# alberto-paparella/MusicRecommendation

Measured on AMD Instinct MI355X. Metric: scored (test-user,song) pairs/sec, ItemBasedModel, 1/2/4/8 MI355X + mAP@10, higher is better.
Workload: dtype int64

## Files before the change

### include/mr_engine.h

```cpp
#ifndef MR_ENGINE_H
#define MR_ENGINE_H

#include <stdint.h>
#include <stddef.h>

#ifdef __cplusplus
extern "C" {
#endif

#define MR_OK          0
#define MR_E_INVALID  -1
#define MR_E_HIP      -2
#define MR_E_OOM      -3
#define MR_E_STATE    -4
#define MR_E_IO       -5
#define MR_E_PARSE    -6
#define MR_E_RCCL     -7

#define MR_UBM 0
#define MR_IBM 1

#define MR_OUT_F32 0
#define MR_OUT_F64 1

typedef struct mr_dataset {
  int32_t n_train_users;
  int32_t n_test_users;
  int32_t n_songs;
  int32_t reserved0;
  const int64_t* tr_off;
  const int32_t* tr_songs;
  const int64_t* te_off;
  const int32_t* te_songs;
  const int32_t* song_count;
  const int32_t* tr_len;
  const int32_t* te_len;
} mr_dataset;

typedef struct mr_options {
  int32_t device;
  int32_t frac_bits;
  int32_t song_lo;
  int32_t song_hi;
  int32_t block_songs;
  int32_t out_dtype;
  int32_t topk;
  int32_t dense;
  int32_t time_kernels;
  int32_t stage1;
  int32_t stage1_chunk;
  int32_t train_order;
  int32_t topk_lists;
  int32_t ibm_route;
  int32_t reserved[2];
} mr_options;

typedef struct mr_ctx mr_ctx;

int mr_options_default(mr_options* opt);

int mr_create(const mr_options* opt, mr_ctx** out);
int mr_destroy(mr_ctx* ctx);

int mr_load(mr_ctx* ctx, const mr_dataset* d);

int mr_shard_info(const mr_ctx* ctx, int32_t* song_lo, int32_t* song_hi, int32_t* n_test_users);

int mr_launch_info(const mr_ctx* ctx, int32_t* shape, int32_t* block_songs, int32_t* n_tiles);

int mr_batch_info(const mr_ctx* ctx, int32_t* batch, int32_t* chunk, int32_t* n_chunks);

int mr_route_info(const mr_ctx* ctx, int32_t* route, int32_t* n_rows, int64_t* pool_entries);

int mr_topk_mode(const mr_ctx* ctx, int32_t* candidate_only);

int mr_cooc_stats(mr_ctx* ctx, int64_t* index_nnz, int64_t* consumed, int64_t* build_reads);

typedef struct mr_cooc_bytes_t {
  int64_t heavy_rows, light_rows;
  int64_t heavy_reads, light_reads;
  int64_t heavy_index_bytes, light_index_bytes;
  int64_t heavy_visits;
  int64_t consumed_bytes;
  int64_t group_tiles;
  int64_t n_groups;
  int64_t index_sparse_entries, index_dense_songs;
  int64_t consumed_sparse_entries, consumed_dense_songs;
} mr_cooc_bytes_t;
int mr_cooc_bytes(mr_ctx* ctx, mr_cooc_bytes_t* out);

int mr_shard_tile_songs(const mr_options* opt, int32_t n_train_users, int32_t n_test_users,
                        int32_t* tile_songs);

int mr_shard_tile_songs_n(const mr_options* opt, int32_t n_train_users, int32_t n_test_users, int32_t n_songs,
                          int32_t n_shards, int32_t* tile_songs);

int mr_run(mr_ctx* ctx, int model);
int mr_sync(mr_ctx* ctx);

int mr_graph_capture(mr_ctx* ctx, int model, int32_t n_steps);
int mr_graph_launch(mr_ctx* ctx);

int mr_device_outputs(const mr_ctx* ctx, void** dense, int32_t** topk_songs,
                      int64_t** topk_keys, double** topk_scores);

int mr_run_into(mr_ctx* ctx, int model, void* dense_dev);

typedef struct mr_view {
  int32_t n_test_users, n_songs, song_lo, song_hi, out_dtype, device;
  const int64_t* te_off;
  const int32_t* te_songs;
  void* stream;
} mr_view;
int mr_view_get(const mr_ctx* ctx, mr_view* view);

int mr_topk_dense_device(mr_ctx* ctx, const void* dense_dev, int32_t k);

int mr_score_dense(mr_ctx* ctx, int model, void* out);
int mr_topk(mr_ctx* ctx, int model, int k, int32_t* songs, double* scores, int64_t* keys);

int mr_copy_dense(mr_ctx* ctx, void* out);
int mr_copy_topk(mr_ctx* ctx, int32_t* songs, double* scores, int64_t* keys);
int mr_copy_topk_device(mr_ctx* ctx, int32_t* songs, int64_t* keys);
int mr_copy_topk_device_async(mr_ctx* ctx, int32_t* songs, int64_t* keys);

int mr_topk_merge_host(int32_t n_shards, int32_t n_te, int32_t k,
                       const int32_t* songs_in, const int64_t* keys_in, const double* scores_in,
                       int32_t* songs_out, int64_t* keys_out, double* scores_out);
int mr_topk_merge_device(mr_ctx* ctx, int32_t n_shards, int32_t n_te, int32_t k,
                         const int32_t* songs_in, const int64_t* keys_in, const double* scores_in,
                         int32_t* songs_out, int64_t* keys_out, double* scores_out);
int mr_topk_merge_device_async(mr_ctx* ctx, int32_t n_shards, int32_t n_te, int32_t k, const int32_t* songs_in,
                               const int64_t* keys_in, int32_t* songs_out, int64_t* keys_out, double* scores_out);

int mr_topk_record_bytes(int32_t n_te, int32_t k, int64_t* rec_bytes);
int mr_topk_merge_records_async(mr_ctx* ctx, int32_t n_shards, int32_t n_te, int32_t k, const void* records,
                                int64_t rec_bytes, int32_t* songs_out, int64_t* keys_out, double* scores_out);

#define MR_COMB_LINEAR      0
#define MR_COMB_AGGREGATION 1
#define MR_COMB_STOCHASTIC  2
int mr_combine_device(mr_ctx* ctx, int kind, double param, uint64_t seed, int64_t pair_base, int64_t n_pairs,
                      const void* ubm, const void* ibm, void* out);
int mr_combine_all_device(mr_ctx* ctx, double alpha, double ibm_percentage, double ibm_probability, uint64_t seed,
                          int64_t pair_base, int64_t n_pairs, const void* ubm, const void* ibm, void* out_linear,
                          void* out_aggregation, void* out_stochastic, double* minmax);
int mr_eval_minmax_device(mr_ctx* ctx, const void* dense, double* mn, double* mx);
int mr_dense_minmax(mr_ctx* ctx, double* mn, double* mx);
int mr_eval_counts_device(mr_ctx* ctx, const void* dense, double mn, double mx, const int64_t* lab_off,
                          const int32_t* lab_songs, int32_t* pred_counts, int32_t* tp_counts, int32_t n_thresholds);
int mr_eval_map(int32_t n_classes, const int32_t* pred_counts, const int32_t* tp_counts, const int32_t* pos,
                int32_t n_label_songs, double* map_out, int32_t n_thresholds);
int mr_eval_map_device(mr_ctx* ctx, const void* dense, double mn, double mx, const int64_t* lab_off,
                       const int32_t* lab_songs, const int32_t* pos, int32_t n_label_songs, double* map_out,
                       int32_t n_thresholds);
int mr_eval_class_counts_device(mr_ctx* ctx, int32_t n_models, const void* const* dense, const double* mn,
                                const double* mx, const int64_t* lab_off, const int32_t* lab_songs, int32_t n_classes,
                                const int32_t* classes, int32_t* counts, int32_t n_thresholds);
int mr_eval_map_counts_device(mr_ctx* ctx, int32_t n_models, int32_t n_classes, const int32_t* class_pos,
                              const int32_t* counts, int32_t n_label_songs, double* maps_out, int32_t n_thresholds);

#define MR_SWEEP_MAX_PARAMS 64
int mr_sweep_minmax_device(mr_ctx* ctx, int kind, int32_t n_params, const double* params, uint64_t seed,
                           int64_t pair_base, int64_t n_pairs, const void* ubm, const void* ibm, double* mn,
                           double* mx);
int mr_sweep_class_counts_device(mr_ctx* ctx, int kind, int32_t n_params, const double* params, uint64_t seed,
                                 int64_t pair_base, int64_t n_pairs, const void* ubm, const void* ibm,
                                 const double* mn, const double* mx, const int64_t* lab_off,
                                 const int32_t* lab_songs, int32_t n_classes, const int32_t* classes,
                                 int32_t* counts, int32_t n_thresholds);
int mr_sweep_map_device(mr_ctx* ctx, int kind, int32_t n_params, const double* params, uint64_t seed,
                        int64_t pair_base, int64_t n_pairs, const void* ubm, const void* ibm, const int64_t* lab_off,
                        const int32_t* lab_songs, const int32_t* pos, int32_t n_label_songs, double* maps_out,
                        double* minmax_out, int32_t n_thresholds);

#define MR_RANK_MAX_K 1024
int mr_rank_dense_device(mr_ctx* ctx, const void* dense_dev, int32_t K, int32_t* songs_dev, double* scores_dev);
int mr_rank_merge_host(int32_t n_lists, int32_t n_te, int32_t K, const int32_t* songs_in, const double* scores_in,
                       int32_t* songs_out, double* scores_out);
int mr_rank_map_device(mr_ctx* ctx, const int32_t* songs_dev, int32_t K, int32_t k_eval, const int64_t* lab_off,
                       const int32_t* lab_songs, double* ap_out, double* map_out);
int mr_rank_map_host(int32_t n_te, const int32_t* songs, int32_t K, int32_t k_eval, const int64_t* lab_off,
                     const int32_t* lab_songs, double* ap_out, double* map_out);

#define MR_SIMILAR_SCRATCH_BYTES (256 << 20)
int mr_similar_songs_device(mr_ctx* ctx, int32_t n_q, const int32_t* query_songs , int32_t K,
                            int32_t* songs_dev, double* scores_dev, double* dense_dev);

#define MR_ASYM_MAX_Q 8
int mr_asym_tables(double alpha, int32_t n, const int32_t* counts, double* pow_a, double* pow_b);
int mr_ibm_asym_device(mr_ctx* ctx, double alpha, int32_t q, void* dense_dev);

#define MR_UASYM_SCRATCH_BYTES (256 << 20)
int mr_ubm_asym_device(mr_ctx* ctx, double alpha, int32_t q, int32_t frac_bits, void* dense_dev);

int mr_kernel_times(mr_ctx* ctx, int32_t which, int64_t* launches, double* total_ms, int32_t reset);

int mr_timing_begin(mr_ctx* ctx);
int mr_timing_stop(mr_ctx* ctx);
int mr_timing_end(mr_ctx* ctx, int64_t* launches, double* total_ms);

int mr_debug_stamps(mr_ctx* ctx, int64_t* out, int64_t n);

void* mr_stream(const mr_ctx* ctx);

const char* mr_last_error(void);

#define MR_TRANSPORT_AUTO 0
#define MR_TRANSPORT_COPY 1
#define MR_TRANSPORT_RCCL 2

typedef struct mr_group_options {
  int32_t n_song_shards;
  int32_t n_user_blocks;
  int32_t transport;
  int32_t n_devices;
  const int32_t* devices;
} mr_group_options;

typedef struct mr_group mr_group;

// ... 45 lines not shown
```

### musicrecommendation_amd/_lib.py

```python
from __future__ import annotations

import ctypes
import os
from ctypes import POINTER, c_char_p, c_double, c_int, c_int32, c_int64, c_void_p

_HERE = os.path.dirname(os.path.abspath(__file__))
_VARIANT = os.environ.get("MR_ENGINE_LIB", "")
LIB_PATH = os.path.join(_HERE, f"libmr_engine_{_VARIANT}.so" if _VARIANT else "libmr_engine.so")

MR_OK = 0
MR_E_INVALID = -1
MR_E_HIP = -2
MR_E_OOM = -3
MR_E_STATE = -4
MR_E_IO = -5
MR_E_PARSE = -6
MR_E_RCCL = -7
MR_TRANSPORT_AUTO, MR_TRANSPORT_COPY, MR_TRANSPORT_RCCL = 0, 1, 2
MR_UBM = 0
MR_IBM = 1
STAGE1 = {"auto": 0, "fused": 1, "separate": 2, "wide": 4}
SHAPES = {0: "separate", 1: "fused", 3: "wide"}
MR_OUT_F32 = 0
MR_OUT_F64 = 1

_ERRNAMES = {
    MR_E_INVALID: "MR_E_INVALID",
    MR_E_HIP: "MR_E_HIP",
    MR_E_OOM: "MR_E_OOM",
    MR_E_STATE: "MR_E_STATE",
    MR_E_IO: "MR_E_IO",
    MR_E_PARSE: "MR_E_PARSE",
    MR_E_RCCL: "MR_E_RCCL",
}


class MrDataset(ctypes.Structure):
    _fields_ = [
        ("n_train_users", c_int32),
        ("n_test_users", c_int32),
        ("n_songs", c_int32),
        ("reserved0", c_int32),
        ("tr_off", POINTER(c_int64)),
        ("tr_songs", POINTER(c_int32)),
        ("te_off", POINTER(c_int64)),
        ("te_songs", POINTER(c_int32)),
        ("song_count", POINTER(c_int32)),
        ("tr_len", POINTER(c_int32)),
        ("te_len", POINTER(c_int32)),
    ]


class MrOptions(ctypes.Structure):
    _fields_ = [
        ("device", c_int32),
        ("frac_bits", c_int32),
        ("song_lo", c_int32),
        ("song_hi", c_int32),
        ("block_songs", c_int32),
        ("out_dtype", c_int32),
        ("topk", c_int32),
        ("dense", c_int32),
        ("time_kernels", c_int32),
        ("stage1", c_int32),
        ("stage1_chunk", c_int32),
        ("train_order", c_int32),
        ("topk_lists", c_int32),
        ("ibm_route", c_int32),
        ("reserved", c_int32 * 2),
    ]


class MrGroupOptions(ctypes.Structure):
    _fields_ = [
        ("n_song_shards", c_int32),
        ("n_user_blocks", c_int32),
        ("transport", c_int32),
        ("n_devices", c_int32),
        ("devices", POINTER(c_int32)),
    ]


class MrView(ctypes.Structure):
    _fields_ = [
        ("n_test_users", c_int32),
        ("n_songs", c_int32),
        ("song_lo", c_int32),
        ("song_hi", c_int32),
        ("out_dtype", c_int32),
        ("device", c_int32),
        ("te_off", c_void_p),
        ("te_songs", c_void_p),
        ("stream", c_void_p),
    ]


class MrCoocBytes(ctypes.Structure):
    _fields_ = [(n, c_int64) for n in ("heavy_rows", "light_rows", "heavy_reads", "light_reads",
                                       "heavy_index_bytes", "light_index_bytes", "heavy_visits", "consumed_bytes",
                                       "group_tiles", "n_groups", "index_sparse_entries", "index_dense_songs",
                                       "consumed_sparse_entries", "consumed_dense_songs")]


MR_COMB_LINEAR = 0
MR_COMB_AGGREGATION = 1
MR_COMB_STOCHASTIC = 2
MR_SWEEP_MAX_PARAMS = 64
MR_RANK_MAX_K = 1024
MR_ASYM_MAX_Q = 8


class EngineError(RuntimeError):
    def __init__(self, code: int, where: str, msg: str):
        super().__init__(f"{where}: {_ERRNAMES.get(code, code)}: {msg}")
        self.code = code


SIGNATURES = {
    "mr_options_default": (c_int, [POINTER(MrOptions)]),
    "mr_create": (c_int, [POINTER(MrOptions), POINTER(c_void_p)]),
    "mr_destroy": (c_int, [c_void_p]),
    "mr_load": (c_int, [c_void_p, POINTER(MrDataset)]),
    "mr_shard_info": (c_int, [c_void_p, POINTER(c_int32), POINTER(c_int32), POINTER(c_int32)]),
    "mr_launch_info": (c_int, [c_void_p, POINTER(c_int32), POINTER(c_int32), POINTER(c_int32)]),
    "mr_batch_info": (c_int, [c_void_p, POINTER(c_int32), POINTER(c_int32), POINTER(c_int32)]),
    "mr_route_info": (c_int, [c_void_p, POINTER(c_int32), POINTER(c_int32), POINTER(c_int64)]),
    "mr_topk_mode": (c_int, [c_void_p, POINTER(c_int32)]),
    "mr_cooc_stats": (c_int, [c_void_p, POINTER(c_int64), POINTER(c_int64), POINTER(c_int64)]),
    "mr_cooc_bytes": (c_int, [c_void_p, POINTER(MrCoocBytes)]),
    "mr_shard_tile_songs": (c_int, [POINTER(MrOptions), c_int32, c_int32, POINTER(c_int32)]),
    "mr_shard_tile_songs_n": (c_int, [POINTER(MrOptions), c_int32, c_int32, c_int32, c_int32, POINTER(c_int32)]),
    "mr_run": (c_int, [c_void_p, c_int]),
    "mr_sync": (c_int, [c_void_p]),
    "mr_graph_capture": (c_int, [c_void_p, c_int, c_int32]),
    "mr_graph_launch": (c_int, [c_void_p]),
    "mr_device_outputs": (c_int, [c_void_p, POINTER(c_void_p), POINTER(c_void_p), POINTER(c_void_p), POINTER(c_void_p)]),
    "mr_score_dense": (c_int, [c_void_p, c_int, c_void_p]),
    "mr_topk": (c_int, [c_void_p, c_int, c_int, c_void_p, c_void_p, c_void_p]),
    "mr_copy_dense": (c_int, [c_void_p, c_void_p]),
    "mr_copy_topk": (c_int, [c_void_p, c_void_p, c_void_p, c_void_p]),
    "mr_copy_topk_device": (c_int, [c_void_p, c_void_p, c_void_p]),
    "mr_copy_topk_device_async": (c_int, [c_void_p, c_void_p, c_void_p]),
    "mr_topk_merge_device_async": (c_int, [c_void_p, c_int32, c_int32, c_int32, c_void_p, c_void_p, c_void_p, c_void_p,
                                           c_void_p]),
    "mr_topk_record_bytes": (c_int, [c_int32, c_int32, POINTER(c_int64)]),
    "mr_topk_merge_records_async": (c_int, [c_void_p, c_int32, c_int32, c_int32, c_void_p, c_int64, c_void_p, c_void_p,
                                            c_void_p]),
    "mr_topk_merge_host": (c_int, [c_int32, c_int32, c_int32, c_void_p, c_void_p, c_void_p, c_void_p, c_void_p, c_void_p]),
    "mr_topk_merge_device": (c_int, [c_void_p, c_int32, c_int32, c_int32, c_void_p, c_void_p, c_void_p, c_void_p, c_void_p, c_void_p]),
    "mr_kernel_times": (c_int, [c_void_p, c_int32, POINTER(c_int64), POINTER(c_double), c_int32]),
    "mr_debug_stamps": (c_int, [c_void_p, c_void_p, c_int64]),
    "mr_timing_begin": (c_int, [c_void_p]),
    "mr_timing_stop": (c_int, [c_void_p]),
    "mr_timing_end": (c_int, [c_void_p, POINTER(c_int64), POINTER(c_double)]),
    "mr_stream": (c_void_p, [c_void_p]),
    "mr_run_into": (c_int, [c_void_p, c_int, c_void_p]),
    "mr_view_get": (c_int, [c_void_p, POINTER(MrView)]),
    "mr_topk_dense_device": (c_int, [c_void_p, c_void_p, c_int32]),
    "mr_combine_device": (c_int, [c_void_p, c_int, c_double, ctypes.c_uint64, c_int64, c_int64, c_void_p, c_void_p, c_void_p]),
    "mr_combine_all_device": (c_int, [c_void_p, c_double, c_double, c_double, ctypes.c_uint64, c_int64, c_int64,
                                      c_void_p, c_void_p, c_void_p, c_void_p, c_void_p, POINTER(c_double)]),
    "mr_eval_minmax_device": (c_int, [c_void_p, c_void_p, POINTER(c_double), POINTER(c_double)]),
    "mr_dense_minmax": (c_int, [c_void_p, POINTER(c_double), POINTER(c_double)]),
    "mr_eval_counts_device": (c_int, [c_void_p, c_void_p, c_double, c_double, c_void_p, c_void_p, c_void_p, c_void_p,
                                      c_int32]),
    "mr_eval_map_device": (c_int, [c_void_p, c_void_p, c_double, c_double, c_void_p, c_void_p, c_void_p, c_int32,
                                   POINTER(c_double), c_int32]),
    "mr_eval_map": (c_int, [c_int32, c_void_p, c_void_p, c_void_p, c_int32, POINTER(c_double), c_int32]),
    "mr_eval_class_counts_device": (c_int, [c_void_p, c_int32, c_void_p, c_void_p, c_void_p, c_void_p, c_void_p,
                                            c_int32, c_void_p, c_void_p, c_int32]),
    "mr_eval_map_counts_device": (c_int, [c_void_p, c_int32, c_int32, c_void_p, c_void_p, c_int32, c_void_p,
                                          c_int32]),
    "mr_sweep_minmax_device": (c_int, [c_void_p, c_int, c_int32, c_void_p, ctypes.c_uint64, c_int64, c_int64, c_void_p,
                                       c_void_p, c_void_p, c_void_p]),
    "mr_sweep_class_counts_device": (c_int, [c_void_p, c_int, c_int32, c_void_p, ctypes.c_uint64, c_int64, c_int64,
                                             c_void_p, c_void_p, c_void_p, c_void_p, c_void_p, c_void_p, c_int32,
                                             c_void_p, c_void_p, c_int32]),
    "mr_sweep_map_device": (c_int, [c_void_p, c_int, c_int32, c_void_p, ctypes.c_uint64, c_int64, c_int64, c_void_p,
                                    c_void_p, c_void_p, c_void_p, c_void_p, c_int32, c_void_p, c_void_p, c_int32]),
    "mr_rank_dense_device": (c_int, [c_void_p, c_void_p, c_int32, c_void_p, c_void_p]),
    "mr_rank_merge_host": (c_int, [c_int32, c_int32, c_int32, c_void_p, c_void_p, c_void_p, c_void_p]),
    "mr_rank_map_device": (c_int, [c_void_p, c_void_p, c_int32, c_int32, c_void_p, c_void_p, c_void_p,
                                   POINTER(c_double)]),
    "mr_rank_map_host": (c_int, [c_int32, c_void_p, c_int32, c_int32, c_void_p, c_void_p, c_void_p,
                                 POINTER(c_double)]),
    "mr_similar_songs_device": (c_int, [c_void_p, c_int32, c_void_p, c_int32, c_void_p, c_void_p, c_void_p]),
    "mr_asym_tables": (c_int, [c_double, c_int32, c_void_p, c_void_p, c_void_p]),
    "mr_ibm_asym_device": (c_int, [c_void_p, c_double, c_int32, c_void_p]),
    "mr_ubm_asym_device": (c_int, [c_void_p, c_double, c_int32, c_int32, c_void_p]),
    "mr_last_error": (c_char_p, []),
    "mr_corpus_from_tsv": (c_int, [c_char_p, c_char_p, c_char_p, POINTER(c_void_p)]),
    "mr_corpus_dataset": (c_int, [c_void_p, POINTER(MrDataset)]),
    "mr_corpus_labels": (c_int, [c_void_p, POINTER(POINTER(c_int64)), POINTER(POINTER(c_int32)), POINTER(c_int32), POINTER(c_int32)]),
    "mr_corpus_name": (c_char_p, [c_void_p, c_int32, c_int32]),
    "mr_corpus_names": (c_int, [c_void_p, c_int32, c_char_p, c_int64, POINTER(c_int64)]),
    "mr_corpus_free": (c_int, [c_void_p]),
    "mr_version": (c_char_p, []),
    "mr_model_write_tsv": (c_int, [c_char_p, c_int32, c_int32, c_void_p, c_void_p, c_void_p, c_int32]),
    "mr_model_read_tsv": (c_int, [c_char_p, c_int32, c_int32, c_void_p, c_void_p, c_void_p]),
    "mr_java_double_string": (c_int, [c_double, c_char_p, c_int32]),
    "mr_song_shards": (c_int, [POINTER(MrDataset), c_int32, c_void_p]),
    "mr_song_shards_tiled": (c_int, [POINTER(MrDataset), c_int32, c_int32, c_void_p]),
    "mr_group_options_default": (c_int, [POINTER(MrGroupOptions)]),
    "mr_group_create": (c_int, [POINTER(MrOptions), POINTER(MrGroupOptions), POINTER(c_void_p)]),
    "mr_group_destroy": (c_int, [c_void_p]),
    "mr_group_load": (c_int, [c_void_p, POINTER(MrDataset)]),
    "mr_group_info": (c_int, [c_void_p, c_int32, POINTER(c_int32), POINTER(c_int32), POINTER(c_int32),
                              POINTER(c_int32), POINTER(c_int32)]),
    "mr_group_transport": (c_int, [c_void_p, POINTER(c_int32)]),
    "mr_group_shape": (c_int, [c_void_p, POINTER(c_int32), POINTER(c_int32), POINTER(c_int32)]),
    "mr_group_context": (c_void_p, [c_void_p, c_int32]),
    "mr_group_run": (c_int, [c_void_p, c_int]),
    "mr_group_sync": (c_int, [c_void_p]),
    "mr_group_copy_topk": (c_int, [c_void_p, c_void_p, c_void_p, c_void_p]),
    "mr_group_topk": (c_int, [c_void_p, c_int, c_int, c_void_p, c_void_p, c_void_p]),
    "mr_group_device_topk": (c_int, [c_void_p, c_int32, POINTER(c_void_p), POINTER(c_void_p), POINTER(c_void_p)]),
    "mr_group_copy_dense": (c_int, [c_void_p, c_void_p]),
    "mr_group_score_dense": (c_int, [c_void_p, c_int, c_void_p]),
    "mr_group_allgather_dense": (c_int, [c_void_p, c_void_p]),
}

_lib = None


def _preload_torch_runtime() -> None:
    try:
        import torch
    except Exception:
        pass


def lib() -> ctypes.CDLL:
    global _lib
    if _lib is not None:
        return _lib
    if not os.path.exists(LIB_PATH):
        raise ImportError(
            f"{LIB_PATH} is missing: build the HIP engine first "
            "(python -c 'import __graft_entry__ as g; g.build()'); there is no CPU fallback"
        )
    _preload_torch_runtime()
    L = ctypes.CDLL(LIB_PATH)
    for name, (res, args) in SIGNATURES.items():
        fn = getattr(L, name)
        fn.restype = res
        fn.argtypes = args
    _lib = L
    return L


def check(rc: int, where: str) -> None:
    if rc != MR_OK:
        msg = lib().mr_last_error()
        raise EngineError(rc, where, msg.decode() if msg else "")
```

### musicrecommendation_amd/csrc/mr_engine.hip

```cpp
#include <hip/hip_runtime.h>

#include <algorithm>
#include <atomic>
#include <climits>
#include <cmath>
#include <cstdarg>
#include <cstdio>
#include <cstdlib>
#include <cstring>
#include <limits>
#include <mutex>
#include <string>
#include <vector>

#ifndef MR_TILE_ROWS
#define MR_TILE_ROWS 32
#endif

#include "mr_engine.h"
#include "mr_hip_util.h"
#include "mr_internal.h"
#include "mr_par.h"
#include "mr_tile_walk.h"


namespace {

using mr_internal::kGridRows;
using mr_internal::kGridRowsXcd;

constexpr int kThreads = 256;
constexpr int kWaves = kThreads / 64;
constexpr int kMaxTopK = 64;
constexpr int kMaxBlockSongs = 16384;
constexpr int kLdsBytes = 160 * 1024;
constexpr int kMaxWideBlockSongs = 65536;
constexpr int kMaxLdsTrainUsers = 16384;
constexpr int kStage1Chunk = 4096;
constexpr int kMaxChunks = 2048;
constexpr int kMaxFusedTrainUsers = 4096;
constexpr long long kKeyNone = -1;
constexpr int kMaxTopkTile = 1024;
constexpr int kMaxTopkLarge = 16;
constexpr int kFusedPre = 4;
constexpr int kWideMapDefault = 1;

thread_local std::string g_err = "no error";

int fail(int code, const char* fmt, ...) {
  char buf[1024];
  va_list ap;
  va_start(ap, fmt);
  vsnprintf(buf, sizeof buf, fmt, ap);
  va_end(ap);
  g_err = buf;
  return code;
}

}

namespace mr_host {
int fail(int code, const char* fmt, ...) {
  char buf[1024];
  va_list ap;
  va_start(ap, fmt);
  vsnprintf(buf, sizeof buf, fmt, ap);
  va_end(ap);
  g_err = buf;
  return code;
}
}

namespace {

struct ScoreLds {
  int acc, y, heard, s_lo, s_w, s_pre, s_scan, wk, ws, fk, fs, flag, cpre, stg, gm, stage_lists, total;
};
constexpr int kTopkScratch256 = (64 + 1) * 12 + 4 + 64 * 4 + 256 * 4;

constexpr int kStgItems = 256;
constexpr int kStgBytes = kStgItems * 8 + kStgItems * 4 + (kStgItems + 4) * 4;

__host__ __device__ inline int align16(int x) { return (x + 15) & ~15; }
__host__ __device__ inline int merge_lists_per_pass(int k);

__host__ __device__ inline ScoreLds score_lds(int bs, int fused_ntr, int k, int n_tiles, int n_chunks = 0) {
  ScoreLds L;
  const int fused = fused_ntr > 0 ? 1 : 0;
  const int kk = k > 0 ? k : 1;
  const int per = merge_lists_per_pass(kk);
  L.stage_lists = (k > 0 && n_tiles > 1) ? (n_tiles < per ? n_tiles : per) : 0;
  int a_bytes = bs * 8 + fused_ntr * 8;
  const int st_bytes = L.stage_lists * kk * 8 + align16(L.stage_lists * kk * 4);
  const int wide_bytes = (k > 0 && bs > kMaxTopkTile) ? kThreads * kk * 8 + kThreads * kk * 4 : 0;
  if (wide_bytes > a_bytes) a_bytes = wide_bytes;
  int o = 0;
  L.acc = o; L.y = bs * 8; o = align16(a_bytes > st_bytes ? a_bytes : st_bytes);
  L.heard = o; o = align16(o + (bs / 32) * 4);
  L.s_lo = o; o += fused * kThreads * 8;
  L.s_w = o; o += fused * kThreads * 8;
  L.s_pre = o; o = align16(o + (kThreads + 1) * 4);
  L.s_scan = o; o = align16(o + kWaves * 4);
  L.wk = o; o = align16(o + kWaves * kMaxTopK * 8);
  L.ws = o; o = align16(o + kWaves * kMaxTopK * 4);
  L.fk = o; o = align16(o + kMaxTopK * 8);
  L.fs = o; o = align16(o + kMaxTopK * 4);
  L.flag = o; o = align16(o + 16);
  L.cpre = o; o = align16(o + (n_chunks > 0 ? (n_chunks + 1) * 4 : 0));
  L.stg = o; o = align16(o + (n_chunks > 0 ? kWaves * kStgBytes : 0));
  L.gm = o; o = align16(o + kTopkScratch256);
  L.total = o;
  return L;
}


constexpr int kStampSlots = 32;
__device__ __forceinline__ void stamp_at(long long* sb, int i) {
#ifdef MR_STAMPS
  if (sb && threadIdx.x == 0) {
    sb[i] = (long long)__builtin_amdgcn_s_memrealtime();
    sb[16 + i] = (long long)__builtin_amdgcn_s_memtime();
  }
#endif
}
__device__ __forceinline__ void stamp_rt(long long* sb, int i) {
#ifdef MR_STAMPS
  if (sb && threadIdx.x == 0) sb[i] = (long long)__builtin_amdgcn_s_memrealtime();
#endif
}
__device__ __forceinline__ void stamp_rt_wave(long long* sb, int i) {
#ifdef MR_STAMPS
  if (sb && (threadIdx.x & 63) == 0) sb[i] = (long long)__builtin_amdgcn_s_memrealtime();
#endif
}
__device__ __forceinline__ void stamp_val(long long* sb, int i, long long v, bool wave = false) {
#ifdef MR_STAMPS
  if (sb && (wave ? (threadIdx.x & 63) == 0 : threadIdx.x == 0)) sb[i] = v;
#endif
}
#ifdef MR_STAMPS
#define MR_STAMP(i) stamp_at(p.stamps ? p.stamps + ((size_t)blockIdx.y * gridDim.x + blockIdx.x) * kStampSlots : nullptr, (i))
#else
#define MR_STAMP(i) do {} while (0)
#endif

__device__ __forceinline__ int wave_incl_scan(int x) {
#ifndef MR_NO_DPP
  x += __builtin_amdgcn_update_dpp(0, x, 0x111, 0xf, 0xf, false);
  x += __builtin_amdgcn_update_dpp(0, x, 0x112, 0xf, 0xf, false);
  x += __builtin_amdgcn_update_dpp(0, x, 0x114, 0xf, 0xf, false);
  x += __builtin_amdgcn_update_dpp(0, x, 0x118, 0xf, 0xf, false);
  x += __builtin_amdgcn_update_dpp(0, x, 0x142, 0xa, 0xf, false);
  x += __builtin_amdgcn_update_dpp(0, x, 0x143, 0xc, 0xf, false);
#else
  const int lane = threadIdx.x & 63;
#pragma unroll
  for (int d = 1; d < 64; d <<= 1) {
    const int y = __shfl_up(x, d, 64);
    if (lane >= d) x += y;
  }
#endif
  return x;
}

__device__ __forceinline__ int wave_lane(int x, int l) { return __builtin_amdgcn_readlane(x, l); }

__host__ __device__ inline unsigned long long ordered_key(double x) {
  unsigned long long b;
  memcpy(&b, &x, sizeof b);
  return (b >> 63) ? ~b : (b | (1ull << 63));
}
__host__ __device__ inline double ordered_value(unsigned long long k) {
  const unsigned long long b = (k >> 63) ? (k & ~(1ull << 63)) : ~k;
  double x;
  memcpy(&x, &b, sizeof x);
  return x;
}

__device__ __forceinline__ int block_excl_scan(int x, int* total, int* sbuf) {
  const int lane = threadIdx.x & 63, w = threadIdx.x >> 6;
  const int incl = wave_incl_scan(x);
  if (lane == 63) sbuf[w] = incl;
  __syncthreads();
  int off = 0, tot = 0;
#pragma unroll
  for (int i = 0; i < kWaves; ++i) {
    int s = sbuf[i];
    off += (i < w) ? s : 0;
    tot += s;
  }
  __syncthreads();
  *total = tot;
  return off + incl - x;
}

__device__ __forceinline__ bool cand_before(long long ka, int sa, long long kb, int sb) {
  return ka > kb || (ka == kb && sa < sb);
}


#define MR_DPP(op, x, mod) asm volatile("s_nop 1\n\t" op " %0, %0, %0 " mod : "+v"(x))
#define MR_DPP_REDUCE(op, x)                                          \
  do {                                                                \
    MR_DPP(op, x, "row_shr:1 row_mask:0xf bank_mask:0xf");            \
    MR_DPP(op, x, "row_shr:2 row_mask:0xf bank_mask:0xf");            \
    MR_DPP(op, x, "row_shr:4 row_mask:0xf bank_mask:0xf");            \
    MR_DPP(op, x, "row_shr:8 row_mask:0xf bank_mask:0xf");            \
    MR_DPP(op, x, "row_bcast:15 row_mask:0xa bank_mask:0xf");         \
    MR_DPP(op, x, "row_bcast:31 row_mask:0xc bank_mask:0xf");         \
    asm volatile("s_nop 1" ::: "memory");                             \
  } while (0)

__device__ __forceinline__ int wave_max_i32(int x) {
  MR_DPP_REDUCE("v_max_i32_dpp", x);
  return __builtin_amdgcn_readlane(x, 63);
}
__device__ __forceinline__ unsigned wave_max_u32(unsigned x) {
  MR_DPP_REDUCE("v_max_u32_dpp", x);
  return (unsigned)__builtin_amdgcn_readlane((int)x, 63);
}
__device__ __forceinline__ int wave_min_i32(int x) {
  MR_DPP_REDUCE("v_min_i32_dpp", x);
  return __builtin_amdgcn_readlane(x, 63);
}

__device__ __forceinline__ void wave_argmax(long long& k, int& s) {
  const int hi = (int)(k >> 32);
  const unsigned lo = (unsigned)(k & 0xffffffffll);
  const int H = wave_max_i32(hi);
  unsigned long long m = __ballot(hi == H);
  unsigned Lo;
  if (__popcll(m) == 1) {
    const int l = __ffsll((long long)m) - 1;
    Lo = (unsigned)__builtin_amdgcn_readlane((int)lo, l);
    s = __builtin_amdgcn_readlane(s, l);
  } else {
    Lo = wave_max_u32(hi == H ? lo : 0u);
    m = __ballot(hi == H && lo == Lo);
    if (__popcll(m) == 1) {
      s = __builtin_amdgcn_readlane(s, __ffsll((long long)m) - 1);
    } else {
      s = wave_min_i32((hi == H && lo == Lo) ? s : INT_MAX);
    }
  }
  k = (long long)(((unsigned long long)(unsigned)H << 32) | Lo);
}

__device__ __forceinline__ void take_if_before(long long& ka, int& sa, long long kb, int sb) {
  const bool t = cand_before(kb, sb, ka, sa);
  ka = t ? kb : ka;
  sa = t ? sb : sa;
}

template <int CTRL>
__device__ __forceinline__ void dpp_take(long long& k, int& s) {
  const unsigned lo = (unsigned)__builtin_amdgcn_update_dpp(0, (int)(unsigned)(unsigned long long)k, CTRL, 0xf, 0xf,
                                                            false);
  const int hi = __builtin_amdgcn_update_dpp(0, (int)(k >> 32), CTRL, 0xf, 0xf, false);
  const int os = __builtin_amdgcn_update_dpp(0, s, CTRL, 0xf, 0xf, false);
  take_if_before(k, s, (long long)(((unsigned long long)(unsigned)hi << 32) | lo), os);
}

template <int GS>
__device__ __forceinline__ void group_best(long long& k, int& s) {
  static_assert(GS == 1 || GS == 2 || GS == 4 || GS == 8 || GS == 16, "group size");
  if constexpr (GS >= 2) dpp_take<0xB1>(k, s);
  if constexpr (GS >= 4) dpp_take<0x4E>(k, s);
  if constexpr (GS >= 8) dpp_take<0x141>(k, s);
  if constexpr (GS >= 16) dpp_take<0x140>(k, s);
}

template <int M>
__device__ __forceinline__ void lane_sort(long long (&rk)[M], int (&rs)[M]) {
#pragma unroll
  for (int round = 0; round < M; ++round) {
#pragma unroll
    for (int j = round & 1; j + 1 < M; j += 2) {
      const bool sw = cand_before(rk[j + 1], rs[j + 1], rk[j], rs[j]);
      const long long k0 = rk[j], k1 = rk[j + 1];
      const int s0 = rs[j], s1 = rs[j + 1];
      rk[j] = sw ? k1 : k0;
      rk[j + 1] = sw ? k0 : k1;
      rs[j] = sw ? s1 : s0;
      rs[j + 1] = sw ? s0 : s1;
    }
  }
}

template <int M, bool SORTED = false>
__device__ __forceinline__ void wave_topk_regs(long long (&rk)[M], int (&rs)[M], int k, long long* out_k,
                                               int* out_s) {
  const int lane = threadIdx.x & 63;
#pragma unroll
  for (int j = 0; j < M; ++j)
    if (rk[j] < 0) { rk[j] = kKeyNone; rs[j] = INT_MAX; }
  if (!SORTED) lane_sort<M>(rk, rs);
  int r = 0;
  for (; r < k; ++r) {
    long long bk = rk[0];
    int bs = rs[0];
    wave_argmax(bk, bs);
    if (bk < 0) break;
    if (lane == 0) { out_k[r] = bk; out_s[r] = bs; }
    const bool win = rk[0] == bk && rs[0] == bs;
#pragma unroll
    for (int j = 0; j + 1 < M; ++j) {
      rk[j] = win ? rk[j + 1] : rk[j];
      rs[j] = win ? rs[j + 1] : rs[j];
    }
    rk[M - 1] = win ? kKeyNone : rk[M - 1];
    rs[M - 1] = win ? INT_MAX : rs[M - 1];
  }
  for (int i = r + lane; i < k; i += 64) { out_k[i] = kKeyNone; out_s[i] = -1; }
}

__device__ __forceinline__ void wave_merge_lists(int L, int k, const long long* lk, const int* ls,
                                                 long long* out_k, int* out_s) {
  const int lane = threadIdx.x & 63;
  int pos[4];
  long long hk[4], nk[4];
  int hs[4], ns[4];
#pragma unroll
  for (int j = 0; j < 4; ++j) {
    const int l = lane + 64 * j;
    pos[j] = 0;
    hk[j] = nk[j] = kKeyNone;
    hs[j] = ns[j] = INT_MAX;
    if (l < L) {
      hk[j] = lk[(size_t)l * k];
      hs[j] = ls[(size_t)l * k];
      if (k > 1) {
        nk[j] = lk[(size_t)l * k + 1];
        ns[j] = ls[(size_t)l * k + 1];
      }
    }
    if (hk[j] < 0) { hk[j] = kKeyNone; hs[j] = INT_MAX; }
    if (nk[j] < 0) { nk[j] = kKeyNone; ns[j] = INT_MAX; }
  }
  int r = 0;
  for (; r < k; ++r) {
    long long bk = hk[0];
    int bs = hs[0];
#pragma unroll
    for (int j = 1; j < 4; ++j) take_if_before(bk, bs, hk[j], hs[j]);
    wave_argmax(bk, bs);
    if (bk < 0) break;
    if (lane == 0) { out_k[r] = bk; out_s[r] = bs; }
#pragma unroll
    for (int j = 0; j < 4; ++j) {
      if (hk[j] == bk && hs[j] == bs) {
        hk[j] = nk[j];
        hs[j] = ns[j];
        ++pos[j];
        nk[j] = kKeyNone;
        ns[j] = INT_MAX;
        if (pos[j] + 1 < k) {
          const int l = lane + 64 * j;
          nk[j] = lk[(size_t)l * k + pos[j] + 1];
          ns[j] = ls[(size_t)l * k + pos[j] + 1];
          if (nk[j] < 0) { nk[j] = kKeyNone; ns[j] = INT_MAX; }
        }
      }
    }
  }
  for (int i = r + lane; i < k; i += 64) { out_k[i] = kKeyNone; out_s[i] = -1; }
}

template <typename Get>
__device__ __forceinline__ void block_topk(int n, int k, Get get, long long* wk, int* ws, long long* out_k,
                                           int* out_s) {
  const int w = threadIdx.x >> 6, lane = threadIdx.x & 63;
  long long rk[4];
  int rs[4];
  if (n <= 256) {
    if (w == 0) {
#pragma unroll
      for (int j = 0; j < 4; ++j) {
        rk[j] = kKeyNone;
        rs[j] = INT_MAX;
        if (lane + 64 * j < n) get(lane + 64 * j, rk[j], rs[j]);
      }
      wave_topk_regs<4>(rk, rs, k, out_k, out_s);
    }
    __syncthreads();
    return;
  }
#pragma unroll
  for (int j = 0; j < 4; ++j) {
    const int i = w * 64 + lane + kThreads * j;
    rk[j] = kKeyNone;
    rs[j] = INT_MAX;
    if (i < n) get(i, rk[j], rs[j]);
  }
  wave_topk_regs<4>(rk, rs, k, wk + w * k, ws + w * k);
  __syncthreads();
  if (w == 0) wave_merge_lists(kWaves, k, wk, ws, out_k, out_s);
  __syncthreads();
}

template <int KS>
__device__ __forceinline__ void lane_list_insert(long long (&tk)[KS], int (&ts)[KS], int k, long long key, int song,
                                                 long long& thr) {
  long long ck = key;
  int cs = song;
#pragma unroll
  for (int t = 0; t < KS; ++t) {
    const bool b = t < k && cand_before(ck, cs, tk[t], ts[t]);
    const long long ok = tk[t];
    const int os = ts[t];
    tk[t] = b ? ck : tk[t];
    ts[t] = b ? cs : ts[t];
    ck = b ? ok : ck;
    cs = b ? os : cs;
  }
  long long nt = kKeyNone;
#pragma unroll
  for (int t = 0; t < KS; ++t) nt = (t == k - 1) ? tk[t] : nt;
  thr = nt;
}

template <typename Get>
__device__ __forceinline__ void block_topk_wide(int n, int k, Get get, long long* lk, int* ls, long long* wk,
                                                int* ws, long long* out_k, int* out_s) {
  const int tid = threadIdx.x, w = tid >> 6;
  long long tk[kMaxTopkLarge];
  int ts[kMaxTopkLarge];
#pragma unroll
  for (int t = 0; t < kMaxTopkLarge; ++t) { tk[t] = kKeyNone; ts[t] = INT_MAX; }
  long long thr = kKeyNone;
  for (int i = tid; i < n; i += kThreads) {
    long long key;
    int song;
    get(i, key, song);
    if (key > thr) lane_list_insert(tk, ts, k, key, song, thr);
  }
  __syncthreads();
#pragma unroll
  for (int t = 0; t < kMaxTopkLarge; ++t)
    if (t < k) { lk[tid * k + t] = tk[t]; ls[tid * k + t] = tk[t] >= 0 ? ts[t] : -1; }
  __syncthreads();
  wave_merge_lists(64, k, lk + (size_t)w * 64 * k, ls + (size_t)w * 64 * k, wk + w * k, ws + w * k);
  __syncthreads();
  if (w == 0) wave_merge_lists(kWaves, k, wk, ws, out_k, out_s);
  __syncthreads();
}

template <int NT, int NG = NT / 16>
__host__ __device__ constexpr int topk_scratch_bytes() {
  return (NG + 1) * 12 + 4 + NG * 4 + 256 * 4;
}
static_assert(topk_scratch_bytes<256, 64>() == kTopkScratch256, "score_lds scratch size");
template <int NT, typename Get>
__device__ __forceinline__ void thread_best(int n, Get get, long long& mk, int& ms) {
  mk = kKeyNone;
  ms = INT_MAX;
#pragma unroll 4
  for (int i = threadIdx.x; i < n; i += NT) {
    long long key;
    int song;
    get(i, key, song);
    if (key >= 0) take_if_before(mk, ms, key, song);
  }
}
struct TopkDst {
  long long* key = nullptr;
  int* song = nullptr;
  double* score = nullptr;
  bool sc1 = false;
};
__device__ __forceinline__ void topk_dst_write(const TopkDst& d, int slot, long long key, int song) {
  if (d.sc1) {
    __hip_atomic_store(d.key + slot, key, __ATOMIC_RELAXED, __HIP_MEMORY_SCOPE_AGENT);
    __hip_atomic_store(d.song + slot, song, __ATOMIC_RELAXED, __HIP_MEMORY_SCOPE_AGENT);
  } else {
    d.key[slot] = key;
    d.song[slot] = song;
  }
  if (d.score) d.score[slot] = key >= 0 ? __longlong_as_double(key) : (double)NAN;
}

#ifndef MR_LIGHT_CAS1
#define MR_LIGHT_CAS1 1
#endif
#ifndef MR_LIGHT_FDIV
#define MR_LIGHT_FDIV 1
#endif
__device__ __forceinline__ int tile_of(int key, int bs, float inv_bs) {
  if (!MR_LIGHT_FDIV) return key / bs;
  int t = (int)((float)key * inv_bs);
  t -= t * bs > key ? 1 : 0;
  t += (t + 1) * bs <= key ? 1 : 0;
  return t;
}

#ifndef MR_RANK_Q_FUSED
#define MR_RANK_Q_FUSED 64
#endif
#ifndef MR_RANK_Q_WIDE
#define MR_RANK_Q_WIDE 16
#endif
#ifndef MR_MERGE_INTERLEAVE
#define MR_MERGE_INTERLEAVE 1
#endif
#ifndef MR_RANK_UNROLL_FUSED
#define MR_RANK_UNROLL_FUSED 4
#endif
template <int NT>
constexpr int kRankQ = NT <= 256 ? MR_RANK_Q_FUSED : MR_RANK_Q_WIDE;
template <int NT>
constexpr int kRankU = NT <= 256 ? MR_RANK_UNROLL_FUSED : 1;

template <int NT>
__device__ __forceinline__ void rank_survivors(int nc, int k, const long long* ck, const int* cs, int* crank,
                                               long long* out_k, int* out_s, const TopkDst& dst = TopkDst{}) {
  const int tid = threadIdx.x, lane = tid & 63;
  if (nc * nc > kRankQ<NT> * NT) {
    if (tid < 64) {
      long long rk[4];
      int rs[4];
#pragma unroll
      for (int j = 0; j < 4; ++j) {
        const int c = lane + 64 * j;
        rk[j] = c < nc ? ck[c] : kKeyNone;
        rs[j] = c < nc ? cs[c] : INT_MAX;
      }
      wave_topk_regs<4>(rk, rs, k, out_k, out_s);
    }
    __syncthreads();
    if (dst.key)
      for (int r = tid; r < k; r += NT) topk_dst_write(dst, r, out_k[r], out_s[r]);
    return;
  }
  if (nc > 0) {
    const int sl = NT / nc;
    const int per = (nc + sl - 1) / sl;
    if (tid < sl * nc) {
      const int i = tid % nc, j0 = (tid / nc) * per;
      const long long mine = ck[i];
      const int mines = cs[i];
      int c = 0;
      const int je = min(nc, j0 + per);
      int j = j0;
      constexpr int U = kRankU<NT>;
      if constexpr (U > 1) {
        for (; j + U <= je; j += U) {
          long long o[U];
          int os[U];
#pragma unroll
          for (int r = 0; r < U; ++r) { o[r] = ck[j + r]; os[r] = cs[j + r]; }
#pragma unroll
          for (int r = 0; r < U; ++r) c += cand_before(o[r], os[r], mine, mines) ? 1 : 0;
        }
      }
      for (; j < je; ++j) c += cand_before(ck[j], cs[j], mine, mines) ? 1 : 0;
      if (c) atomicAdd(&crank[i], c);
    }
  }
  __syncthreads();
  if (dst.key) {
    if (tid < nc && crank[tid] < k) topk_dst_write(dst, crank[tid], ck[tid], cs[tid]);
    if (tid >= nc && tid < k) topk_dst_write(dst, tid, kKeyNone, -1);
    return;
  }
  if (tid < nc && crank[tid] < k) { out_k[crank[tid]] = ck[tid]; out_s[crank[tid]] = cs[tid]; }
  if (tid >= nc && tid < k) { out_k[tid] = kKeyNone; out_s[tid] = -1; }
  __syncthreads();
}


template <int NT, int NG = NT / 16>
__device__ __forceinline__ void block_tau(int k, long long mk, int ms, unsigned char* gm, long long& tau_k,
                                          int& tau_s, long long* sb = nullptr) {
  constexpr int GS = NT / NG;
  static_assert(NT % 64 == 0 && NT % NG == 0 && NG <= 64 && GS <= 64 && NT * 16 >= NG * NG,
                "block shape");
  long long* gk = reinterpret_cast<long long*>(gm);
  int* gs = reinterpret_cast<int*>(gk + NG + 1);
  int* counter = gs + NG + 1;
  int* grank = counter + 1;
  int* crank = grank + NG;
  const int tid = threadIdx.x, lane = tid & 63;
#ifndef MR_NO_DPP
  if constexpr (GS <= 16) {
    group_best<GS>(mk, ms);
  } else
#endif
  {
#pragma unroll
    for (int d = 1; d < GS; d <<= 1) {
      const long long ok = __shfl_xor(mk, d, 64);
      const int os = __shfl_xor(ms, d, 64);
      take_if_before(mk, ms, ok, os);
    }
  }
  if ((lane & (GS - 1)) == 0) { gk[tid / GS] = mk; gs[tid / GS] = ms; }
  if (tid < NG) grank[tid] = 0;
  if (tid == 0) *counter = 0;
  __syncthreads();
  stamp_at(sb, 9);
  {
    constexpr int SL = NT / NG, PER = (NG + SL - 1) / SL;
    const int i = tid % NG, j0 = (tid / NG) * PER;
    const long long mine = gk[i];
    const int mines = gs[i];
    int c = 0;
#pragma unroll
    for (int jj = 0; jj < PER; ++jj) {
      const int j = j0 + jj;
      if (j < NG) {
        const long long o = gk[j];
        const int os = gs[j];
        c += (cand_before(o, os, mine, mines) || (o == mine && os == mines && j < i)) ? 1 : 0;
      }
    }
    if (c) atomicAdd(&grank[i], c);
  }
  __syncthreads();
  if (tid < NG && grank[tid] == k - 1) { gk[NG] = gk[tid]; gs[NG] = gs[tid]; }
  if (tid < 256) crank[tid] = 0;
  __syncthreads();
  stamp_at(sb, 10);
  tau_k = gk[NG];
  tau_s = gs[NG];
  if (tau_k < 0) { tau_k = 0; tau_s = INT_MAX; }
}

template <int NT, typename Get, int NG = NT / 16>
__device__ __forceinline__ bool block_topk_threshold(int n, int k, Get get, long long mk, int ms, unsigned char* gm,
                                                     long long* ck, int* cs, int cap, long long* out_k, int* out_s,
                                                     long long* sb = nullptr, const TopkDst& dst = TopkDst{}) {
  long long* gk = reinterpret_cast<long long*>(gm);
  int* gs = reinterpret_cast<int*>(gk + NG + 1);
  int* counter = gs + NG + 1;
  int* crank = counter + 1 + NG;
  const int tid = threadIdx.x;
  if (k > NG || k <= 0 || cap > 256) return false;
  long long tk;
  int tsg;
  block_tau<NT, NG>(k, mk, ms, gm, tk, tsg, sb);
#pragma unroll 4
  for (int i = tid; i < n; i += NT) {
    long long key;
    int song;
    get(i, key, song);
    if (key >= 0 && !cand_before(tk, tsg, key, song)) {
      const int pos = atomicAdd(counter, 1);
      if (pos < cap) { ck[pos] = key; cs[pos] = song; }
    }
  }
  __syncthreads();
  stamp_at(sb, 11);
  const int nc = *counter;
  if (nc > cap) return false;
  rank_survivors<NT>(nc, k, ck, cs, crank, out_k, out_s, dst);
  return true;
}

constexpr int kMergeStageBytes = 32 * 1024;
__host__ __device__ inline int merge_lists_per_pass(int k) {
  const int kk = k > 0 ? k : 1;
  int l = kMergeStageBytes / (12 * kk);
  return l > 256 ? 256 : (l < 2 ? 2 : l);
}

__device__ __forceinline__ void wave_lds_sync() {
  __builtin_amdgcn_fence(__ATOMIC_RELEASE, "wavefront");
  __builtin_amdgcn_wave_barrier();
  __builtin_amdgcn_fence(__ATOMIC_ACQUIRE, "wavefront");
}

template <typename T>
__device__ __forceinline__ void st_sc1(T* p, T v) {
  __hip_atomic_store(p, v, __ATOMIC_RELAXED, __HIP_MEMORY_SCOPE_AGENT);
}
template <typename T>
__device__ __forceinline__ T ld_sc1(const T* p) {
  return __hip_atomic_load(const_cast<T*>(p), __ATOMIC_RELAXED, __HIP_MEMORY_SCOPE_AGENT);
}

struct NbrParams {
  int n_tr;
  int user0;
  int cap;
  int frac_bits;
  int chunk, n_chunks;
  const long long* te_off;
  const int* te_songs;
  const long long* trs_off;
  const int* trs_users;
  const long long* q_song;
  const double* sqrt_tr;
  const double* sqrt_te;
  int* nbr_v;
  long long* nbr_q;
  int* nbr_cnt;
  const int* sbound;
};

__device__ __forceinline__ long long lower_bound_user(const int* trs_users, long long lo, long long hi, int v) {
  while (lo < hi) {
    const long long m = (lo + hi) >> 1;
    if (trs_users[m] < v) lo = m + 1; else hi = m;
  }
  return lo;
}

template <int MODEL, typename Add, typename Mark>
__device__ __forceinline__ void walk_neighbours(long long t0, long long t1, const int* te_songs,
                                                const long long* trs_off, const int* trs_users,
                                                const long long* q_song, long long* s_lo, long long* s_w,
                                                int* s_pre, int* s_scan, Add add, Mark mark, bool ranged = false,
                                                int v0 = 0, int v1 = 0, const int* sbound = nullptr,
                                                int chunk_idx = 0, int nc1 = 0, const int2* te_rng = nullptr,
                                                const long long* te_q = nullptr, long long* sb = nullptr) {
  const int tid = threadIdx.x;
  for (long long base = t0; base < t1; base += kThreads) {
    const int n = (int)min((long long)kThreads, t1 - base);
    int len = 0;
    if (tid < n && te_rng && !ranged) {
      const int s2 = te_songs[base + tid];
      const int2 r = te_rng[base + tid];
      len = r.y;
      s_lo[tid] = r.x;
      s_w[tid] = (MODEL == MR_IBM) ? te_q[base + tid] : 1ll;
      mark(s2);
    } else if (tid < n) {
      const int s2 = te_songs[base + tid];
      long long lo = trs_off[s2], hi = trs_off[s2 + 1];
      if (ranged && sbound) {
        const int* b = sbound + (size_t)s2 * nc1 + chunk_idx;
        lo = b[0];
        hi = b[1];
      } else if (ranged) {
        lo = lower_bound_user(trs_users, lo, hi, v0);
        hi = lower_bound_user(trs_users, lo, hi, v1);
      }
      len = (int)(hi - lo);
      s_lo[tid] = lo;
      s_w[tid] = (MODEL == MR_IBM) ? q_song[s2] : 1ll;
      mark(s2);
    }
    int total;
    const int pre = block_excl_scan(len, &total, s_scan);
    s_pre[tid] = pre;
    if (tid == 0) s_pre[kThreads] = total;
    __syncthreads();
    stamp_at(sb, 10);
    const int nsteps = n > 1 ? 32 - __clz(n - 1) : 0;
    for (int i0 = tid; i0 < total; i0 += 16 * kThreads) {
      const int ib = i0 - tid;
      int v[16];
      unsigned long long wv[16];
#pragma unroll
      for (int r = 0; r < 16; ++r) { v[r] = -1; wv[r] = 0ull; }
#pragma unroll
      for (int g2 = 0; g2 < 4; g2 += 2) {
        if (ib + g2 * 4 * kThreads >= total) break;
        if (ib + (g2 + 1) * 4 * kThreads < total) {
          int a[8], b[8];
#pragma unroll
          for (int e = 0; e < 8; ++e) { a[e] = 0; b[e] = n; }
          for (int st = 0; st < nsteps; ++st) {
#pragma unroll
            for (int e = 0; e < 8; ++e) {
              const int i = i0 + (g2 * 4 + e) * kThreads;
              const int m = (a[e] + b[e]) >> 1;
              if (s_pre[m] <= i) a[e] = m; else b[e] = m;
            }
          }
#pragma unroll
          for (int e = 0; e < 8; ++e) {
            const int i = i0 + (g2 * 4 + e) * kThreads;
            if (i < total) {
              v[g2 * 4 + e] = trs_users[s_lo[a[e]] + (i - s_pre[a[e]])];
              wv[g2 * 4 + e] = (unsigned long long)s_w[a[e]];
            }
          }
          continue;
        }
        const int g = g2;
        int a[4], b[4];
#pragma unroll
        for (int e = 0; e < 4; ++e) { a[e] = 0; b[e] = n; }
        for (int st = 0; st < nsteps; ++st) {
#pragma unroll
          for (int e = 0; e < 4; ++e) {
            const int i = i0 + (g * 4 + e) * kThreads;
            const int m = (a[e] + b[e]) >> 1;
            if (s_pre[m] <= i) a[e] = m; else b[e] = m;
          }
        }
#pragma unroll
        for (int e = 0; e < 4; ++e) {
          const int i = i0 + (g * 4 + e) * kThreads;
          if (i < total) {
            v[g * 4 + e] = trs_users[s_lo[a[e]] + (i - s_pre[a[e]])];
            wv[g * 4 + e] = (unsigned long long)s_w[a[e]];
          }
        }
      }
#pragma unroll
      for (int r = 0; r < 16; ++r)
        if (v[r] >= 0) add(v[r], wv[r]);
    }
    stamp_at(sb, 11);
    __syncthreads();
  }
}

template <int MODEL>
__device__ __forceinline__ void accumulate_neighbours(unsigned long long* Y, long long t0, long long t1,
                                                      const int* te_songs, const long long* trs_off,
                                                      const int* trs_users, const long long* q_song,
                                                      long long* s_lo, long long* s_w, int* s_pre, int* s_scan,
                                                      unsigned* heard, int blo, int bhi, bool ranged = false,
                                                      int v0 = 0, int v1 = 0, const int* sbound = nullptr,
                                                      int chunk_idx = 0, int nc1 = 0, const int2* te_rng = nullptr,
                                                      const long long* te_q = nullptr, long long* sb = nullptr) {
  walk_neighbours<MODEL>(
      t0, t1, te_songs, trs_off, trs_users, q_song, s_lo, s_w, s_pre, s_scan,
      [&](int v, unsigned long long w) { atomicAdd(&Y[v - v0], w); },
      [&](int s2) {
        if (heard && s2 >= blo && s2 < bhi) atomicOr(&heard[(s2 - blo) >> 5], 1u << ((s2 - blo) & 31));
      },
      ranged, v0, v1, sbound, chunk_idx, nc1, te_rng, te_q, sb);
}

template <int MODEL>
__device__ __forceinline__ long long neighbour_weight(unsigned long long y, double rs_u, double sqrt_tr_v,
                                                      double two_f) {
  if (MODEL == MR_IBM) return (long long)y;
  const double c = (double)(long long)y / (rs_u * sqrt_tr_v);
  return (long long)rint(c * two_f);
}

template <int MODEL>
__global__ __launch_bounds__(kThreads) void k_neighbours(NbrParams p) {
  extern __shared__ __align__(16) unsigned char smem_raw[];
  unsigned long long* Y = reinterpret_cast<unsigned long long*>(smem_raw);
  long long* s_lo = reinterpret_cast<long long*>(smem_raw + align16(p.chunk * 8));
  long long* s_w = s_lo + kThreads;
  int* s_pre = reinterpret_cast<int*>(s_w + kThreads);
  int* s_scan = s_pre + kThreads + 4;

  const int c = blockIdx.x;
  const int bu = blockIdx.y;
  const int u = p.user0 + bu;
  const int tid = threadIdx.x;
  const int cv0 = c * p.chunk, cv1 = min(p.n_tr, cv0 + p.chunk), cw = cv1 - cv0;
  for (int i = tid; i < cw; i += kThreads) Y[i] = 0ull;
  __syncthreads();
  accumulate_neighbours<MODEL>(Y, p.te_off[u], p.te_off[u + 1], p.te_songs, p.trs_off, p.trs_users, p.q_song,
                               s_lo, s_w, s_pre, s_scan, nullptr, 0, 0, p.n_chunks > 1, cv0, cv1, p.sbound, c,
                               p.n_chunks + 1);

  const double two_f = ldexp(1.0, p.frac_bits);
  const double rs_u = p.sqrt_te[u];
  int* out_v = p.nbr_v + (size_t)bu * p.cap + (size_t)c * p.chunk;
  long long* out_q = p.nbr_q + (size_t)bu * p.cap + (size_t)c * p.chunk;
  const int lane = tid & 63, w = tid >> 6;
  const int q4 = (cw + kWaves * 64 - 1) / (kWaves * 64) * 64;
  const int wb = min(cw, w * q4), we = min(cw, wb + q4);
  int nz = 0;
  for (int i0 = wb; i0 < we; i0 += 64) {
    const int i = i0 + lane;
    nz += __popcll(__ballot(i < we && Y[i] != 0ull));
  }
  if (lane == 0) s_scan[w] = nz;
  __syncthreads();
  int base = 0, written = 0;
#pragma unroll
  for (int x = 0; x < kWaves; ++x) {
    base += x < w ? s_scan[x] : 0;
    written += s_scan[x];
  }
  const unsigned long long below = lane ? (~0ull >> (64 - lane)) : 0ull;
  for (int i0 = wb; i0 < we; i0 += 64) {
    const int i = i0 + lane;
    const unsigned long long y = i < we ? Y[i] : 0ull;
    const unsigned long long m = __ballot(y != 0ull);
    if (y != 0ull) {
      const int pos = base + __popcll(m & below);
      const int v = cv0 + i;
      out_v[pos] = v;
      out_q[pos] = neighbour_weight<MODEL>(y, rs_u, MODEL == MR_UBM ? p.sqrt_tr[v] : 0.0, two_f);
    }
    base += __popcll(m);
  }
  if (tid == 0) p.nbr_cnt[(size_t)bu * p.n_chunks + c] = written;
}

#ifndef MR_FUSED_SCHED
#define MR_FUSED_SCHED 1
#endif
#ifndef MR_SCHED_SE
#define MR_SCHED_SE 8
#endif
#ifndef MR_COUNTER_STRIDE
#define MR_COUNTER_STRIDE 64
#endif
constexpr int kCounterStride = MR_COUNTER_STRIDE;
struct ScoreParams {
  int n_tr;
  int user0;
  int song_lo, song_hi, width;
  int block_songs, n_tiles;
  int frac_bits, topk, dense;
  const long long* te_off;
  const int* te_songs;
  const int* toff;
  const unsigned short* tsongs;
  const unsigned* tpack;
  const int2* te_rng;
  const long long* te_q;
  const uint2* te_sched;
  const long long* sched_off;
  const double* sqrt_c;
  const long long* trs_off;
  const int* trs_users;
  const long long* q_song;
  const double* sqrt_tr;
  const double* sqrt_te;
  int cap;
  int chunk, n_chunks;
  int n_users, xcd_remap;
  int merge_rows;
  const int* nbr_v;
  const long long* nbr_q;
  const int* nbr_cnt;
  void* dense_out;
  long long* cand_key;
  int* cand_song;
  unsigned* counter;
  long long* top_key;
  int* top_song;
  double* top_score;
  long long* stamps;
  int topk_lists;
  int n_rows, nseg;
  const int* te_row;
  const long long* seg_off;
  const int* seg_len;
  const unsigned* pool;
  unsigned long long* mm_key;
  int mm_n;
  int cand;
  const float* rsq_c;
};

template <int MODEL, typename OutT, bool FUSED>
__global__ __launch_bounds__(kThreads) void k_score(ScoreParams p) {
  extern __shared__ __align__(16) unsigned char smem_raw[];
  const int bs = p.block_songs;
  const ScoreLds L = score_lds(bs, FUSED ? p.n_tr : 0, p.topk, p.n_tiles, FUSED ? 0 : p.n_chunks);
  unsigned long long* acc = reinterpret_cast<unsigned long long*>(smem_raw + L.acc);
  unsigned* heard = reinterpret_cast<unsigned*>(smem_raw + L.heard);
  long long* wk = reinterpret_cast<long long*>(smem_raw + L.wk);
  int* ws = reinterpret_cast<int*>(smem_raw + L.ws);
  long long* fk = reinterpret_cast<long long*>(smem_raw + L.fk);
  int* fs = reinterpret_cast<int*>(smem_raw + L.fs);
  int* flag = reinterpret_cast<int*>(smem_raw + L.flag);

  int tile = blockIdx.x;
  int bu = blockIdx.y;
  if (p.xcd_remap) {
    const int lin = blockIdx.y * gridDim.x + blockIdx.x;
    const int slot = lin >> 3;
    bu = (slot / p.n_tiles) * 8 + (lin & 7);
    tile = slot % p.n_tiles;
    if (bu >= p.n_users) return;
  }
  const int u = p.user0 + bu;
  const int tid = threadIdx.x;
  const int blo = p.song_lo + tile * bs;
  const int bhi = min(p.song_hi, blo + bs);
  const int bw = bhi - blo;
  const double two_f = ldexp(1.0, p.frac_bits);
#ifdef MR_STAMPS
  long long* sb = p.stamps ? p.stamps + ((size_t)blockIdx.y * gridDim.x + blockIdx.x) * kStampSlots : nullptr;
#endif
  MR_STAMP(0);

  for (int i = tid; i < bw; i += kThreads) acc[i] = 0ull;
  for (int i = tid; i < bs / 32; i += kThreads) heard[i] = 0u;
  const long long t0 = p.te_off[u], t1 = p.te_off[u + 1];
  const bool sched = FUSED && p.te_sched != nullptr;
  constexpr int kSE = MR_SCHED_SE;
  long long se0 = 0, se1 = 0;
  int hs0 = -1;
  uint2 sc1[kSE];
  if (sched) {
    se0 = p.sched_off[u];
    se1 = p.sched_off[u + 1];
    if (t1 > t0) hs0 = p.te_songs[min(t0 + tid, t1 - 1)];
    if (se1 > se0) {
#pragma unroll
      for (int r = 0; r < kSE; ++r) sc1[r] = p.te_sched[min(se0 + tid + (long long)r * kThreads, se1 - 1)];
    }
  }
  double sc[kFusedPre];
#pragma unroll
  for (int j = 0; j < kFusedPre; ++j) {
    const int i = tid + j * kThreads;
    sc[j] = (MODEL == MR_IBM && i < bw) ? p.sqrt_c[blo + i] : 1.0;
  }

  if (FUSED) {
    const int e0 = p.toff[(size_t)tile * p.n_tr], e1 = p.toff[(size_t)(tile + 1) * p.n_tr];
    unsigned pk[kFusedPre];
#pragma unroll
    for (int j = 0; j < kFusedPre; ++j) {
      const int i = e0 + tid + j * kThreads;
      pk[j] = i < e1 ? p.tpack[i] : 0xffffffffu;
    }
    double str[kFusedPre];
#pragma unroll
    for (int r = 0; r < kFusedPre; ++r) {
      const int v = tid + r * kThreads;
      str[r] = (MODEL == MR_UBM && v < p.n_tr) ? p.sqrt_tr[v] : 1.0;
    }
    unsigned long long* Y = reinterpret_cast<unsigned long long*>(smem_raw + L.y);
    int v[kSE];
    unsigned long long wv[kSE];
    auto gather = [&]() {
#pragma unroll
      for (int r = 0; r < kSE; ++r) {
        v[r] = p.trs_users[sc1[r].x];
        wv[r] = (MODEL == MR_IBM) ? (unsigned long long)p.te_q[t0 + sc1[r].y] : 1ull;
      }
    };
    const bool any = sched && se1 > se0;
    for (int i = tid; i < p.n_tr; i += kThreads) Y[i] = 0ull;
    __syncthreads();
    if (sched) {
      if (any) gather();
      auto mark = [&](int s2) {
        if (s2 >= blo && s2 < bhi) atomicOr(&heard[(s2 - blo) >> 5], 1u << ((s2 - blo) & 31));
      };
      if (t0 + tid < t1) mark(hs0);
      for (long long i = t0 + tid + kThreads; i < t1; i += kThreads) mark(p.te_songs[i]);
#ifdef MR_STAMPS
      stamp_at(sb, 10);
#endif
      for (long long i0 = se0 + tid; any;) {
#pragma unroll
        for (int r = 0; r < kSE; ++r)
          if (i0 + (long long)r * kThreads < se1) atomicAdd(&Y[v[r]], wv[r]);
        i0 += (long long)kSE * kThreads;
        if (i0 >= se1) break;
#pragma unroll
        for (int r = 0; r < kSE; ++r) sc1[r] = p.te_sched[min(i0 + (long long)r * kThreads, se1 - 1)];
        gather();
      }
#ifdef MR_STAMPS
      stamp_at(sb, 11);
#endif
      __syncthreads();
    } else
    accumulate_neighbours<MODEL>(Y, t0, t1, p.te_songs, p.trs_off, p.trs_users, p.q_song,
                                 reinterpret_cast<long long*>(smem_raw + L.s_lo),
                                 reinterpret_cast<long long*>(smem_raw + L.s_w),
                                 reinterpret_cast<int*>(smem_raw + L.s_pre),
                                 reinterpret_cast<int*>(smem_raw + L.s_scan), heard, blo, bhi, false, 0, 0,
                                 nullptr, 0, 0, p.te_rng, p.te_q,
#ifdef MR_STAMPS
                                 sb
#else
                                 nullptr
#endif
    );
    MR_STAMP(1);
    if (MODEL == MR_UBM) {
      const double rs_u = p.sqrt_te[u];
      for (int v = tid, r = 0; v < p.n_tr; v += kThreads, ++r) {
        const unsigned long long y = Y[v];
        if (y != 0ull) {
          double sv;
          if (r < kFusedPre) {
            sv = str[0];
#pragma unroll
            for (int x = 1; x < kFusedPre; ++x) sv = r == x ? str[x] : sv;
          } else {
            sv = p.sqrt_tr[v];
          }
          Y[v] = (unsigned long long)neighbour_weight<MODEL>(y, rs_u, sv, two_f);
        }
      }
      __syncthreads();
    }
#pragma unroll
    for (int j = 0; j < kFusedPre; ++j) {
      if (pk[j] == 0xffffffffu) continue;
      const unsigned long long y = Y[pk[j] >> 16];
      if (y != 0ull) atomicAdd(&acc[pk[j] & 0xffffu], y);
    }
    for (int i = e0 + tid + kFusedPre * kThreads; i < e1; i += kThreads) {
      const unsigned e = p.tpack[i];
      const unsigned long long y = Y[e >> 16];
      if (y != 0ull) atomicAdd(&acc[e & 0xffffu], y);
    }
  } else {
    __syncthreads();
    for (long long i = t0 + tid; i < t1; i += kThreads) {
      const int s = p.te_songs[i];
      if (s >= blo && s < bhi) atomicOr(&heard[(s - blo) >> 5], 1u << ((s - blo) & 31));
    }
    int* cpre = reinterpret_cast<int*>(smem_raw + L.cpre);
    int* s_scan = reinterpret_cast<int*>(smem_raw + L.s_scan);
    const int nch = p.n_chunks;
    int cnt = 0;
    for (int c0 = 0; c0 < nch; c0 += kThreads) {
      const int cc = c0 + tid;
      const int x = cc < nch ? p.nbr_cnt[(size_t)bu * nch + cc] : 0;
      int tot;
      const int pre = block_excl_scan(x, &tot, s_scan);
      if (cc < nch) cpre[cc] = cnt + pre;
      cnt += tot;
    }
    if (tid == 0) cpre[nch] = cnt;
    __syncthreads();
    MR_STAMP(1);
    const int* nv = p.nbr_v + (size_t)bu * p.cap;
    const long long* nq = p.nbr_q + (size_t)bu * p.cap;
    const int lane = tid & 63, w = tid >> 6;
    unsigned char* stg = smem_raw + L.stg + w * kStgBytes;
    unsigned long long* st_q = reinterpret_cast<unsigned long long*>(stg);
    int* st_a = reinterpret_cast<int*>(stg + kStgItems * 8);
    int* st_pre = st_a + kStgItems;
    constexpr int R = kStgItems / 64;
    constexpr int E = 16;
    const int* toff_t = p.toff + (size_t)tile * p.n_tr;
    int cur = 0;
    auto load_list = [&](int k0, int (&v)[R], unsigned long long (&q)[R]) {
#pragma unroll
      for (int r = 0; r < R; ++r) {
        const int k = k0 + r * 64 + lane;
        v[r] = -1;
        q[r] = 0ull;
        if (k < cnt) {
          while (cur + 1 < nch && cpre[cur + 1] <= k) ++cur;
          const size_t idx = (size_t)cur * p.chunk + (k - cpre[cur]);
          v[r] = nv[idx];
          q[r] = (unsigned long long)nq[idx];
        }
      }
    };
    auto load_offsets = [&](const int (&v)[R], int (&a)[R], int (&b)[R]) {
#pragma unroll
      for (int r = 0; r < R; ++r) {
        a[r] = b[r] = 0;
        if (v[r] >= 0) {
          a[r] = toff_t[v[r]];
          b[r] = toff_t[v[r] + 1];
        }
      }
    };
    const int step = kWaves * kStgItems;
    int v0[R], a0[R], b0[R], v1[R], a1[R], b1[R], v2[R];
    unsigned long long q0[R], q1[R], q2[R];
    int k0 = w * kStgItems;
    load_list(k0, v0, q0);
    load_offsets(v0, a0, b0);
    load_list(k0 + step, v1, q1);
    for (; k0 < cnt; k0 += step) {
      int run = 0;
#pragma unroll
      for (int r = 0; r < R; ++r) {
        const int len = b0[r] - a0[r];
        const int incl = wave_incl_scan(len);
        const int it = r * 64 + lane;
        st_a[it] = a0[r];
        st_pre[it] = run + incl - len;
        st_q[it] = q0[r];
        run += __shfl(incl, 63, 64);
      }
      if (lane == 0) st_pre[kStgItems] = run;
      wave_lds_sync();
      load_offsets(v1, a1, b1);
      load_list(k0 + 2 * step, v2, q2);
      for (int j0 = 0; j0 < run; j0 += 64 * E) {
        int song[E], it[E];
#pragma unroll
        for (int e = 0; e < E; ++e) {
          const int j = j0 + e * 64 + lane;
          song[e] = -1;
          it[e] = 0;
          if (j < run) {
            int lo = 0, hi = kStgItems;
#pragma unroll
            for (int st = 0; st < 8; ++st) {
              const int m = (lo + hi) >> 1;
              if (st_pre[m] <= j) lo = m; else hi = m;
            }
            song[e] = (int)p.tsongs[st_a[lo] + (j - st_pre[lo])];
            it[e] = lo;
          }
        }
#pragma unroll
        for (int e = 0; e < E; ++e)
          if (song[e] >= 0) atomicAdd(&acc[song[e]], st_q[it[e]]);
      }
      wave_lds_sync();
#pragma unroll
      for (int r = 0; r < R; ++r) {
        a0[r] = a1[r]; b0[r] = b1[r]; q0[r] = q1[r];
        v1[r] = v2[r]; q1[r] = q2[r];
      }
    }
  }
  __syncthreads();
  MR_STAMP(2);

  const double inv_f = ldexp(1.0, -p.frac_bits);
  OutT* out = reinterpret_cast<OutT*>(p.dense_out) + (size_t)u * p.width + (blo - p.song_lo);
  long long mk = kKeyNone;
  int ms = INT_MAX;
#pragma unroll
  for (int j = 0; j < kFusedPre; ++j) {
    const int i = tid + j * kThreads;
    if (i < bw) {
      const bool h = (heard[i >> 5] >> (i & 31)) & 1u;
      double score = (double)(long long)acc[i] * inv_f;
      if (MODEL == MR_IBM) score = score / sc[j];
      if (p.dense) out[i] = h ? (OutT)NAN : (OutT)score;
      const long long key = h ? kKeyNone : __double_as_longlong(score);
      acc[i] = (unsigned long long)key;
      if (key > mk) { mk = key; ms = blo + i; }
    }
  }
  for (int i = tid + kFusedPre * kThreads; i < bw; i += kThreads) {
    const bool h = (heard[i >> 5] >> (i & 31)) & 1u;
    double score = (double)(long long)acc[i] * inv_f;
    if (MODEL == MR_IBM) score = score / p.sqrt_c[blo + i];
    if (p.dense) out[i] = h ? (OutT)NAN : (OutT)score;
    const long long key = h ? kKeyNone : __double_as_longlong(score);
    acc[i] = (unsigned long long)key;
    if (key > mk) { mk = key; ms = blo + i; }
  }
  const int k = p.topk;
  if (k <= 0) return;
  __syncthreads();
  MR_STAMP(3);

  auto get_key = [&](int i, long long& key, int& song) {
    key = (long long)acc[i];
    song = blo + i;
  };
  bool thr_done = false;
  long long* ck = p.cand_key + (size_t)u * p.n_tiles * k;
  int* cs = p.cand_song + (size_t)u * p.n_tiles * k;
  TopkDst tdst;
#ifndef MR_TOPK_VIA_LDS
  if (p.n_tiles == 1) {
    tdst.key = p.top_key + (size_t)u * k;
    tdst.song = p.top_song + (size_t)u * k;
    tdst.score = p.top_score + (size_t)u * k;
  } else {
    tdst.key = ck + (size_t)tile * k;
    tdst.song = cs + (size_t)tile * k;
    tdst.sc1 = true;
  }
#endif
  if (!p.topk_lists && k <= kThreads / 16) {
#ifdef MR_STAMPS
    long long* sbt = sb ? sb + 3 : nullptr;
#else
    long long* sbt = nullptr;
#endif
    thr_done = block_topk_threshold<kThreads, decltype(get_key), MR_TILE_ROWS>(
        bw, k, get_key, mk, ms, smem_raw + L.gm, wk, ws, kWaves * kMaxTopK, fk, fs, sbt, tdst);
  }
  const bool direct = thr_done && tdst.key;
  if (thr_done) {
  } else if (bs <= kMaxTopkTile) {
    block_topk(bw, k, get_key, wk, ws, fk, fs);
  } else {
    long long* lk = reinterpret_cast<long long*>(smem_raw + L.acc);
    int* ls = reinterpret_cast<int*>(smem_raw + L.acc + kThreads * k * 8);
    block_topk_wide(bw, k, get_key, lk, ls, wk, ws, fk, fs);
  }
  MR_STAMP(4);

  if (p.n_tiles == 1) {
    if (!direct)
      for (int r = tid; r < k; r += kThreads) {
        const size_t o = (size_t)u * k + r;
        p.top_key[o] = fk[r];
        p.top_song[o] = fs[r];
        p.top_score[o] = fk[r] >= 0 ? __longlong_as_double(fk[r]) : (double)NAN;
      }
    return;
  }

  if (!direct)
    for (int r = tid; r < k; r += kThreads) {
      st_sc1(&ck[(size_t)tile * k + r], fk[r]);
      st_sc1(&cs[(size_t)tile * k + r], fs[r]);
    }
  asm volatile("s_waitcnt vmcnt(0)" ::: "memory");
  __syncthreads();
  if (tid == 0) {
    const unsigned old = __hip_atomic_fetch_add(&p.counter[(size_t)u * kCounterStride], 1u, __ATOMIC_RELAXED,
                                                __HIP_MEMORY_SCOPE_AGENT);
    *flag = (old == (unsigned)(p.n_tiles - 1));
  }
  __syncthreads();
  MR_STAMP(5);
#ifdef MR_STAMPS
  if (tid == 0 && sb)
    sb[15] = (long long)(*flag) | ((long long)__builtin_amdgcn_s_getreg((20 << 0) | (0 << 6) | (3 << 11)) << 8);
#endif
  if (!*flag) return;

  bool merged_direct = false;
  {
    long long* mk = reinterpret_cast<long long*>(smem_raw + L.acc);
    int* ms = reinterpret_cast<int*>(smem_raw + L.acc + L.stage_lists * k * 8);
    const int w = tid >> 6;
    int done = 0, off = 0;
    merged_direct = false;
#ifndef MR_MERGE_VIA_LDS
    const int nck = p.n_tiles * k;
    if (!p.topk_lists && nck <= kThreads && k <= kThreads / 16 && p.merge_rows == 32) {
      long long rk = kKeyNone;
      int rs = INT_MAX;
      if (tid < nck) {
#if MR_MERGE_INTERLEAVE
        const int ci = (tid % p.n_tiles) * k + tid / p.n_tiles;
#else
        const int ci = tid;
#endif
        rk = ld_sc1(&ck[ci]);
        rs = ld_sc1(&cs[ci]);
      }
      MR_STAMP(6);
      auto get_r = [&](int, long long& key, int& song) { key = rk; song = rs; };
      TopkDst mdst;
      mdst.key = p.top_key + (size_t)u * k;
      mdst.song = p.top_song + (size_t)u * k;
      mdst.score = p.top_score + (size_t)u * k;
      merged_direct = block_topk_threshold<kThreads, decltype(get_r), 32>(
          nck, k, get_r, rk >= 0 ? rk : kKeyNone, rk >= 0 ? rs : INT_MAX, smem_raw + L.gm, wk, ws,
          kWaves * kMaxTopK, fk, fs, nullptr, mdst);
      MR_STAMP(8);
    }
#endif
    while (!merged_direct && done < p.n_tiles) {
      const int nl = min(p.n_tiles - done, L.stage_lists - off);
      for (int i0 = tid; i0 < nl * k; i0 += 4 * kThreads) {
        long long lk4[4];
        int ls4[4];
#pragma unroll
        for (int r = 0; r < 4; ++r) {
          const int i = i0 + r * kThreads;
          lk4[r] = kKeyNone;
          ls4[r] = -1;
          if (i < nl * k) {
            lk4[r] = ld_sc1(&ck[(size_t)done * k + i]);
            ls4[r] = ld_sc1(&cs[(size_t)done * k + i]);
          }
        }
#pragma unroll
        for (int r = 0; r < 4; ++r) {
          const int i = i0 + r * kThreads;
          if (i < nl * k) {
            mk[off * k + i] = lk4[r];
            ms[off * k + i] = ls4[r];
          }
        }
      }
      for (int i = tid; i < off * k; i += kThreads) {
        mk[i] = fk[i];
        ms[i] = fs[i];
      }
      __syncthreads();
      MR_STAMP(6);
      bool merged = false;
      TopkDst mdst;
#ifndef MR_TOPK_VIA_LDS
      mdst.key = p.top_key + (size_t)u * k;
      mdst.song = p.top_song + (size_t)u * k;
      mdst.score = p.top_score + (size_t)u * k;
#endif
      if (!p.topk_lists && done == 0 && nl == p.n_tiles && k <= kThreads / 16) {
        auto get_c = [&](int i, long long& key, int& song) { key = mk[i]; song = ms[i]; };
        long long bk;
        int bsg;
        thread_best<kThreads>(nl * k, get_c, bk, bsg);
        if (p.merge_rows == 16)
          merged = block_topk_threshold<kThreads, decltype(get_c), 16>(nl * k, k, get_c, bk, bsg, smem_raw + L.gm,
                                                                      wk, ws, kWaves * kMaxTopK, fk, fs, nullptr, mdst);
        else if (p.merge_rows == 64)
          merged = block_topk_threshold<kThreads, decltype(get_c), 64>(nl * k, k, get_c, bk, bsg, smem_raw + L.gm,
                                                                      wk, ws, kWaves * kMaxTopK, fk, fs, nullptr, mdst);
        else
          merged = block_topk_threshold<kThreads, decltype(get_c), 32>(nl * k, k, get_c, bk, bsg, smem_raw + L.gm,
                                                                      wk, ws, kWaves * kMaxTopK, fk, fs, nullptr, mdst);
      }
      if (!merged) {
        if (w == 0) wave_merge_lists(nl + off, k, mk, ms, fk, fs);
        __syncthreads();
      }
      MR_STAMP(8);
      merged_direct = merged && mdst.key;
      done += nl;
      off = 1;
    }
  }
  if (!merged_direct)
    for (int r = tid; r < k; r += kThreads) {
      const size_t o = (size_t)u * k + r;
      p.top_key[o] = fk[r];
      p.top_song[o] = fs[r];
      p.top_score[o] = fk[r] >= 0 ? __longlong_as_double(fk[r]) : (double)NAN;
    }
  if (tid == 0) p.counter[(size_t)u * kCounterStride] = 0u;
  MR_STAMP(9);
}

template <int NT>
__device__ __forceinline__ int block_excl_scan_nt(int x, int* total, int* sbuf) {
  constexpr int NW = NT / 64;
  const int lane = threadIdx.x & 63, w = threadIdx.x >> 6;
  const int incl = wave_incl_scan(x);
  if (lane == 63) sbuf[w] = incl;
  __syncthreads();
  int off = 0, tot = 0;
#pragma unroll
  for (int i = 0; i < NW; ++i) {
    const int v = sbuf[i];
    off += (i < w) ? v : 0;
    tot += v;
  }
  __syncthreads();
  *total = tot;
  return off + incl - x;
}

template <int NT>
struct WideLds {
  int acc, heard, cpre, s_scan, wk, ws, fk, fs, gm, total;
  WideLds<1024> as_wide() const { return WideLds<1024>{acc, heard, cpre, s_scan, wk, ws, fk, fs, gm, total}; }
};
template <int NT>
__host__ __device__ inline WideLds<NT> wide_lds(int bs, int k, int n_chunks) {
  constexpr int NW = NT / 64;
  const int kk = k > 0 ? k : 1;
  WideLds<NT> L;
  int o = 0;
  L.acc = o; o = align16(o + bs * 8);
  L.heard = o; o = align16(o + (bs / 32) * 4);
  L.cpre = o; o = align16(o + (n_chunks + 1) * 4);
  L.s_scan = o; o = align16(o + NW * 4);
  L.wk = o; o = align16(o + NW * kk * 8);
  L.ws = o; o = align16(o + NW * kk * 4);
  L.fk = o; o = align16(o + kk * 8);
  L.fs = o; o = align16(o + kk * 4);
  L.gm = o; o = align16(o + topk_scratch_bytes<NT>());
  L.total = o;
  return L;
}

constexpr int kWideThreads = 1024;
#ifndef MR_WIDE_R
#define MR_WIDE_R 4
#endif
#ifndef MR_WIDE_SEG
#define MR_WIDE_SEG 12
#endif
#ifndef MR_WIDE_Z16
#define MR_WIDE_Z16 1
#endif
#ifndef MR_WIDE_EB
#define MR_WIDE_EB 8
#endif
#ifndef MR_COOC_U
#define MR_COOC_U 4
#endif
#ifndef MR_COOC_DU
#define MR_COOC_DU 4
#endif
#ifndef MR_COOC_DS
#define MR_COOC_DS 8
#endif
#ifndef MR_COOC_SPLIT
#define MR_COOC_SPLIT 1
#endif
#ifndef MR_COOC_DOT2
#define MR_COOC_DOT2 1
#endif
typedef unsigned short us2_t __attribute__((ext_vector_type(2)));
#ifndef MR_COOC_NOZERO
#define MR_COOC_NOZERO 1
#endif
#ifndef MR_GROUP_STUB
#define MR_GROUP_STUB 0
#endif
#ifndef MR_COOC_DPF
#define MR_COOC_DPF 1
#endif
#ifndef MR_COOC_PF
#define MR_COOC_PF 0
#endif
#ifndef MR_COOC_R
#define MR_COOC_R 2
#endif
#ifndef MR_COOC_NT16
#define MR_COOC_NT16 512
#endif
#ifndef MR_COOC_P16
#define MR_COOC_P16 1
#endif
#ifndef MR_COOC_NT
#define MR_COOC_NT 1024
#endif
typedef unsigned u32x4_a4 __attribute__((ext_vector_type(4), aligned(4)));
constexpr int kCoocCntBits = 17;
constexpr int kCoocDenseTail = -3;
constexpr int kDenseDS = MR_COOC_DS;
constexpr int kDenseBlock = 64 * kDenseDS;
__host__ __device__ inline int cooc_dense_words(int bw) {
  return (bw + kDenseBlock - 1) / kDenseBlock * (kDenseBlock / 4);
}
__host__ __device__ inline int cooc_dense_song(int c, int i) { return (c >> 6) * kDenseBlock + 64 * i + (c & 63); }
constexpr int kCoocDenseDiv = 3;
#ifndef MR_COOC_BIG_ROW
#define MR_COOC_BIG_ROW 2048
#endif
constexpr int kCoocBigRow = MR_COOC_BIG_ROW;
constexpr unsigned kCoocCntMask = (1u << kCoocCntBits) - 1u;
constexpr int kCoocMaxTile = 1 << (32 - kCoocCntBits);

#ifndef MR_WIDE_U16
constexpr bool kWideWordSeg = true;
#else
constexpr bool kWideWordSeg = false;
#endif

#ifndef MR_CAND_EB
#define MR_CAND_EB 4
#endif
#ifndef MR_CAND_PRE
#define MR_CAND_PRE 1
#endif
template <int MODEL, int NT, int EMAX>
__device__ __forceinline__ bool wide_cand_topk(const ScoreParams& p, const unsigned long long* acc,
                                               const unsigned* heard, int blo, int bw, int k, unsigned char* gm,
                                               long long* ck, int* cs, int cap, long long* fk, int* fs,
                                               long long* sb, bool have_rv, const float (&pre_rv)[MR_CAND_EB]) {
  constexpr int NG = NT / 16;
  const int tid = threadIdx.x;
  float ap[EMAX];
  float ba = -1.f;
  int be = -1;
  constexpr int EB = MR_CAND_EB;
#pragma unroll
  for (int e0 = 0; e0 < EMAX; e0 += EB) {
    unsigned long long av[EB];
    float rv[EB];
#pragma unroll
    for (int j = 0; j < EB; ++j) {
      const int i = tid + (e0 + j) * NT;
      av[j] = 0ull;
// ... 1492 lines not shown
    p.top_song[o] = fs[r];
    p.top_score[o] = fk[r] >= 0 ? __longlong_as_double(fk[r]) : (double)NAN;
  }
}

constexpr long long kWideMinUserPairs = 100000;

struct MergeParams {
  int n_lists, k_in, k_out;
  long long user_stride, list_stride_k, list_stride_s;
  const long long* keys;
  const int* songs;
  long long* out_keys;
  int* out_songs;
  double* out_scores;
};

inline int64_t topk_record_bytes(size_t n) { return (int64_t)((12 * n + 15) / 16 * 16); }

__host__ __device__ inline int merge_lds_bytes(int k) {
  return align16(merge_lists_per_pass(k) * k * 12) + align16(kMaxTopK * 12);
}

__global__ __launch_bounds__(kThreads) void k_topk_merge(MergeParams p) {
  extern __shared__ __align__(16) unsigned char smem_raw[];
  const int k = p.k_out;
  const int per = merge_lists_per_pass(k);
  long long* mk = reinterpret_cast<long long*>(smem_raw);
  int* ms = reinterpret_cast<int*>(mk + per * k);
  long long* fk = reinterpret_cast<long long*>(smem_raw + align16(per * k * 12));
  int* fs = reinterpret_cast<int*>(fk + kMaxTopK);
  const int bu = blockIdx.x;
  const int tid = threadIdx.x;
  const long long* keys = p.keys + (size_t)bu * p.user_stride;
  const int* songs = p.songs + (size_t)bu * p.user_stride;
  int done = 0, off = 0;
  while (done < p.n_lists) {
    const int nl = min(p.n_lists - done, per - off);
    for (int i = tid; i < nl * k; i += kThreads) {
      const int l = done + i / k, r = i - (i / k) * k;
      const bool in = r < p.k_in;
      mk[off * k + i] = in ? keys[(size_t)l * p.list_stride_k + r] : kKeyNone;
      ms[off * k + i] = in ? songs[(size_t)l * p.list_stride_s + r] : -1;
    }
    for (int i = tid; i < off * k; i += kThreads) {
      mk[i] = fk[i];
      ms[i] = fs[i];
    }
    __syncthreads();
    if ((tid >> 6) == 0) wave_merge_lists(nl + off, k, mk, ms, fk, fs);
    __syncthreads();
    done += nl;
    off = 1;
  }
  const size_t o = (size_t)bu * k;
  for (int r = tid; r < k; r += kThreads) {
    p.out_keys[o + r] = fk[r];
    p.out_songs[o + r] = fs[r];
    if (p.out_scores) p.out_scores[o + r] = fk[r] >= 0 ? __longlong_as_double(fk[r]) : (double)NAN;
  }
}

__global__ __launch_bounds__(256) void k_sbound(const long long* trs_off, const int* trs_users, int n_s, int nc1,
                                                int chunk, int* sbound) {
  const size_t total = (size_t)n_s * nc1;
  for (size_t i = (size_t)blockIdx.x * 256 + threadIdx.x; i < total; i += (size_t)gridDim.x * 256) {
    const int s = (int)(i / nc1);
    const long long bound = (long long)(int)(i - (size_t)s * nc1) * chunk;
    long long a = trs_off[s], b = trs_off[s + 1];
    while (a < b) {
      const long long m = (a + b) >> 1;
      if (trs_users[m] < bound) a = m + 1; else b = m;
    }
    sbound[i] = (int)a;
  }
}

template <typename T>
struct DevBuf {
  T* p = nullptr;
  size_t n = 0;
  bool own = true;
  void release() {
    if (p && own) (void)hipFree(p);
    p = nullptr;
    n = 0;
    own = true;
  }
};

template <typename T>
int dev_alloc(DevBuf<T>& b, size_t n) {
  b.release();
  if (n == 0) n = 1;
  MR_HIP(hipMalloc(reinterpret_cast<void**>(&b.p), n * sizeof(T)));
  b.n = n;
  return MR_OK;
}

template <typename T>
int dev_upload(DevBuf<T>& b, const T* src, size_t n, hipStream_t st) {
  int rc = dev_alloc(b, n);
  if (rc) return rc;
  if (n) MR_HIP(hipMemcpyAsync(b.p, src, n * sizeof(T), hipMemcpyHostToDevice, st));
  return MR_OK;
}

using ScoreKernel = void (*)(ScoreParams);
using NbrKernel = void (*)(NbrParams);

enum Shape { kShapeSeparate = 0, kShapeFused = 1, kShapeWide = 3 };

struct CoocPlan {
  int route = 1;
  std::vector<int32_t> row_song, te_row;
  std::vector<int64_t> row_base;
  std::vector<int64_t> row_reads;
  std::vector<int32_t> row_slots;
  std::vector<int32_t> heavy_rows, light_rows;
  std::vector<int32_t> shard_deg;
  std::vector<int32_t> row_users;
  std::vector<int32_t> row_listeners;
  std::vector<uint8_t> row_light;
  int64_t build_reads = 0;
  int64_t pool_cap = 0;
  int32_t max_shard_deg = 0;
  int n_light_tier[6] = {0, 0, 0, 0, 0, 0};
  bool all32 = false;
  int n_heavy32 = 0;
  int n_big16 = 0, tcap16 = 0, tcap32 = 0;
  int dense_div = 0, force32 = 0;
  unsigned sat = 255;
  int grp = 0, n_grp = 0, urec_words = 0, lrec_words = 0;
  int64_t n_lrec = 0;
  int64_t n_llrec = 0;
  int group_nt = 1024;
  int cooc_nt = 1024;
  int n_rows() const { return (int)row_song.size(); }
  int n_heavy() const { return (int)heavy_rows.size(); }
  int n_light() const { return (int)light_rows.size(); }
};

inline bool is_u32_row(const CoocPlan& p, int32_t listeners) { return p.all32 || listeners >= 65536; }

}

struct mr_ctx {
  mr_options opt{};
  int dev_share = 1;
  hipStream_t stream = nullptr;
  bool loaded = false;
  bool ran = false;
  bool fused = false;
  int shape = kShapeSeparate;
  int last_model = -1;
  int n_tr = 0, n_te = 0, n_s = 0;
  int song_lo = 0, song_hi = 0, width = 0;
  int block_songs = 0, n_tiles = 0;
  int cap = 0, batch = 0;
  int chunk = 1, n_chunks = 1;
  size_t score_lds = 0, nbr_lds = 0, merge_lds = 0, wide_lds = 0;
  ScoreKernel score_kernel[2] = {nullptr, nullptr};
  NbrKernel nbr_kernel[2] = {nullptr, nullptr};
  DevBuf<long long> tr_off, te_off, trs_off, q_song, cand_key, top_key, nbr_q;
  DevBuf<int> te_songs, trs_users, toff, nbr_v, nbr_cnt, cand_song, top_song;
  DevBuf<unsigned short> tsongs;
  DevBuf<unsigned> tpack;
  DevBuf<int2> te_rng;
  DevBuf<long long> te_q;
  DevBuf<uint2> te_sched;
  DevBuf<long long> sched_off;
  DevBuf<int> sbound;
  DevBuf<unsigned> counter;
  DevBuf<double> sqrt_c, sqrt_tr, sqrt_te, top_score;
  DevBuf<float> rsq_c;
  std::vector<int32_t> song_count;
  std::vector<int32_t> te_len_h, tr_len_h;
  int32_t max_ctr = 0;
  bool cand_on = false;
  DevBuf<unsigned char> dense;
  DevBuf<long long> stamps;
  hipEvent_t stage_ev[2] = {nullptr, nullptr};
  static constexpr int kRing = 1024;
  std::vector<hipEvent_t> ring;
  int ring_used = 0;
  bool ring_has_stage1[kRing] = {};
  long long launches[3] = {0, 0, 0};
  double ms[3] = {0, 0, 0};
  hipEvent_t win[2] = {nullptr, nullptr};
  bool win_open = false;
  bool win_stopped = false;
  void* dense_override = nullptr;
  DevBuf<unsigned long long> mm_key;
  bool mm_on = false, mm_valid = false;
  hipGraph_t graph = nullptr;
  hipGraphExec_t graph_exec = nullptr;
  int graph_steps = 0;
  DevBuf<unsigned> flag;
  long long win_launches = 0;
  CoocPlan cooc;
  size_t cooc_score_lds = 0, cooc_lds = 0;
  int nseg = 0;
  ScoreKernel cooc_kernel = nullptr;
  DevBuf<int> row_song, te_row, seg_len;
  DevBuf<long long> row_base, seg_off;
  DevBuf<unsigned> pool;
  DevBuf<unsigned> row_nnz;
  bool cooc_ran = false;
  hipStream_t side[2] = {nullptr, nullptr};
  hipEvent_t side_fork = nullptr, side_join[2] = {nullptr, nullptr};
  size_t bstamp_off = 0;
  size_t lstamp_off = 0;
  DevBuf<int> rows_order, row_slots;
  DevBuf<int4> rdesc;
  DevBuf<long long> sr_off;
  DevBuf<unsigned> sr_songs;
  DevBuf<unsigned> urec;
  DevBuf<unsigned> lrec;
  DevBuf<uint2> llrec;

  void release_data() {
    tr_off.release(); te_off.release(); trs_off.release(); q_song.release();
    cand_key.release(); top_key.release(); nbr_q.release();
    tsongs.release(); tpack.release(); te_rng.release(); te_q.release(); te_sched.release(); sched_off.release(); te_songs.release(); trs_users.release(); toff.release(); sbound.release();
    nbr_v.release(); nbr_cnt.release(); cand_song.release(); top_song.release();
    counter.release();
    sqrt_c.release(); sqrt_tr.release(); sqrt_te.release(); top_score.release();
    rsq_c.release(); cand_on = false;
    song_count = std::vector<int32_t>();
    te_len_h = std::vector<int32_t>(); tr_len_h = std::vector<int32_t>(); max_ctr = 0;
    dense.release();
    mm_key.release(); mm_on = mm_valid = false;
    stamps.release();
    flag.release();
    row_song.release(); te_row.release(); seg_len.release(); row_base.release(); seg_off.release();
    pool.release();
    rows_order.release(); row_slots.release(); sr_off.release(); sr_songs.release(); row_nnz.release();
    urec.release(); lrec.release(); llrec.release(); rdesc.release();
    cooc = CoocPlan{};
    cooc_kernel = nullptr;
    if (graph_exec) (void)hipGraphExecDestroy(graph_exec);
    if (graph) (void)hipGraphDestroy(graph);
    graph_exec = nullptr;
    graph = nullptr;
    graph_steps = 0;
    loaded = ran = cooc_ran = false;
  }
};

namespace {

template <class F>
int64_t first_bad(int64_t n, F&& bad, int64_t grain = 1 << 14) {
  std::atomic<int64_t> best{INT64_MAX};
  mr_par::parallel_for(n, [&](int64_t lo, int64_t hi, int) {
    for (int64_t i = lo; i < hi && i < best.load(std::memory_order_relaxed); ++i)
      if (bad(i)) {
        int64_t cur = best.load();
        while (i < cur && !best.compare_exchange_weak(cur, i)) {}
        return;
      }
  }, grain);
  const int64_t b = best.load();
  return b == INT64_MAX ? -1 : b;
}

int validate_csr(const char* what, int n_rows, int n_cols, const int64_t* off, const int32_t* col) {
  if (!off || (off[n_rows] > 0 && !col)) return fail(MR_E_INVALID, "%s: null CSR array", what);
  if (off[0] != 0) return fail(MR_E_INVALID, "%s: offsets[0] = %lld != 0", what, (long long)off[0]);
  const int64_t r0 = first_bad(n_rows, [&](int64_t r) { return off[r + 1] < off[r]; });
  if (r0 >= 0) return fail(MR_E_INVALID, "%s: offsets decrease at row %d", what, (int)r0);
  const int64_t r1 = first_bad(n_rows, [&](int64_t r) {
    for (int64_t i = off[r]; i < off[r + 1]; ++i)
      if (col[i] < 0 || col[i] >= n_cols || (i > off[r] && col[i] <= col[i - 1])) return true;
    return false;
  }, 1 << 10);
  if (r1 >= 0) {
    const int r = (int)r1;
    for (int64_t i = off[r]; i < off[r + 1]; ++i) {
      if (col[i] < 0 || col[i] >= n_cols)
        return fail(MR_E_INVALID, "%s: row %d has column %d outside [0,%d)", what, r, col[i], n_cols);
      if (i > off[r] && col[i] <= col[i - 1])
        return fail(MR_E_INVALID, "%s: row %d is not sorted strictly ascending", what, r);
    }
  }
  if (off[n_rows] >= (int64_t)INT32_MAX)
    return fail(MR_E_INVALID, "%s: %lld entries exceed the int32 index range", what, (long long)off[n_rows]);
  return MR_OK;
}

std::vector<int64_t> weighted_cuts(const int64_t* prefix, int64_t n, int parts) {
  std::vector<int64_t> cut(parts + 1, n);
  cut[0] = 0;
  const int64_t total = prefix[n] - prefix[0];
  for (int w = 1; w < parts; ++w) {
    const int64_t target = prefix[0] + total * w / parts;
    cut[w] = std::max(cut[w - 1], (int64_t)(std::lower_bound(prefix, prefix + n + 1, target) - prefix));
    cut[w] = std::min(cut[w], n);
  }
  return cut;
}

int merge_rows_opt() {
  static const int rows = [] {
    const char* e = std::getenv("MR_MERGE_ROWS");
    const int r = e ? std::atoi(e) : 32;
    return (r == 16 || r == 64) ? r : 32;
  }();
  return rows;
}

constexpr int64_t kLightSlotsNarrow = 8192;
int64_t cooc_light_max_opt(bool narrow) {
  const char* e = std::getenv("MR_COOC_LIGHT_MAX");
  int64_t v = e ? std::atoll(e) : (narrow ? kLightSlotsNarrow : kLightSlots);
  int64_t s = 1024;
  while (s * 2 <= std::min<int64_t>(v, kLightSlots)) s *= 2;
  return s;
}
int64_t cooc_light_load_opt() {
  const char* e = std::getenv("MR_COOC_LIGHT_LOAD");
  const int64_t v = e ? std::atoll(e) : 80;
  return std::min<int64_t>(100, std::max<int64_t>(10, v));
}
bool cooc_light_opt() {
  const char* e = std::getenv("MR_COOC_LIGHT");
  return !(e && std::atoi(e) == 0);
}
bool fused_sched_opt() {
  const char* e = std::getenv("MR_FUSED_SCHED");
  return MR_FUSED_SCHED && !(e && std::atoi(e) == 0);
}
int cooc_nt_opt() {
  const char* e = std::getenv("MR_COOC_NT");
  return e && std::atoi(e) == 512 ? 512 : 1024;
}
int cooc_group_nt_opt() {
  const char* e = std::getenv("MR_COOC_GNT");
  return e && std::atoi(e) == 512 ? 512 : 1024;
}
int cooc_group_max_opt() {
  const char* e = std::getenv("MR_COOC_GRP");
  const int v = e ? std::atoi(e) : 0;
  return v > 0 ? v : kMaxGroupTiles;
}
bool cooc_group_opt() {
  const char* e = std::getenv("MR_COOC_GROUP");
  return !(e && std::atoi(e) == 0);
}
bool cooc_side_opt() {
  const char* e = std::getenv("MR_COOC_SIDE");
  return !(e && std::atoi(e) == 0);
}
int cooc_dense_div_opt() {
  const char* e = std::getenv("MR_COOC_DENSE_DIV");
  return e ? std::max(0, std::atoi(e)) : kCoocDenseDiv;
}
int cooc_dense32_opt() {
  const char* e = std::getenv("MR_COOC_DENSE32");
  return e && std::atoi(e) == 1 ? 1 : 0;
}
unsigned cooc_sat_opt() {
  const char* e = std::getenv("MR_COOC_SAT");
  const long v = e ? std::atol(e) : 255;
  return (unsigned)std::min<long>(255, std::max<long>(1, v));
}

bool cooc_pays(double v_est, double e_est, const std::vector<int64_t>& bound, const std::vector<int64_t>& reads,
               const std::vector<int32_t>& row_song, const std::vector<int32_t>& col_tr, int n_tiles) {
  double build = 0.0;
  for (size_t r = 0; r < row_song.size(); ++r) {
    const double c = col_tr[row_song[r]];
    if (bound[r] <= light_bound_max(kLightSlots) && c <= kLightCntMask) build += 12.8e-12 * (double)(reads[r] - c) + 28e-9;
    else build += n_tiles * (35e-12 * c + 24e-9);
  }
  return build + 0.49e-12 * e_est < 5.75e-12 * v_est;
}

int batch_users_opt() {
  const char* e = std::getenv("MR_BATCH_USERS");
  const int n = e ? std::atoi(e) : 0;
  return n >= 1 ? n : 0;
}

int wide_map_opt() {
  static const int m = [] {
    const char* e = std::getenv("MR_WIDE_MAP");
    const int v = e ? std::atoi(e) : 0;
    return v >= 1 && v <= 3 ? v : kWideMapDefault;
  }();
  return m;
}

int auto_block_songs(int width, int n_te, bool fused, int k, int n_tr) {
  long long cover = ((long long)width + 255) / 256 * 256;
  if (!fused && n_tr > kMaxLdsTrainUsers && k <= kMaxTopkLarge)
    return (int)std::max<long long>(256, std::min<long long>(kMaxBlockSongs, cover));
  const long long cap = k > 0 ? kMaxTopkTile : (fused ? 8192 : kMaxBlockSongs);
  const long long target = fused ? 256 : 1024;
  long long want = ((long long)width * std::max(1, n_te) + target - 1) / target;
  long long bs = ((want + 255) / 256) * 256;
  bs = std::max<long long>(256, std::min<long long>(cap, bs));
  return (int)std::max<long long>(256, std::min(bs, cover));
}

template <int MODEL>
void pick_kernels(mr_ctx* c) {
  const bool f64 = c->opt.out_dtype == MR_OUT_F64;
  if (c->fused)
    c->score_kernel[MODEL] = f64 ? k_score<MODEL, double, true> : k_score<MODEL, float, true>;
  else
    c->score_kernel[MODEL] = f64 ? k_score<MODEL, double, false> : k_score<MODEL, float, false>;
  if (c->shape == kShapeWide) {
    if (c->opt.topk == 10)
      c->score_kernel[MODEL] = f64 ? k_score_wide<MODEL, double, kWideThreads, 10, false>
                                   : k_score_wide<MODEL, float, kWideThreads, 10, false>;
    else
      c->score_kernel[MODEL] = f64 ? k_score_wide<MODEL, double, kWideThreads, kMaxTopkLarge, false>
                                   : k_score_wide<MODEL, float, kWideThreads, kMaxTopkLarge, false>;
    if constexpr (MODEL == MR_IBM) {
      if (c->cooc.route == 2 && c->cooc.cooc_nt == 512) {
        if (c->opt.topk == 10)
          c->cooc_kernel = f64 ? k_score_wide<MR_IBM, double, 512, 10, true> : k_score_wide<MR_IBM, float, 512, 10, true>;
        else
          c->cooc_kernel = f64 ? k_score_wide<MR_IBM, double, 512, kMaxTopkLarge, true>
                               : k_score_wide<MR_IBM, float, 512, kMaxTopkLarge, true>;
      } else if (c->cooc.route == 2) {
        if (c->opt.topk == 10)
          c->cooc_kernel = f64 ? k_score_wide<MR_IBM, double, kWideThreads, 10, true>
                               : k_score_wide<MR_IBM, float, kWideThreads, 10, true>;
        else
          c->cooc_kernel = f64 ? k_score_wide<MR_IBM, double, kWideThreads, kMaxTopkLarge, true>
                               : k_score_wide<MR_IBM, float, kWideThreads, kMaxTopkLarge, true>;
      }
    }
  }
  c->nbr_kernel[MODEL] = k_neighbours<MODEL>;
}

int pick_shape(const mr_options& o, int n_tr, int n_te) {
  const int k = o.topk;
  if (o.stage1 == 1) return kShapeFused;
  if (o.stage1 == 2) return kShapeSeparate;
  if (o.stage1 == 4) return kShapeWide;
  if (n_tr > kMaxFusedTrainUsers && k <= kMaxTopkLarge) return kShapeWide;
  if ((long long)n_te * n_tr >= kWideMinUserPairs && k <= kMaxTopkLarge) return kShapeWide;
  return n_tr <= kMaxFusedTrainUsers ? kShapeFused : kShapeSeparate;
}

int stage1_chunk_for(const mr_options& o, int n_tr) {
  return o.stage1_chunk > 0 ? std::min(o.stage1_chunk, std::max(1, n_tr))
         : n_tr <= kMaxLdsTrainUsers ? std::max(1, n_tr) : kStage1Chunk;
}

int wide_bmax(int k, int n_chunks) {
  int bmax = 256;
  while (bmax + 256 <= 65536 && wide_lds<kWideThreads>(bmax + 256, k, n_chunks).total <= kLdsBytes) bmax += 256;
  return bmax;
}

}

static int check_dataset(const mr_dataset* d, std::vector<int32_t>& col_tr) {
  mr_par::PhaseTrace trace("MR_LOAD_TRACE", "mr_load");
  const int n_tr = d->n_train_users, n_te = d->n_test_users, n_s = d->n_songs;
  if (n_tr < 0 || n_te <= 0 || n_s <= 0)
    return fail(MR_E_INVALID, "bad sizes: n_train_users=%d n_test_users=%d n_songs=%d", n_tr, n_te, n_s);
  if (n_tr > kMaxChunks * kStage1Chunk)
    return fail(MR_E_INVALID, "n_train_users=%d exceeds the stage-1 limit %d of this build", n_tr,
                kMaxChunks * kStage1Chunk);
  int rc;
  if ((rc = validate_csr("train user->songs", n_tr, n_s, d->tr_off, d->tr_songs))) return rc;
  if ((rc = validate_csr("test user->songs", n_te, n_s, d->te_off, d->te_songs))) return rc;
  if (!d->song_count || !d->tr_len || !d->te_len) return fail(MR_E_INVALID, "null count arrays");
  {
    const int64_t v = first_bad(n_tr, [&](int64_t v) {
      const int64_t deg = d->tr_off[v + 1] - d->tr_off[v];
      return deg <= 0 || d->tr_len[v] < deg;
    });
    if (v >= 0)
      return fail(MR_E_INVALID, "train user %d: %lld distinct songs but length %d", (int)v,
                  (long long)(d->tr_off[v + 1] - d->tr_off[v]), d->tr_len[v]);
    const int64_t u = first_bad(n_te, [&](int64_t u) {
      const int64_t deg = d->te_off[u + 1] - d->te_off[u];
      return deg <= 0 || d->te_len[u] < deg;
    });
    if (u >= 0)
      return fail(MR_E_INVALID, "test user %d: %lld distinct songs but length %d", (int)u,
                  (long long)(d->te_off[u + 1] - d->te_off[u]), d->te_len[u]);
  }
  const int64_t nnz_tr = d->tr_off[n_tr];
  const int W = (int)std::max<int64_t>(1, std::min<int64_t>(mr_par::usable_cores(), nnz_tr >> 18));
  col_tr.assign(n_s, 0);
  std::vector<int32_t> col_te(n_s, 0);
  {
    std::vector<std::vector<int32_t>> h(W);
    const std::vector<int64_t> cut = weighted_cuts(d->tr_off, n_tr, W);
    mr_par::parallel_for(W, [&](int64_t w0, int64_t w1, int) {
      for (int64_t w = w0; w < w1; ++w) {
        h[w].assign(n_s, 0);
        for (int64_t i = d->tr_off[cut[w]]; i < d->tr_off[cut[w + 1]]; ++i) h[w][d->tr_songs[i]]++;
      }
    }, 1, W);
    mr_par::parallel_for(n_s, [&](int64_t a, int64_t b, int) {
      for (int w = 0; w < W; ++w)
        for (int64_t s2 = a; s2 < b; ++s2) col_tr[s2] += h[w][s2];
    }, 4096);
  }
  for (int64_t i = 0; i < d->te_off[n_te]; ++i) col_te[d->te_songs[i]]++;
  {
    const int64_t s_bad = first_bad(n_s, [&](int64_t s2) {
      return d->song_count[s2] < col_tr[s2] + col_te[s2] || d->song_count[s2] <= 0;
    });
    if (s_bad >= 0)
      return fail(MR_E_INVALID, "song %d: count %d below its %d distinct listeners (or zero)", (int)s_bad,
                  d->song_count[s_bad], col_tr[s_bad] + col_te[s_bad]);
  }
  trace("validate");
  return MR_OK;
}

namespace {

struct TrainIndex {
  int W = 1;
  std::vector<int64_t> ucut;
  std::vector<int32_t> perm, len;
  std::vector<int64_t> off, trs_off;
  mr_par::buffer<int32_t> songs, trs_users;
};

void renumber_train(const mr_dataset* d, int train_order, TrainIndex& ti) {
  const int n_tr = d->n_train_users;
  ti.perm.resize(std::max(1, n_tr));
  if (train_order == 0 && n_tr > 0) {
    int64_t max_deg = 0;
    for (int v = 0; v < n_tr; ++v) max_deg = std::max(max_deg, d->tr_off[v + 1] - d->tr_off[v]);
    std::vector<int64_t> at((size_t)max_deg + 1, 0);
    for (int v = 0; v < n_tr; ++v) at[max_deg - (d->tr_off[v + 1] - d->tr_off[v])]++;
    int64_t run = 0;
    for (auto& x : at) { const int64_t n = x; x = run; run += n; }
    for (int v = 0; v < n_tr; ++v) ti.perm[at[max_deg - (d->tr_off[v + 1] - d->tr_off[v])]++] = v;
  } else {
    for (int v = 0; v < n_tr; ++v) ti.perm[v] = v;
  }
  ti.off.assign((size_t)n_tr + 1, 0);
  mr_par::parallel_for(n_tr, [&](int64_t a, int64_t b, int) {
    for (int64_t v = a; v < b; ++v) ti.off[v] = d->tr_off[ti.perm[v] + 1] - d->tr_off[ti.perm[v]];
  });
  ti.off[n_tr] = mr_par::exclusive_scan(ti.off.data(), (int64_t)n_tr);
  ti.songs.resize((size_t)std::max<int64_t>(1, d->tr_off[n_tr]));
  ti.len.resize(std::max(1, n_tr));
  mr_par::parallel_dynamic(n_tr, 2048, [&](int64_t v, int) {
    const int o = ti.perm[v];
    std::copy(d->tr_songs + d->tr_off[o], d->tr_songs + d->tr_off[o + 1], ti.songs.begin() + ti.off[v]);
    ti.len[v] = d->tr_len[o];
  });
}

void transpose_train(int n_tr, int n_s, TrainIndex& ti) {
  const int W = ti.W;
  ti.ucut = weighted_cuts(ti.off.data(), n_tr, W);
  const std::vector<int64_t>&tr_off = ti.off, &trs_off = ti.trs_off, &ucut = ti.ucut;
// ... 395 lines not shown
                 const TileCsr& tiles) {
  const int n_tr = d->n_train_users, n_te = d->n_test_users;
  const std::vector<int64_t>& trs_off = ti.trs_off;
  hipStream_t st = c->stream;
  int rc;
  std::vector<uint32_t> tpack(tiles.tsongs.size(), 0u);
  for (size_t t = 0; t < (size_t)lp.n_tiles; ++t)
    for (int v = 0; v < n_tr; ++v)
      for (int32_t i = tiles.toff[t * n_tr + v]; i < tiles.toff[t * n_tr + v + 1]; ++i)
        tpack[i] = ((uint32_t)v << 16) | tiles.tsongs[i];
  if ((rc = dev_upload(c->tpack, tpack.data(), tpack.size(), st))) return rc;
  const size_t nte = (size_t)d->te_off[n_te];
  std::vector<int2> rng(std::max<size_t>(1, nte));
  std::vector<long long> tq(std::max<size_t>(1, nte));
  for (size_t i = 0; i < nte; ++i) {
    const int s2 = d->te_songs[i];
    rng[i] = make_int2((int)trs_off[s2], (int)(trs_off[s2 + 1] - trs_off[s2]));
    tq[i] = sc.q_song[s2];
  }
  if ((rc = dev_upload(c->te_rng, rng.data(), rng.size(), st))) return rc;
  if ((rc = dev_upload(c->te_q, tq.data(), tq.size(), st))) return rc;
  std::vector<long long> h_sched_off((size_t)n_te + 1, 0);
  for (int u = 0; u < n_te; ++u) {
    long long n = 0;
    for (long long i = d->te_off[u]; i < d->te_off[u + 1]; ++i) n += rng[(size_t)i].y;
    h_sched_off[(size_t)u + 1] = h_sched_off[(size_t)u] + n;
  }
  const long long n_sched = h_sched_off[(size_t)n_te];
  if (fused_sched_opt() && n_sched <= (1ll << 26)) {
    std::vector<uint2> sched(std::max<long long>(1, n_sched));
    size_t o = 0;
    for (int u = 0; u < n_te; ++u)
      for (long long i = d->te_off[u]; i < d->te_off[u + 1]; ++i)
        for (int e = 0; e < rng[(size_t)i].y; ++e)
          sched[o++] = make_uint2((unsigned)(rng[(size_t)i].x + e), (unsigned)(i - d->te_off[u]));
    if ((rc = dev_upload(c->te_sched, sched.data(), sched.size(), st))) return rc;
    if ((rc = dev_upload(c->sched_off, h_sched_off.data(), h_sched_off.size(), st))) return rc;
  }
  return MR_OK;
}

int upload_cooc(mr_ctx* c, const CoocPlan& p, const TrainIndex& ti, const LaunchPlan& lp, int n_tr) {
  const int n_tiles = lp.n_tiles, lo = lp.lo;
  const std::vector<int64_t>& trs_off = ti.trs_off;
  hipStream_t st = c->stream;
  int rc;
  const size_t nr = p.row_song.size();
  if ((rc = dev_upload(c->row_song, p.row_song.data(), nr, st))) return rc;
  if ((rc = dev_upload(c->te_row, p.te_row.data(), p.te_row.size(), st))) return rc;
  if ((rc = dev_upload(c->row_base, reinterpret_cast<const long long*>(p.row_base.data()), nr + 1, st))) return rc;
  if ((rc = dev_alloc(c->row_nnz, nr))) return rc;
  if ((rc = dev_alloc(c->seg_off, nr * n_tiles))) return rc;
  if ((rc = dev_alloc(c->seg_len, nr * n_tiles))) return rc;
  if ((rc = dev_alloc(c->pool, (size_t)p.pool_cap))) return rc;
  const size_t n_heavy = p.heavy_rows.size();
  std::vector<int32_t> order(p.heavy_rows);
  order.insert(order.end(), p.light_rows.begin(), p.light_rows.end());
  if ((rc = dev_upload(c->rows_order, order.data(), order.size(), st))) return rc;
  {
    std::vector<int4> rd(std::max<size_t>(1, order.size()));
    int64_t at_lrec = 0, at_llrec = 0;
    for (size_t i = 0; i < order.size(); ++i) {
      const int32_t r = order[i], s2 = p.row_song[r];
      const int cnt = (int)(trs_off[s2 + 1] - trs_off[s2]);
      int z = (int)trs_off[s2];
      if (p.grp > 0 && (int)i >= p.n_heavy32 && i < n_heavy) {
        z = (int)at_lrec;
        at_lrec += cnt;
      } else if (i >= n_heavy) {
        z = (int)at_llrec;
        at_llrec += cnt;
      }
      rd[i] = make_int4(r, p.row_slots[r], z, cnt);
    }
    if ((rc = dev_upload(c->rdesc, rd.data(), rd.size(), st))) return rc;
    MR_HIP(hipStreamSynchronize(st));
  }
  if ((rc = dev_upload(c->row_slots, p.row_slots.data(), p.row_slots.size(), st))) return rc;
  if (p.light_rows.empty() && p.grp == 0) return MR_OK;
  std::vector<int64_t> so((size_t)n_tr + 1, 0);
  std::copy(p.shard_deg.begin(), p.shard_deg.begin() + n_tr, so.begin());
  so[n_tr] = mr_par::exclusive_scan(so.data(), (int64_t)n_tr);
  mr_par::buffer<uint32_t> ss((size_t)so[n_tr] + 4);
  std::fill(ss.begin() + so[n_tr], ss.end(), 0u);
  mr_par::parallel_for(n_tr, [&](int64_t a, int64_t b, int) {
    for (int64_t v = a; v < b; ++v) {
      const int32_t* r0 = std::lower_bound(ti.songs.data() + ti.off[v], ti.songs.data() + ti.off[v + 1], lo);
      for (int64_t i = 0; i < so[v + 1] - so[v]; ++i) ss[so[v] + i] = (uint32_t)(r0[i] - lo);
    }
  });
  if ((rc = dev_upload(c->sr_off, reinterpret_cast<const long long*>(so.data()), so.size(), st))) return rc;
  if ((rc = dev_upload(c->sr_songs, ss.data(), ss.size(), st))) return rc;
  if (!p.light_rows.empty()) {
    if ((rc = dev_alloc(c->llrec, (size_t)std::max<int64_t>(1, p.n_llrec)))) return rc;
    hipLaunchKernelGGL(k_llrec, dim3((unsigned)p.light_rows.size()), dim3(256), 0, st, c->rdesc.p + n_heavy,
                       c->row_song.p, c->trs_off.p, c->trs_users.p, c->sr_off.p, c->llrec.p);
    MR_HIP(hipGetLastError());
  }
  if (p.grp > 0) {
    if ((rc = dev_alloc(c->urec, (size_t)std::max(1, n_tr) * p.urec_words))) return rc;
    hipLaunchKernelGGL(k_urec, dim3((std::max(1, n_tr) + 255) / 256), dim3(256), 0, st, c->sr_off.p,
                       c->sr_songs.p, n_tr, n_tiles, lp.block_songs, p.urec_words, c->urec.p);
    MR_HIP(hipGetLastError());
    if ((rc = dev_alloc(c->lrec, (size_t)std::max<int64_t>(1, p.n_lrec) * p.lrec_words))) return rc;
    const int n16 = (int)n_heavy - p.n_heavy32;
    if (n16 > 0)
      hipLaunchKernelGGL(k_lrec, dim3(n16), dim3(256), 0, st, c->rdesc.p + p.n_heavy32, c->row_song.p,
                         c->trs_off.p, c->trs_users.p, c->urec.p, p.urec_words, n_tiles, p.grp, p.n_grp, p.lrec_words,
                         c->lrec.p);
    MR_HIP(hipGetLastError());
    MR_HIP(hipStreamSynchronize(st));
    c->urec.release();
  }
  MR_HIP(hipStreamSynchronize(st));
  return MR_OK;
}

int alloc_outputs(mr_ctx* c, const LaunchPlan& lp, int route, int n_te) {
  hipStream_t st = c->stream;
  const int k = lp.k;
  int rc;
  if (k > 0) {
    const int cand_users = !lp.wide() ? n_te : route == 2 ? std::max(lp.batch, std::min(n_te, kGridRowsXcd)) : lp.batch;
    const size_t nc = (size_t)cand_users * lp.n_tiles * k;
    if ((rc = dev_alloc(c->cand_key, nc))) return rc;
    if ((rc = dev_alloc(c->cand_song, nc))) return rc;
    const size_t nk = (size_t)n_te * k;
    if ((rc = dev_alloc(c->top_key, (size_t)topk_record_bytes(nk) / 8))) return rc;
    c->top_song.p = reinterpret_cast<int*>(c->top_key.p + nk);
    c->top_song.n = nk;
    c->top_song.own = false;
    if ((rc = dev_alloc(c->top_score, (size_t)n_te * k))) return rc;
    const size_t n_ctr = lp.wide() ? (size_t)n_te : (size_t)n_te * kCounterStride;
    if ((rc = dev_alloc(c->counter, n_ctr))) return rc;
    MR_HIP(hipMemsetAsync(c->counter.p, 0, n_ctr * sizeof(unsigned), st));
  }
  const size_t esz = c->opt.out_dtype == MR_OUT_F64 ? 8 : 4;
  if ((rc = dev_alloc(c->dense, c->opt.dense ? (size_t)n_te * lp.width * esz : 1))) return rc;
  if ((rc = dev_alloc(c->flag, 1))) return rc;
  return MR_OK;
}

int setup_kernels(mr_ctx* c, const LaunchPlan& lp, int n_tr) {
  const CoocPlan& p = c->cooc;
  const int bs = lp.block_songs, k = lp.k, n_chunks = lp.n_chunks;
  const bool fused = lp.fused(), wide = lp.wide();
  {
    const char* e = std::getenv("MR_WIDE_CAND");
    const int nt = p.route == 2 ? p.cooc_nt : kWideThreads;
    c->cand_on = wide && !c->opt.dense && k >= 1 && k <= nt / 16 && !c->opt.topk_lists && bs <= kCandE * nt &&
                 !(e && e[0] == '0');
  }
  c->wide_lds = wide ? (size_t)wide_lds<kWideThreads>(bs, k, n_chunks).total : 0;
  pick_kernels<MR_UBM>(c);
  pick_kernels<MR_IBM>(c);
  c->score_lds = wide ? c->wide_lds
                      : (size_t)score_lds(bs, fused ? n_tr : 0, k, lp.n_tiles, fused ? 0 : n_chunks).total;
  if (c->score_lds > 160 * 1024)
    return fail(MR_E_INVALID, "scoring kernel needs %zu B of LDS (> 160 KiB): lower block_songs or topk",
                c->score_lds);
  c->nbr_lds = (size_t)align16(lp.chunk * 8) + kThreads * 16 + (kThreads + 4 + kWaves) * 4;
  for (int m = 0; m < 2; ++m) {
    MR_HIP(hipFuncSetAttribute((const void*)c->score_kernel[m], hipFuncAttributeMaxDynamicSharedMemorySize,
                               (int)c->score_lds));
    MR_HIP(hipFuncSetAttribute((const void*)c->nbr_kernel[m], hipFuncAttributeMaxDynamicSharedMemorySize,
                               (int)c->nbr_lds));
  }
  if (p.route == 2) {
    const WideLds<kWideThreads> WL = p.cooc_nt == 512 ? wide_lds<512>(bs, k, n_chunks).as_wide()
                                                      : wide_lds<kWideThreads>(bs, k, n_chunks);
    c->cooc_score_lds = (size_t)WL.total;
    c->nseg = std::min(std::min(p.cooc_nt, (WL.total - WL.wk - 8) / 40), 255);
    if (c->nseg < 16) return fail(MR_E_INVALID, "co-listening route: no LDS for row descriptors");
    c->cooc_lds = (size_t)cooc_build_lds<false>(bs);
    if (p.grp > 0)
      MR_HIP(hipFuncSetAttribute(p.group_nt == 512 ? (const void*)k_cooc_group<512> : (const void*)k_cooc_group<1024>,
                                 hipFuncAttributeMaxDynamicSharedMemorySize, cooc_group_lds(bs, p.grp)));
    for (int t = 0; t < kLightTiers; ++t)
      if (int rc2 = light_tier_call(t, nullptr, 0, nullptr, CoocParams{})) return rc2;
    MR_HIP(hipFuncSetAttribute((const void*)c->cooc_kernel, hipFuncAttributeMaxDynamicSharedMemorySize,
                               (int)c->cooc_score_lds));
    MR_HIP(hipFuncSetAttribute((const void*)k_cooc_build<MR_COOC_NT, false>, hipFuncAttributeMaxDynamicSharedMemorySize,
                               (int)c->cooc_lds));
    MR_HIP(hipFuncSetAttribute((const void*)k_cooc_build<MR_COOC_NT16, true>, hipFuncAttributeMaxDynamicSharedMemorySize,
                               cooc_build_lds<true>(bs)));
  }
  if (wide && k > 0) {
    c->merge_lds = (size_t)merge_lds_bytes(k);
    MR_HIP(hipFuncSetAttribute((const void*)k_topk_merge, hipFuncAttributeMaxDynamicSharedMemorySize,
                               (int)c->merge_lds));
  }
  return MR_OK;
}

}


extern "C" {

const char* mr_last_error(void) { return g_err.c_str(); }
const char* mr_version(void) { return "mr_engine 0.2 (gfx950)"; }

int mr_options_default(mr_options* opt) {
  if (!opt) return fail(MR_E_INVALID, "null options");
  std::memset(opt, 0, sizeof *opt);
  opt->device = 0;
  opt->frac_bits = 32;
  opt->song_lo = 0;
  opt->song_hi = 0;
  opt->block_songs = 0;
  opt->out_dtype = MR_OUT_F32;
  opt->topk = 10;
  opt->dense = 1;
  opt->time_kernels = 0;
  opt->stage1 = 0;
  return MR_OK;
}

int mr_create(const mr_options* opt, mr_ctx** out) {
  if (!out) return fail(MR_E_INVALID, "null output pointer");
  *out = nullptr;
  mr_options o;
  if (opt) o = *opt; else mr_options_default(&o);
  if (o.frac_bits < 8 || o.frac_bits > 40) return fail(MR_E_INVALID, "frac_bits %d outside [8,40]", o.frac_bits);
  if (o.topk < 0 || o.topk > kMaxTopK) return fail(MR_E_INVALID, "topk %d outside [0,%d]", o.topk, kMaxTopK);
  if (o.out_dtype != MR_OUT_F32 && o.out_dtype != MR_OUT_F64) return fail(MR_E_INVALID, "bad out_dtype %d", o.out_dtype);
  if (o.block_songs < 0 || o.block_songs > (o.stage1 == 4 ? kMaxWideBlockSongs : kMaxBlockSongs) ||
      (o.block_songs % 256) != 0)
    return fail(MR_E_INVALID, "block_songs %d must be a multiple of 256 in [0,%d]", o.block_songs,
                o.stage1 == 4 ? kMaxWideBlockSongs : kMaxBlockSongs);
  if (o.stage1 < 0 || o.stage1 > 4 || o.stage1 == 3)
    return fail(MR_E_INVALID, "stage1 %d is not 0 (auto), 1 (fused), 2 (separate) or 4 (wide)", o.stage1);
  if (o.topk_lists != 0 && o.topk_lists != 1) return fail(MR_E_INVALID, "topk_lists %d not 0 or 1", o.topk_lists);
  if (o.ibm_route < 0 || o.ibm_route > 2)
    return fail(MR_E_INVALID, "ibm_route %d is not 0 (auto), 1 (two-hop) or 2 (co-listening index)", o.ibm_route);
  if (!o.dense && o.topk == 0) return fail(MR_E_INVALID, "dense=0 and topk=0: nothing to compute");
  if (o.stage1_chunk < 0 || o.stage1_chunk > kMaxLdsTrainUsers)
    return fail(MR_E_INVALID, "stage1_chunk %d outside [0,%d]", o.stage1_chunk, kMaxLdsTrainUsers);
  int ndev = 0;
  MR_HIP(hipGetDeviceCount(&ndev));
  if (o.device < 0 || o.device >= ndev) return fail(MR_E_INVALID, "device %d not present (%d devices)", o.device, ndev);
  MR_HIP(hipSetDevice(o.device));
  mr_ctx* c = new mr_ctx();
  c->opt = o;
  hipError_t e = hipStreamCreateWithFlags(&c->stream, hipStreamNonBlocking);
  if (e != hipSuccess) {
    delete c;
    return fail(MR_E_HIP, "hipStreamCreate: %s", hipGetErrorString(e));
  }
  for (int i = 0; i < 2 && e == hipSuccess; ++i) e = hipStreamCreateWithFlags(&c->side[i], hipStreamNonBlocking);
  if (e == hipSuccess) e = hipEventCreateWithFlags(&c->side_fork, hipEventDisableTiming);
  for (int i = 0; i < 2 && e == hipSuccess; ++i) e = hipEventCreateWithFlags(&c->side_join[i], hipEventDisableTiming);
  if (e != hipSuccess) {
    mr_destroy(c);
    return fail(MR_E_HIP, "side streams: %s", hipGetErrorString(e));
  }
  for (auto& ev : c->win) {
    e = hipEventCreate(&ev);
    if (e != hipSuccess) {
      ev = nullptr;
      mr_destroy(c);
      return fail(MR_E_HIP, "hipEventCreate: %s", hipGetErrorString(e));
    }
  }
  if (o.time_kernels) {
    c->ring.resize((size_t)mr_ctx::kRing * 3);
    for (auto& ev : c->ring) {
      e = hipEventCreate(&ev);
      if (e != hipSuccess) {
        ev = nullptr;
        mr_destroy(c);
        return fail(MR_E_HIP, "hipEventCreate: %s", hipGetErrorString(e));
      }
    }
  }
  *out = c;
  return MR_OK;
}

int mr_destroy(mr_ctx* c) {
  if (!c) return MR_OK;
  (void)hipSetDevice(c->opt.device);
  if (c->stream) (void)hipStreamSynchronize(c->stream);
  c->release_data();
  for (int i = 0; i < 2; ++i) {
    if (c->stage_ev[i]) (void)hipEventDestroy(c->stage_ev[i]);
  }
  for (auto& ev : c->ring) if (ev) (void)hipEventDestroy(ev);
  for (auto& ev : c->win) if (ev) (void)hipEventDestroy(ev);
  for (int i = 0; i < 2; ++i) {
    if (c->side[i]) { (void)hipStreamSynchronize(c->side[i]); (void)hipStreamDestroy(c->side[i]); }
    if (c->side_join[i]) (void)hipEventDestroy(c->side_join[i]);
  }
  if (c->side_fork) (void)hipEventDestroy(c->side_fork);
  if (c->stream) (void)hipStreamDestroy(c->stream);
  delete c;
  return MR_OK;
}

void* mr_stream(const mr_ctx* c) { return c ? (void*)c->stream : nullptr; }

int mr_load(mr_ctx* c, const mr_dataset* d) {
  if (!c || !d) return fail(MR_E_INVALID, "null argument");
  mr_par::PhaseTrace trace("MR_LOAD_TRACE", "mr_load");
  MR_HIP(hipSetDevice(c->opt.device));
  MR_HIP(hipStreamSynchronize(c->stream));
  c->ring_used = 0;
  c->release_data();
  const int n_tr = d->n_train_users, n_te = d->n_test_users, n_s = d->n_songs;
  std::vector<int32_t> col_tr;
// ... 5 lines not shown
  if ((rc = plan_launch(c->opt, n_tr, n_te, n_s, free_b, c->dev_share, lp))) return rc;

  TrainIndex ti;
  ti.W = (int)std::max<int64_t>(1, std::min<int64_t>(mr_par::usable_cores(), d->tr_off[n_tr] >> 18));
  ti.trs_off.assign((size_t)n_s + 1, 0);
  for (int s2 = 0; s2 < n_s; ++s2) ti.trs_off[s2 + 1] = ti.trs_off[s2] + col_tr[s2];
  trace("counts");
  renumber_train(d, c->opt.train_order, ti);
  trace("renumber");
  transpose_train(n_tr, n_s, ti);
  trace("transpose");
  const ScaleTables scales = make_scales(d, ti, c->opt.frac_bits);
  TileCsr tiles;
  build_tiles(ti, lp, n_tr, tiles);
  trace("tiles");
  CoocPlan plan;
  const char* why = nullptr;
  if ((rc = plan_cooc(CoocIn{d, c->opt, ti, lp, col_tr}, free_b, c->dev_share, &plan, &why))) return rc;
  if (c->opt.ibm_route == 2 && why)
    return fail(MR_E_INVALID, "ibm_route 2 (co-listening index) needs %s", why);
  trace("route");

  if ((rc = upload_base(c, d, ti, lp, scales, tiles))) return rc;
  if (lp.fused() && (rc = upload_fused(c, d, ti, lp, scales, tiles))) return rc;
  if (plan.route == 2 && (rc = upload_cooc(c, plan, ti, lp, n_tr))) return rc;
  if ((rc = alloc_outputs(c, lp, plan.route, n_te))) return rc;
  c->fused = lp.fused();
  c->shape = lp.shape;
  c->cooc = std::move(plan);
  if ((rc = setup_kernels(c, lp, n_tr))) return rc;
#ifdef MR_STAMPS
  const size_t stamp_users = (size_t)std::max(lp.batch, c->cooc.route == 2 ? std::min(n_te, kGridRowsXcd) : 0) + 8;
  const size_t build_wgs = (size_t)c->cooc.n_heavy() * lp.n_tiles + 64 * (size_t)std::max(1, lp.n_tiles);
  c->bstamp_off = (size_t)lp.n_tiles * stamp_users * kStampSlots;
  c->lstamp_off = c->bstamp_off + build_wgs * 8;
  const size_t n_stamps = c->lstamp_off + (size_t)c->cooc.n_light() * 8;
  if ((rc = dev_alloc(c->stamps, n_stamps))) return rc;
  MR_HIP(hipMemsetAsync(c->stamps.p, 0, n_stamps * 8, c->stream));
#endif
  MR_HIP(hipStreamSynchronize(c->stream));
  trace("upload");

  c->n_tr = n_tr; c->n_te = n_te; c->n_s = n_s;
  c->song_lo = lp.lo; c->song_hi = lp.hi; c->width = lp.width;
  c->block_songs = lp.block_songs; c->n_tiles = lp.n_tiles;
  c->cap = lp.cap; c->batch = lp.batch;
  c->chunk = lp.chunk; c->n_chunks = lp.n_chunks;
  c->song_count.assign(d->song_count, d->song_count + n_s);
  c->te_len_h.assign(d->te_len, d->te_len + n_te);
  c->tr_len_h.assign(ti.len.begin(), ti.len.begin() + n_tr);
  c->max_ctr = col_tr.empty() ? 0 : *std::max_element(col_tr.begin(), col_tr.end());
  c->loaded = true;
  c->ran = false;
  return MR_OK;
}

int mr_route_info(const mr_ctx* c, int32_t* route, int32_t* n_rows, int64_t* pool_entries) {
  if (!c) return fail(MR_E_INVALID, "null context");
  if (!c->loaded) return fail(MR_E_STATE, "mr_route_info before mr_load");
  if (route) *route = c->cooc.route;
  if (n_rows) *n_rows = c->cooc.n_rows();
  if (pool_entries) *pool_entries = c->cooc.pool_cap;
  return MR_OK;
}

int mr_topk_mode(const mr_ctx* c, int32_t* candidate_only) {
  if (!c || !candidate_only) return fail(MR_E_INVALID, "null argument");
  if (!c->loaded) return fail(MR_E_STATE, "mr_topk_mode before mr_load");
  *candidate_only = c->cand_on ? 1 : 0;
  return MR_OK;
}

int mr_cooc_stats(mr_ctx* c, int64_t* index_nnz, int64_t* consumed, int64_t* build_reads) {
  if (!c) return fail(MR_E_INVALID, "null context");
  if (!c->loaded || c->cooc.route != 2) return fail(MR_E_STATE, "mr_cooc_stats needs a context on ibm_route 2");
  if (!c->cooc_ran) return fail(MR_E_STATE, "mr_cooc_stats before an ibm run");
  MR_HIP(hipSetDevice(c->opt.device));
  std::vector<unsigned> nnz((size_t)std::max(1, c->cooc.n_rows()), 0u);
  if (c->cooc.n_rows() > 0)
    MR_HIP(hipMemcpyAsync(nnz.data(), c->row_nnz.p, (size_t)c->cooc.n_rows() * 4, hipMemcpyDeviceToHost, c->stream));
  MR_HIP(hipStreamSynchronize(c->stream));
  int64_t tot = 0, use = 0;
  for (int r = 0; r < c->cooc.n_rows(); ++r) {
    tot += nnz[r];
    use += (int64_t)nnz[r] * c->cooc.row_users[r];
  }
  if (index_nnz) *index_nnz = tot;
  if (consumed) *consumed = use;
  if (build_reads) *build_reads = c->cooc.build_reads;
  return MR_OK;
}

int mr_cooc_bytes(mr_ctx* c, mr_cooc_bytes_t* out) {
  if (!c || !out) return fail(MR_E_INVALID, "null argument");
  if (!c->loaded || c->cooc.route != 2) return fail(MR_E_STATE, "mr_cooc_bytes needs a context on ibm_route 2");
  if (!c->cooc_ran) return fail(MR_E_STATE, "mr_cooc_bytes before an ibm run");
  MR_HIP(hipSetDevice(c->opt.device));
  const CoocPlan& p = c->cooc;
  const int nr = p.n_rows(), nt = c->n_tiles;
  std::vector<int32_t> len((size_t)std::max(1, nr) * nt, 0);
  if (nr > 0)
    MR_HIP(hipMemcpyAsync(len.data(), c->seg_len.p, (size_t)nr * nt * 4, hipMemcpyDeviceToHost, c->stream));
  MR_HIP(hipStreamSynchronize(c->stream));
  mr_cooc_bytes_t b{};
  for (int r = 0; r < nr; ++r) {
    int64_t seg = 0;
    int64_t sp = 0, ds = 0;
    for (int t = 0; t < nt; ++t) {
      const int blo = c->song_lo + t * c->block_songs;
      const int64_t bw = std::min(c->song_hi, blo + c->block_songs) - blo;
      const int32_t l = len[(size_t)t * nr + r];
      seg += l >= 0 ? std::min<int64_t>(4 * (int64_t)l, bw) : bw;
      if (l >= 0) sp += l;
      else { ds += bw; sp += kCoocDenseTail - l; }
    }
    b.index_sparse_entries += sp;
    b.index_dense_songs += ds;
    b.consumed_sparse_entries += sp * p.row_users[r];
    b.consumed_dense_songs += ds * p.row_users[r];
    if (p.row_light[r]) {
      b.light_rows++;
      b.light_reads += p.row_reads[r];
      b.light_index_bytes += seg;
    } else {
      b.heavy_rows++;
      b.heavy_reads += p.row_reads[r];
      b.heavy_index_bytes += seg;
      const bool u32row = is_u32_row(c->cooc, p.row_listeners[r]);
      b.heavy_visits += (int64_t)p.row_listeners[r] * (p.grp > 0 && !u32row ? p.n_grp : nt);
    }
    b.consumed_bytes += seg * p.row_users[r];
  }
  b.group_tiles = p.grp;
  b.n_groups = p.grp > 0 ? p.n_grp : nt;
  *out = b;
  return MR_OK;
}

int mr_shard_info(const mr_ctx* c, int32_t* lo, int32_t* hi, int32_t* n_te) {
  if (!c) return fail(MR_E_INVALID, "null context");
  if (!c->loaded) return fail(MR_E_STATE, "mr_shard_info before mr_load");
  if (lo) *lo = c->song_lo;
  if (hi) *hi = c->song_hi;
  if (n_te) *n_te = c->n_te;
  return MR_OK;
}

int mr_launch_info(const mr_ctx* c, int32_t* fused, int32_t* block_songs, int32_t* n_tiles) {
  if (!c) return fail(MR_E_INVALID, "null context");
  if (!c->loaded) return fail(MR_E_STATE, "mr_launch_info before mr_load");
  if (fused) *fused = c->shape;
  if (block_songs) *block_songs = c->block_songs;
  if (n_tiles) *n_tiles = c->n_tiles;
  return MR_OK;
}

int mr_batch_info(const mr_ctx* c, int32_t* batch, int32_t* chunk, int32_t* n_chunks) {
  if (!c) return fail(MR_E_INVALID, "null context");
  if (!c->loaded) return fail(MR_E_STATE, "mr_batch_info before mr_load");
  if (batch) *batch = c->batch;
  if (chunk) *chunk = c->chunk;
  if (n_chunks) *n_chunks = c->n_chunks;
  return MR_OK;
}

int mr_shard_tile_songs(const mr_options* opt, int32_t n_train_users, int32_t n_test_users, int32_t* tile_songs) {
  if (!tile_songs) return fail(MR_E_INVALID, "null output pointer");
  mr_options o;
  if (opt) o = *opt; else mr_options_default(&o);
  if (n_train_users < 0 || n_test_users <= 0)
    return fail(MR_E_INVALID, "bad sizes: n_train_users=%d n_test_users=%d", n_train_users, n_test_users);
  *tile_songs = 0;
  if (pick_shape(o, n_train_users, n_test_users) != kShapeWide || o.topk > kMaxTopkLarge) return MR_OK;
  const int chunk = stage1_chunk_for(o, n_train_users);
  const int n_chunks = (std::max(1, n_train_users) + chunk - 1) / chunk;
  *tile_songs = o.block_songs > 0 ? o.block_songs : wide_bmax(o.topk, n_chunks);
  return MR_OK;
}

int mr_shard_tile_songs_n(const mr_options* opt, int32_t n_train_users, int32_t n_test_users, int32_t n_songs,
                          int32_t n_shards, int32_t* tile_songs) {
  if (n_songs <= 0 || n_shards < 1) return fail(MR_E_INVALID, "bad sizes: n_songs=%d n_shards=%d", n_songs, n_shards);
  int rc = mr_shard_tile_songs(opt, n_train_users, n_test_users, tile_songs);
  if (rc || *tile_songs == 0 || n_shards == 1 || (opt && opt->block_songs > 0)) return rc;
  const long long t0 = ((long long)n_songs + *tile_songs - 1) / *tile_songs;
  const long long t = (t0 + n_shards - 1) / n_shards * n_shards;
  *tile_songs = (int32_t)((((long long)n_songs + t - 1) / t + 255) / 256 * 256);
  return MR_OK;
}

}

namespace {

int flush_timing(mr_ctx* c) {
  if (c->ring_used == 0) return MR_OK;
  MR_HIP(hipEventSynchronize(c->ring[(size_t)(c->ring_used - 1) * 3 + 2]));
  for (int i = 0; i < c->ring_used; ++i) {
    hipEvent_t* e = &c->ring[(size_t)i * 3];
    float t;
    if (c->ring_has_stage1[i]) { MR_HIP(hipEventElapsedTime(&t, e[0], e[1])); c->ms[0] += t; c->launches[0]++; }
    MR_HIP(hipEventElapsedTime(&t, e[1], e[2])); c->ms[1] += t; c->launches[1]++;
  }
  c->ring_used = 0;
  return MR_OK;
}

int run_cooc(mr_ctx* c) {
  hipStream_t st = c->stream;
  const CoocPlan& p = c->cooc;
  const bool timed = c->opt.time_kernels != 0;
  const int k = c->opt.topk;
  hipEvent_t* ev = nullptr;
  if (timed) {
    if (c->ring_used == mr_ctx::kRing) {
      int rc = flush_timing(c);
      if (rc) return rc;
    }
    ev = &c->ring[(size_t)c->ring_used * 3];
    c->ring_has_stage1[c->ring_used] = true;
    c->ring_used++;
    MR_HIP(hipEventRecord(ev[0], st));
  }
  if (p.n_rows() > 0) {
    MR_HIP(hipMemsetAsync(c->row_nnz.p, 0, (size_t)p.n_rows() * sizeof(unsigned), st));
    const bool side = c->side[0] && p.n_light() > 0 && cooc_side_opt();
    if (side) {
      MR_HIP(hipEventRecord(c->side_fork, st));
      for (int i = 0; i < 2; ++i) MR_HIP(hipStreamWaitEvent(c->side[i], c->side_fork, 0));
    }
    CoocParams cp{c->n_tr, p.n_rows(), c->n_tiles, c->block_songs, c->song_lo, c->song_hi, c->toff.p, c->tsongs.p,
                  c->trs_off.p, c->trs_users.p, c->row_song.p, c->row_base.p, c->pool.p,
                  c->seg_off.p, c->seg_len.p, c->rows_order.p, c->sr_off.p, c->sr_songs.p, c->row_slots.p,
                  p.dense_div, p.force32, 255u, c->stamps.p ? c->stamps.p + c->bstamp_off : nullptr,
                  c->row_nnz.p};
    cp.sat = p.sat;
    const int n32 = p.n_heavy32, n16 = p.n_heavy() - p.n_heavy32;
    if (n32 > 0) {
      CoocParams hp = cp;
      hp.n_big = n32;
      hp.tcap = p.tcap32;
      hipLaunchKernelGGL((k_cooc_build<MR_COOC_NT, false>), dim3(n32 * c->n_tiles), dim3(MR_COOC_NT), c->cooc_lds, st,
                         hp);
      MR_HIP(hipGetLastError());
    }
    if (n16 > 0 && p.grp > 0) {
      CoocParams hp = cp;
      hp.rows = c->rows_order.p + n32;
      hp.n_big = p.n_big16;
      hp.tcap = p.tcap16;
      hp.lrec = c->lrec.p;
      hp.lrec_words = p.lrec_words;
      hp.grp = p.grp;
      hp.n_grp = p.n_grp;
      hp.rdesc = c->rdesc.p + n32;
      if (hp.stamps) hp.stamps += (size_t)n32 * c->n_tiles * 8;
      const int nblk = (p.n_big16 + 7) / 8 * 8 * p.n_grp + (n16 - p.n_big16);
      const size_t glds = (size_t)cooc_group_lds(c->block_songs, p.grp);
      if (p.group_nt == 512)
        hipLaunchKernelGGL(k_cooc_group<512>, dim3(nblk), dim3(512), glds, st, hp);
      else
        hipLaunchKernelGGL(k_cooc_group<1024>, dim3(nblk), dim3(1024), glds, st, hp);
      MR_HIP(hipGetLastError());
    } else if (n16 > 0) {
      CoocParams hp = cp;
      hp.rows = c->rows_order.p + n32;
      hp.n_big = p.n_big16;
      hp.tcap = p.tcap16;
      if (hp.stamps) hp.stamps += (size_t)n32 * c->n_tiles * 8;
      hipLaunchKernelGGL((k_cooc_build<MR_COOC_NT16, true>), dim3(p.n_big16 * c->n_tiles + n16 - p.n_big16),
                         dim3(MR_COOC_NT16),
                         (size_t)cooc_build_lds<true>(c->block_songs), st, hp);
      MR_HIP(hipGetLastError());
    }
    int lr = p.n_heavy();
    for (int t = 0; t < kLightTiers; ++t) {
      if (p.n_light_tier[t] == 0) continue;
      CoocParams lp = cp;
      lp.rows = c->rows_order.p + lr;
      lp.rdesc = c->rdesc.p + lr;
      lp.llrec = reinterpret_cast<const unsigned*>(c->llrec.p);
      lp.lstamps = c->stamps.p ? c->stamps.p + c->lstamp_off + (size_t)(lr - p.n_heavy()) * 8 : nullptr;
      hipStream_t ls = side ? c->side[t < 2 ? 0 : 1] : st;
      if (int rc2 = light_tier_call(t, ls, p.n_light_tier[t], &lp, lp)) return rc2;
      lr += p.n_light_tier[t];
    }
    if (side)
      for (int i = 0; i < 2; ++i) {
        MR_HIP(hipEventRecord(c->side_join[i], c->side[i]));
        MR_HIP(hipStreamWaitEvent(st, c->side_join[i], 0));
      }
  }
  if (timed) MR_HIP(hipEventRecord(ev[1], st));
  const int rows = mr_internal::launch_rows(kGridRowsXcd);
  for (int y0 = 0; y0 < c->n_te; y0 += rows) {
    const int ny = std::min(rows, c->n_te - y0);
    const int remap = wide_map_opt();
    ScoreParams sp{};
    sp.chunk = c->chunk; sp.n_chunks = c->n_chunks;
    sp.n_users = ny; sp.xcd_remap = remap;
    sp.merge_rows = merge_rows_opt();
    sp.n_tr = c->n_tr;
    sp.user0 = y0;
    sp.song_lo = c->song_lo; sp.song_hi = c->song_hi; sp.width = c->width;
    sp.block_songs = c->block_songs; sp.n_tiles = c->n_tiles;
    sp.frac_bits = c->opt.frac_bits; sp.topk = k; sp.dense = c->opt.dense;
    sp.te_off = c->te_off.p; sp.te_songs = c->te_songs.p;
    sp.sqrt_c = c->sqrt_c.p; sp.q_song = c->q_song.p;
    sp.n_rows = p.n_rows(); sp.nseg = c->nseg;
    sp.te_row = c->te_row.p; sp.seg_off = c->seg_off.p; sp.seg_len = c->seg_len.p; sp.pool = c->pool.p;
    sp.dense_out = c->dense_override ? c->dense_override : (void*)c->dense.p;
    sp.cand_key = c->cand_key.p; sp.cand_song = c->cand_song.p; sp.counter = c->counter.p;
    sp.top_key = c->top_key.p; sp.top_song = c->top_song.p; sp.top_score = c->top_score.p;
    sp.stamps = y0 == 0 ? c->stamps.p : nullptr;
    sp.topk_lists = c->opt.topk_lists;
    if (c->mm_on) { sp.mm_key = c->mm_key.p; sp.mm_n = c->n_te; }
    sp.cand = c->cand_on && !sp.mm_key; sp.rsq_c = c->rsq_c.p;
    hipLaunchKernelGGL(c->cooc_kernel, dim3(c->n_tiles, (ny + 7) / 8 * 8), dim3(p.cooc_nt), c->cooc_score_lds, st, sp);
    MR_HIP(hipGetLastError());
    if (k > 0 && c->n_tiles > 1) {
      MergeParams mp{c->n_tiles, k, k, (long long)c->n_tiles * k, (long long)k, (long long)k, c->cand_key.p,
                     c->cand_song.p, c->top_key.p + (size_t)y0 * k, c->top_song.p + (size_t)y0 * k,
                     c->top_score.p + (size_t)y0 * k};
      hipLaunchKernelGGL(k_topk_merge, dim3(ny), dim3(kThreads), c->merge_lds, st, mp);
      MR_HIP(hipGetLastError());
    }
    if (c->win_open) c->win_launches++;
  }
  if (timed) MR_HIP(hipEventRecord(ev[2], st));
  return MR_OK;
}

int ensure_nbr(mr_ctx* c) {
  if (c->shape == kShapeFused || (c->nbr_v.p && c->nbr_q.p && c->nbr_cnt.p)) return MR_OK;
  int rc;
  if ((rc = dev_alloc(c->nbr_v, (size_t)c->batch * c->cap))) return rc;
  if ((rc = dev_alloc(c->nbr_q, (size_t)c->batch * c->cap))) return rc;
  if ((rc = dev_alloc(c->nbr_cnt, (size_t)c->batch * c->n_chunks))) return rc;
  return MR_OK;
}

int run_model(mr_ctx* c, int model) {
  if (model == MR_IBM && c->cooc.route == 2) {
    c->cooc_ran = true;
    return run_cooc(c);
  }
  hipStream_t st = c->stream;
  const bool timed = c->opt.time_kernels != 0;
  const int k = c->opt.topk;
  const int rows1 = mr_internal::launch_rows(kGridRows);
  const int rows = mr_internal::launch_rows(kGridRowsXcd);
  for (int user0 = 0; user0 < c->n_te; user0 += c->batch) {
    const int nb = std::min(c->batch, c->n_te - user0);
    hipEvent_t* ev = nullptr;
    if (timed) {
      if (c->ring_used == mr_ctx::kRing) {
        int rc = flush_timing(c);
        if (rc) return rc;
      }
      ev = &c->ring[(size_t)c->ring_used * 3];
      c->ring_has_stage1[c->ring_used] = c->shape != kShapeFused;
      c->ring_used++;
      MR_HIP(hipEventRecord(ev[0], st));
    }
    if (c->shape == kShapeSeparate || c->shape == kShapeWide) {
      if (!c->nbr_v.p || !c->nbr_q.p || !c->nbr_cnt.p) {
        if (int rc0 = ensure_nbr(c)) return rc0;
      }
      NbrParams np{c->n_tr, user0, c->cap, c->opt.frac_bits, c->chunk, c->n_chunks, c->te_off.p, c->te_songs.p,
                   c->trs_off.p, c->trs_users.p, c->q_song.p, c->sqrt_tr.p, c->sqrt_te.p, c->nbr_v.p, c->nbr_q.p,
                   c->nbr_cnt.p, c->n_chunks > 1 ? c->sbound.p : nullptr};
      for (int y0 = 0; y0 < nb; y0 += rows1) {
        NbrParams q = np;
        q.user0 = user0 + y0;
        q.nbr_v += (size_t)y0 * c->cap;
        q.nbr_q += (size_t)y0 * c->cap;
        q.nbr_cnt += (size_t)y0 * c->n_chunks;
        hipLaunchKernelGGL(c->nbr_kernel[model], dim3(c->n_chunks, std::min(rows1, nb - y0)), dim3(kThreads),
                           c->nbr_lds, st, q);
      }
      MR_HIP(hipGetLastError());
    }
    if (timed) MR_HIP(hipEventRecord(ev[1], st));
    for (int y0 = 0; y0 < nb; y0 += rows) {
      const int ny = std::min(rows, nb - y0);
      const bool wide = c->shape == kShapeWide;
      int remap = (c->shape == kShapeSeparate && c->n_tiles > 1) || wide;
      if (wide) remap = wide_map_opt();
      const int gy = remap ? (ny + 7) / 8 * 8 : ny;
      ScoreParams sp{};
      sp.chunk = c->chunk; sp.n_chunks = c->n_chunks;
      sp.n_users = ny; sp.xcd_remap = remap;
      sp.merge_rows = merge_rows_opt();
      sp.n_tr = c->n_tr;
      sp.user0 = user0 + y0;
      sp.song_lo = c->song_lo; sp.song_hi = c->song_hi; sp.width = c->width;
      sp.block_songs = c->block_songs; sp.n_tiles = c->n_tiles;
      sp.frac_bits = c->opt.frac_bits; sp.topk = k; sp.dense = c->opt.dense;
      sp.te_off = c->te_off.p; sp.te_songs = c->te_songs.p;
      sp.toff = c->toff.p; sp.tsongs = c->tsongs.p; sp.tpack = c->tpack.p; sp.sqrt_c = c->sqrt_c.p;
      sp.te_rng = c->te_rng.p; sp.te_q = c->te_q.p;
      sp.te_sched = c->te_sched.p; sp.sched_off = c->sched_off.p;
#ifdef MR_NO_TERNG
      sp.te_rng = nullptr;
#endif
      sp.trs_off = c->trs_off.p; sp.trs_users = c->trs_users.p; sp.q_song = c->q_song.p;
      sp.sqrt_tr = c->sqrt_tr.p; sp.sqrt_te = c->sqrt_te.p;
      sp.cap = c->cap;
      sp.nbr_v = c->fused ? nullptr : c->nbr_v.p + (size_t)y0 * c->cap;
      sp.nbr_q = c->fused ? nullptr : c->nbr_q.p + (size_t)y0 * c->cap;
      sp.nbr_cnt = c->fused ? nullptr : c->nbr_cnt.p + (size_t)y0 * c->n_chunks;
      sp.dense_out = c->dense_override ? c->dense_override : (void*)c->dense.p;
      sp.cand_key = c->cand_key.p; sp.cand_song = c->cand_song.p; sp.counter = c->counter.p;
      sp.top_key = c->top_key.p; sp.top_song = c->top_song.p; sp.top_score = c->top_score.p;
      sp.stamps = c->stamps.p ? c->stamps.p + (size_t)y0 * c->n_tiles * kStampSlots : nullptr;
      sp.topk_lists = c->opt.topk_lists;
      if (c->mm_on && wide) { sp.mm_key = c->mm_key.p; sp.mm_n = c->n_te; }
      sp.cand = wide && c->cand_on && !sp.mm_key; sp.rsq_c = c->rsq_c.p;
      hipLaunchKernelGGL(c->score_kernel[model], dim3(c->n_tiles, gy), dim3(wide ? kWideThreads : kThreads),
                         c->score_lds, st, sp);
      MR_HIP(hipGetLastError());
      if (wide && k > 0 && c->n_tiles > 1) {
        MergeParams mp{c->n_tiles, k, k, (long long)c->n_tiles * k, (long long)k, (long long)k, c->cand_key.p, c->cand_song.p,
                       c->top_key.p + (size_t)(user0 + y0) * k, c->top_song.p + (size_t)(user0 + y0) * k,
                       c->top_score.p + (size_t)(user0 + y0) * k};
        hipLaunchKernelGGL(k_topk_merge, dim3(ny), dim3(kThreads), c->merge_lds, st, mp);
        MR_HIP(hipGetLastError());
      }
      if (c->win_open) c->win_launches++;
    }
    if (timed) MR_HIP(hipEventRecord(ev[2], st));
  }
  return MR_OK;
}

}

namespace mr_internal {

namespace {
struct StagePool {
  std::mutex m;
  void* buf[2] = {nullptr, nullptr};
};
StagePool& stage_pool() {
  static StagePool* p = new StagePool;
  return *p;
}
}

int d2h_staged(mr_ctx* c, void* dst, size_t dpitch, const void* src, size_t spitch, size_t row_bytes, size_t rows) {
  const size_t total = row_bytes * rows;
  if (total == 0) return MR_OK;
  hipPointerAttribute_t attr;
  const bool pinned = hipPointerGetAttributes(&attr, dst) == hipSuccess && attr.type == hipMemoryTypeHost;
  (void)hipGetLastError();
  constexpr size_t kStage = (size_t)64 << 20;
  if (pinned || total < ((size_t)8 << 20) || row_bytes > kStage) {
    MR_HIP(hipMemcpy2DAsync(dst, dpitch, src, spitch, row_bytes, rows, hipMemcpyDeviceToHost, c->stream));
    MR_HIP(hipStreamSynchronize(c->stream));
    return MR_OK;
  }
  StagePool& pool = stage_pool();
  std::lock_guard<std::mutex> lock(pool.m);
  for (int i = 0; i < 2; ++i) {
    if (!pool.buf[i]) MR_HIP(hipHostMalloc(&pool.buf[i], kStage, hipHostMallocPortable));
    if (!c->stage_ev[i]) MR_HIP(hipEventCreateWithFlags(&c->stage_ev[i], hipEventDisableTiming));
  }
  const size_t per = kStage / row_bytes;
  const size_t n_chunks = (rows + per - 1) / per;
  auto enqueue = [&](size_t k) -> int {
    const size_t r0 = k * per, nr = std::min(per, rows - r0);
    MR_HIP(hipMemcpy2DAsync(pool.buf[k & 1], row_bytes, static_cast<const char*>(src) + r0 * spitch, spitch,
                            row_bytes, nr, hipMemcpyDeviceToHost, c->stream));
    MR_HIP(hipEventRecord(c->stage_ev[k & 1], c->stream));
    return MR_OK;
  };
  int rc = enqueue(0);
  if (!rc && n_chunks > 1) rc = enqueue(1);
  if (rc) return rc;
  for (size_t k = 0; k < n_chunks; ++k) {
    MR_HIP(hipEventSynchronize(c->stage_ev[k & 1]));
    const size_t r0 = k * per, nr = std::min(per, rows - r0);
    const char* from = static_cast<const char*>(pool.buf[k & 1]);
    char* to = static_cast<char*>(dst) + r0 * dpitch;
    if (dpitch == row_bytes) {
      mr_par::parallel_for((int64_t)(nr * row_bytes), [&](int64_t a, int64_t b, int) {
        std::memcpy(to + a, from + a, (size_t)(b - a));
      }, (int64_t)4 << 20);
    } else {
      mr_par::parallel_for((int64_t)nr, [&](int64_t a, int64_t b, int) {
        for (int64_t r = a; r < b; ++r) std::memcpy(to + r * dpitch, from + r * row_bytes, row_bytes);
      }, std::max<int64_t>(1, ((int64_t)4 << 20) / (int64_t)row_bytes));
    }
    if (k + 2 < n_chunks && (rc = enqueue(k + 2))) return rc;
  }
  return MR_OK;
}

namespace {
int launch_merge(mr_ctx* c, int32_t n_shards, int32_t n_te, int32_t k, const MergeParams& mp) {
  const int lds = merge_lds_bytes(k);
  if (lds > 160 * 1024) return fail(MR_E_INVALID, "merge of %d lists x %d needs too much LDS", n_shards, k);
  MR_HIP(hipFuncSetAttribute((const void*)k_topk_merge, hipFuncAttributeMaxDynamicSharedMemorySize, lds));
  const int rows = launch_rows(kGridRows);
  for (int y0 = 0; y0 < n_te; y0 += rows) {
    MergeParams q = mp;
    q.keys += (size_t)y0 * k;
    q.songs += (size_t)y0 * k;
    q.out_keys += (size_t)y0 * k;
    q.out_songs += (size_t)y0 * k;
    if (q.out_scores) q.out_scores += (size_t)y0 * k;
    hipLaunchKernelGGL(k_topk_merge, dim3(std::min(rows, n_te - y0)), dim3(kThreads), lds, c->stream, q);
  }
  MR_HIP(hipGetLastError());
  return MR_OK;
}
}

int merge_async(mr_ctx* c, int32_t n_shards, int32_t n_te, int32_t k, const int32_t* songs_in,
                const int64_t* keys_in, int32_t* songs_out, int64_t* keys_out, double* scores_out) {
  if (!c || !songs_in || !keys_in || !songs_out || !keys_out) return fail(MR_E_INVALID, "null argument");
  if (n_shards <= 0 || n_te <= 0 || k <= 0 || k > kMaxTopK) return fail(MR_E_INVALID, "bad merge shape");
  MR_HIP(hipSetDevice(c->opt.device));
  MergeParams mp{n_shards, k, k, k, (long long)n_te * k, (long long)n_te * k, reinterpret_cast<const long long*>(keys_in),
                 songs_in, reinterpret_cast<long long*>(keys_out), songs_out, scores_out};
  return launch_merge(c, n_shards, n_te, k, mp);
}

int merge_records_async(mr_ctx* c, int32_t n_shards, int32_t n_te, int32_t k, const void* records, int64_t rec_bytes,
                        int32_t* songs_out, int64_t* keys_out, double* scores_out) {
  if (!c || !records || !songs_out || !keys_out) return fail(MR_E_INVALID, "null argument");
  if (n_shards <= 0 || n_te <= 0 || k <= 0 || k > kMaxTopK) return fail(MR_E_INVALID, "bad merge shape");
  const size_t nk = (size_t)n_te * k;
  if (rec_bytes < (int64_t)(12 * nk) || rec_bytes % 8)
    return fail(MR_E_INVALID, "record blocks of %lld B cannot hold %zu keys + songs (multiple of 8 B needed)",
                (long long)rec_bytes, nk);
  MR_HIP(hipSetDevice(c->opt.device));
  const char* base = static_cast<const char*>(records);
  MergeParams mp{n_shards, k, k, k, rec_bytes / 8, rec_bytes / 4, reinterpret_cast<const long long*>(base),
                 reinterpret_cast<const int*>(base + 8 * nk), reinterpret_cast<long long*>(keys_out), songs_out,
                 scores_out};
  return launch_merge(c, n_shards, n_te, k, mp);
}

int topk_records(mr_ctx* c, void** records, int64_t* rec_bytes) {
  if (!c || !records || !rec_bytes) return fail(MR_E_INVALID, "null argument");
  if (!c->loaded || c->opt.topk <= 0) return fail(MR_E_STATE, "no top-k lists (not loaded or topk = 0)");
  *records = c->top_key.p;
  *rec_bytes = topk_record_bytes((size_t)c->n_te * c->opt.topk);
  return MR_OK;
}

int set_error(int code, const char* msg) { return fail(code, "%s", msg); }

int launch_rows(int production_max) {
  const char* e = std::getenv("MR_LAUNCH_ROWS");
  const int n = e ? std::atoi(e) : 0;
  return n >= 8 ? std::min(production_max, n / 8 * 8) : production_max;
}

int shard_tables(mr_ctx* c, const char* what, ShardTables* out) {
  if (!c || !out) return fail(MR_E_INVALID, "null argument");
  if (!c->loaded) return fail(MR_E_STATE, "%s before mr_load", what);
  ShardTables& t = *out;
  t.n_tr = c->n_tr; t.n_te = c->n_te; t.n_s = c->n_s;
  t.song_lo = c->song_lo; t.song_hi = c->song_hi; t.block_songs = c->block_songs; t.n_tiles = c->n_tiles;
  t.device = c->opt.device;
  t.f64 = c->opt.out_dtype == MR_OUT_F64;
  t.frac_bits = c->opt.frac_bits;
  t.max_ctr = c->max_ctr;
  t.stream = c->stream;
  t.trs_off = c->trs_off.p; t.trs_users = c->trs_users.p;
// ... 320 lines not shown
```

### musicrecommendation_amd/engine.py

```python
from __future__ import annotations

import ctypes
from typing import Optional, Tuple, Union

import numpy as np

from . import _lib
from .dataset import Dataset

MODELS = {"ubm": _lib.MR_UBM, "ibm": _lib.MR_IBM, _lib.MR_UBM: _lib.MR_UBM, _lib.MR_IBM: _lib.MR_IBM}
KERNELS = {"neighbours": 0, "score": 1}
IBM_ROUTES = {"auto": 0, "two_hop": 1, "cooc": 2}


def model_id(model: Union[str, int]) -> int:
    try:
        return MODELS[model]
    except KeyError:
        raise ValueError(f"unknown model {model!r}: use 'ubm' or 'ibm'") from None


class Engine:
    def __init__(self, dataset: Dataset, *, device: int = 0, frac_bits: int = 32, song_lo: int = 0,
                 song_hi: int = 0, block_songs: int = 0, out_dtype: str = "f32", topk: int = 10,
                 dense: bool = True, time_kernels: bool = False, stage1: str = "auto",
                 stage1_chunk: int = 0, train_order: str = "auto", topk_lists: bool = False,
                 ibm_route: str = "auto"):
        self._L = _lib.lib()
        opt = _lib.MrOptions()
        _lib.check(self._L.mr_options_default(ctypes.byref(opt)), "mr_options_default")
        opt.device = device
        opt.frac_bits = frac_bits
        opt.song_lo = song_lo
        opt.song_hi = song_hi
        opt.block_songs = block_songs
        opt.out_dtype = {"f32": _lib.MR_OUT_F32, "f64": _lib.MR_OUT_F64}[out_dtype]
        opt.topk = topk
        opt.dense = 1 if dense else 0
        opt.time_kernels = 1 if time_kernels else 0
        opt.stage1 = _lib.STAGE1[stage1]
        opt.stage1_chunk = stage1_chunk
        opt.train_order = {"auto": 0, "given": 1}[train_order]
        opt.topk_lists = 1 if topk_lists else 0
        opt.ibm_route = IBM_ROUTES[ibm_route]
        self.opt = opt
        self.dtype = np.float32 if out_dtype == "f32" else np.float64
        self._h = ctypes.c_void_p()
        _lib.check(self._L.mr_create(ctypes.byref(opt), ctypes.byref(self._h)), "mr_create")
        self.dataset = dataset
        try:
            cd = dataset.c_struct()
            _lib.check(self._L.mr_load(self._h, ctypes.byref(cd)), "mr_load")
        except Exception:
            self.close()
            raise
        lo, hi, nte = ctypes.c_int32(), ctypes.c_int32(), ctypes.c_int32()
        _lib.check(self._L.mr_shard_info(self._h, ctypes.byref(lo), ctypes.byref(hi), ctypes.byref(nte)),
                   "mr_shard_info")
        self.song_lo, self.song_hi, self.n_test = lo.value, hi.value, nte.value
        self.width = self.song_hi - self.song_lo
        self.topk_k = topk
        fz, bsz, nt = ctypes.c_int32(), ctypes.c_int32(), ctypes.c_int32()
        _lib.check(self._L.mr_launch_info(self._h, ctypes.byref(fz), ctypes.byref(bsz), ctypes.byref(nt)),
                   "mr_launch_info")
        self.shape = _lib.SHAPES[fz.value]
        self.fused, self.block_songs, self.n_tiles = self.shape == "fused", bsz.value, nt.value
        b, ch, nch = ctypes.c_int32(), ctypes.c_int32(), ctypes.c_int32()
        _lib.check(self._L.mr_batch_info(self._h, ctypes.byref(b), ctypes.byref(ch), ctypes.byref(nch)),
                   "mr_batch_info")
        self.batch, self.stage1_chunk, self.n_chunks = b.value, ch.value, nch.value
        rt, nr, pe = ctypes.c_int32(), ctypes.c_int32(), ctypes.c_int64()
        _lib.check(self._L.mr_route_info(self._h, ctypes.byref(rt), ctypes.byref(nr), ctypes.byref(pe)),
                   "mr_route_info")
        self.ibm_route = {1: "two_hop", 2: "cooc"}[rt.value]
        self.cooc_rows, self.cooc_pool_entries = nr.value, pe.value
        co = ctypes.c_int32()
        _lib.check(self._L.mr_topk_mode(self._h, ctypes.byref(co)), "mr_topk_mode")
        self.candidate_topk = bool(co.value)

    def close(self) -> None:
        if getattr(self, "_h", None) is not None and self._h.value:
            self._L.mr_destroy(self._h)
            self._h = ctypes.c_void_p()

    def __enter__(self):
        return self

    def __exit__(self, *exc):
        self.close()

    def __del__(self):
        try:
            self.close()
        except Exception:
            pass

    def run(self, model: Union[str, int]) -> None:
        _lib.check(self._L.mr_run(self._h, model_id(model)), "mr_run")

    def cooc_stats(self) -> Tuple[int, int, int]:
        a, b, c = ctypes.c_int64(), ctypes.c_int64(), ctypes.c_int64()
        _lib.check(self._L.mr_cooc_stats(self._h, ctypes.byref(a), ctypes.byref(b), ctypes.byref(c)), "mr_cooc_stats")
        return a.value, b.value, c.value

    def cooc_bytes(self) -> dict:
        b = _lib.MrCoocBytes()
        _lib.check(self._L.mr_cooc_bytes(self._h, ctypes.byref(b)), "mr_cooc_bytes")
        return {name: int(getattr(b, name)) for name, _t in _lib.MrCoocBytes._fields_}

    def sync(self) -> None:
        _lib.check(self._L.mr_sync(self._h), "mr_sync")

    def graph_capture(self, model: Union[str, int], n_steps: int) -> None:
        _lib.check(self._L.mr_graph_capture(self._h, model_id(model), int(n_steps)), "mr_graph_capture")

    def graph_launch(self) -> None:
        _lib.check(self._L.mr_graph_launch(self._h), "mr_graph_launch")

    @property
    def stream(self) -> int:
        return self._L.mr_stream(self._h) or 0

    def dense(self) -> np.ndarray:
        out = np.empty((self.n_test, self.width), dtype=self.dtype)
        _lib.check(self._L.mr_copy_dense(self._h, out.ctypes.data_as(ctypes.c_void_p)), "mr_copy_dense")
        return out

    def topk(self) -> Tuple[np.ndarray, np.ndarray, np.ndarray]:
        k = self.topk_k
        songs = np.empty((self.n_test, k), dtype=np.int32)
        scores = np.empty((self.n_test, k), dtype=np.float64)
        keys = np.empty((self.n_test, k), dtype=np.int64)
        _lib.check(self._L.mr_copy_topk(self._h, songs.ctypes.data_as(ctypes.c_void_p),
                                        scores.ctypes.data_as(ctypes.c_void_p),
                                        keys.ctypes.data_as(ctypes.c_void_p)), "mr_copy_topk")
        return songs, scores, keys

    def copy_topk_device(self, songs_ptr: int, keys_ptr: int, wait: bool = True) -> None:
        fn = self._L.mr_copy_topk_device if wait else self._L.mr_copy_topk_device_async
        _lib.check(fn(self._h, songs_ptr, keys_ptr), "mr_copy_topk_device")

    def score_dense(self, model: Union[str, int]) -> np.ndarray:
        self.run(model)
        return self.dense()

    def device_outputs(self) -> Tuple[int, int, int, int]:
        ptrs = [ctypes.c_void_p() for _ in range(4)]
        _lib.check(self._L.mr_device_outputs(self._h, *[ctypes.byref(p) for p in ptrs]), "mr_device_outputs")
        return tuple(p.value or 0 for p in ptrs)

    def merge_topk_device(self, n_shards: int, songs_ptr: int, keys_ptr: int, out_songs_ptr: int,
                          out_keys_ptr: int, out_scores_ptr: int = 0, wait: bool = True) -> None:
        if wait:
            rc = self._L.mr_topk_merge_device(self._h, n_shards, self.n_test, self.topk_k, songs_ptr, keys_ptr,
                                              None, out_songs_ptr, out_keys_ptr, out_scores_ptr or None)
        else:
            rc = self._L.mr_topk_merge_device_async(self._h, n_shards, self.n_test, self.topk_k, songs_ptr,
                                                    keys_ptr, out_songs_ptr, out_keys_ptr, out_scores_ptr or None)
        _lib.check(rc, "mr_topk_merge_device")

    def record_bytes(self) -> int:
        b = ctypes.c_int64()
        _lib.check(self._L.mr_topk_record_bytes(self.n_test, self.topk_k, ctypes.byref(b)), "mr_topk_record_bytes")
        return b.value

    def copy_topk_record(self, record_ptr: int, wait: bool = False) -> None:
        n = self.n_test * self.topk_k
        self.copy_topk_device(record_ptr + 8 * n, record_ptr, wait=wait)

    def merge_topk_records(self, n_shards: int, records_ptr: int, rec_bytes: int, out_songs_ptr: int,
                           out_keys_ptr: int, out_scores_ptr: int = 0) -> None:
        _lib.check(self._L.mr_topk_merge_records_async(self._h, n_shards, self.n_test, self.topk_k, records_ptr,
                                                       rec_bytes, out_songs_ptr, out_keys_ptr, out_scores_ptr or None),
                   "mr_topk_merge_records_async")

    def run_into(self, model: Union[str, int], dense_ptr: int) -> None:
        _lib.check(self._L.mr_run_into(self._h, model_id(model), ctypes.c_void_p(dense_ptr)), "mr_run_into")

    def topk_dense(self, dense_ptr: int) -> None:
        _lib.check(self._L.mr_topk_dense_device(self._h, ctypes.c_void_p(dense_ptr), self.topk_k),
                   "mr_topk_dense_device")

    def combine(self, kind: int, param: float, ubm_ptr: int, ibm_ptr: int, out_ptr: int, *, seed: int = 0,
                pair_base: int = 0, n_pairs: int = 0) -> None:
        _lib.check(self._L.mr_combine_device(self._h, kind, float(param), int(seed) & (2 ** 64 - 1), int(pair_base),
                                             int(n_pairs), ctypes.c_void_p(ubm_ptr), ctypes.c_void_p(ibm_ptr),
                                             ctypes.c_void_p(out_ptr)), "mr_combine_device")

    def combine_all(self, alpha: float, ibm_percentage: float, ibm_probability: float, ubm_ptr: int, ibm_ptr: int,
                    out_ptrs: Tuple[int, int, int], *, seed: int = 0, pair_base: int = 0,
                    n_pairs: int = 0) -> Tuple[Tuple[float, float], Tuple[float, float], Tuple[float, float]]:
        mm = (ctypes.c_double * 6)()
        _lib.check(self._L.mr_combine_all_device(self._h, float(alpha), float(ibm_percentage), float(ibm_probability),
                                                 int(seed) & (2 ** 64 - 1), int(pair_base), int(n_pairs),
                                                 ctypes.c_void_p(ubm_ptr), ctypes.c_void_p(ibm_ptr),
                                                 *(ctypes.c_void_p(x) for x in out_ptrs), mm),
                   "mr_combine_all_device")
        return (mm[0], mm[1]), (mm[2], mm[3]), (mm[4], mm[5])

    def dense_minmax(self) -> Optional[Tuple[float, float]]:
        mn, mx = ctypes.c_double(), ctypes.c_double()
        if self._L.mr_dense_minmax(self._h, ctypes.byref(mn), ctypes.byref(mx)) != 0:
            return None
        return mn.value, mx.value

    def eval_minmax(self, dense_ptr: int) -> Tuple[float, float]:
        mn, mx = ctypes.c_double(), ctypes.c_double()
        _lib.check(self._L.mr_eval_minmax_device(self._h, ctypes.c_void_p(dense_ptr), ctypes.byref(mn),
                                                 ctypes.byref(mx)), "mr_eval_minmax_device")
        return mn.value, mx.value

    def eval_counts(self, dense_ptr: int, mn: float, mx: float, lab_off: np.ndarray,
                    lab_songs: np.ndarray, pred: Optional[np.ndarray] = None,
                    tp: Optional[np.ndarray] = None, n_thresholds: int = 10) -> Tuple[np.ndarray, np.ndarray]:
        lab_off = np.ascontiguousarray(lab_off, dtype=np.int64)
        lab_songs = np.ascontiguousarray(lab_songs, dtype=np.int32)
        shape = (self.width, n_thresholds)
        for a in (pred, tp):
            if a is not None and (a.dtype != np.int32 or a.shape != shape or not a.flags.c_contiguous):
# ... 202 lines not shown
```

Baseline: 16.97 billion.

## Template fused score kernel on workgroup size and add lean top-k variant

Makes the fused scoring kernel a template over its workgroup size (256/512/1024 threads). Wide tiles (block_songs > 512) now launch 512-thread workgroups, and the LDS layout, scans, neighbour walk and top-k helpers are all sized to match. It also adds a LEAN variant that fixes the merge to 32 rows and marks the staged-merge fallback as cold when the config allows, moving that merge loop into a separate helper. The aim is more parallelism per tile and less branching and register pressure in the merge path, at the cost of more template instantiations and a risk of lower occupancy with larger workgroups.

```diff
diff --git a/include/mr_engine.h b/include/mr_engine.h
--- a/include/mr_engine.h
+++ b/include/mr_engine.h
@@ -67,6 +67,8 @@
 int mr_shard_info(const mr_ctx* ctx, int32_t* song_lo, int32_t* song_hi, int32_t* n_test_users);
 
 int mr_launch_info(const mr_ctx* ctx, int32_t* shape, int32_t* block_songs, int32_t* n_tiles);
+
+int mr_fused_info(const mr_ctx* ctx, int32_t* threads, int32_t* lean);
 
 int mr_batch_info(const mr_ctx* ctx, int32_t* batch, int32_t* chunk, int32_t* n_chunks);
 
diff --git a/musicrecommendation_amd/_lib.py b/musicrecommendation_amd/_lib.py
--- a/musicrecommendation_amd/_lib.py
+++ b/musicrecommendation_amd/_lib.py
@@ -123,6 +123,7 @@
     "mr_load": (c_int, [c_void_p, POINTER(MrDataset)]),
     "mr_shard_info": (c_int, [c_void_p, POINTER(c_int32), POINTER(c_int32), POINTER(c_int32)]),
     "mr_launch_info": (c_int, [c_void_p, POINTER(c_int32), POINTER(c_int32), POINTER(c_int32)]),
+    "mr_fused_info": (c_int, [c_void_p, POINTER(c_int32), POINTER(c_int32)]),
     "mr_batch_info": (c_int, [c_void_p, POINTER(c_int32), POINTER(c_int32), POINTER(c_int32)]),
     "mr_route_info": (c_int, [c_void_p, POINTER(c_int32), POINTER(c_int32), POINTER(c_int64)]),
     "mr_topk_mode": (c_int, [c_void_p, POINTER(c_int32)]),
diff --git a/musicrecommendation_amd/csrc/mr_engine.hip b/musicrecommendation_amd/csrc/mr_engine.hip
--- a/musicrecommendation_amd/csrc/mr_engine.hip
+++ b/musicrecommendation_amd/csrc/mr_engine.hip
@@ -84,7 +84,9 @@
 __host__ __device__ inline int align16(int x) { return (x + 15) & ~15; }
 __host__ __device__ inline int merge_lists_per_pass(int k);
 
-__host__ __device__ inline ScoreLds score_lds(int bs, int fused_ntr, int k, int n_tiles, int n_chunks = 0) {
+__host__ __device__ inline ScoreLds score_lds(int bs, int fused_ntr, int k, int n_tiles, int n_chunks = 0,
+                                              int nt = kThreads) {
+  const int nw = nt / 64;
   ScoreLds L;
   const int fused = fused_ntr > 0 ? 1 : 0;
   const int kk = k > 0 ? k : 1;
@@ -92,22 +94,22 @@
   L.stage_lists = (k > 0 && n_tiles > 1) ? (n_tiles < per ? n_tiles : per) : 0;
   int a_bytes = bs * 8 + fused_ntr * 8;
   const int st_bytes = L.stage_lists * kk * 8 + align16(L.stage_lists * kk * 4);
-  const int wide_bytes = (k > 0 && bs > kMaxTopkTile) ? kThreads * kk * 8 + kThreads * kk * 4 : 0;
+  const int wide_bytes = (k > 0 && bs > kMaxTopkTile) ? 256 * kk * 8 + 256 * kk * 4 : 0;
   if (wide_bytes > a_bytes) a_bytes = wide_bytes;
   int o = 0;
   L.acc = o; L.y = bs * 8; o = align16(a_bytes > st_bytes ? a_bytes : st_bytes);
   L.heard = o; o = align16(o + (bs / 32) * 4);
-  L.s_lo = o; o += fused * kThreads * 8;
-  L.s_w = o; o += fused * kThreads * 8;
-  L.s_pre = o; o = align16(o + (kThreads + 1) * 4);
-  L.s_scan = o; o = align16(o + kWaves * 4);
-  L.wk = o; o = align16(o + kWaves * kMaxTopK * 8);
-  L.ws = o; o = align16(o + kWaves * kMaxTopK * 4);
+  L.s_lo = o; o += fused * nt * 8;
+  L.s_w = o; o += fused * nt * 8;
+  L.s_pre = o; o = align16(o + (nt + 1) * 4);
+  L.s_scan = o; o = align16(o + nw * 4);
+  L.wk = o; o = align16(o + nw * kMaxTopK * 8);
+  L.ws = o; o = align16(o + nw * kMaxTopK * 4);
   L.fk = o; o = align16(o + kMaxTopK * 8);
   L.fs = o; o = align16(o + kMaxTopK * 4);
   L.flag = o; o = align16(o + 16);
   L.cpre = o; o = align16(o + (n_chunks > 0 ? (n_chunks + 1) * 4 : 0));
-  L.stg = o; o = align16(o + (n_chunks > 0 ? kWaves * kStgBytes : 0));
+  L.stg = o; o = align16(o + (n_chunks > 0 ? nw * kStgBytes : 0));
   L.gm = o; o = align16(o + kTopkScratch256);
   L.total = o;
   return L;
@@ -177,6 +179,7 @@
   return x;
 }
 
+template <int NT = kThreads>
 __device__ __forceinline__ int block_excl_scan(int x, int* total, int* sbuf) {
   const int lane = threadIdx.x & 63, w = threadIdx.x >> 6;
   const int incl = wave_incl_scan(x);
@@ -184,7 +187,7 @@
   __syncthreads();
   int off = 0, tot = 0;
 #pragma unroll
-  for (int i = 0; i < kWaves; ++i) {
+  for (int i = 0; i < NT / 64; ++i) {
     int s = sbuf[i];
     off += (i < w) ? s : 0;
     tot += s;
@@ -366,7 +369,7 @@
   for (int i = r + lane; i < k; i += 64) { out_k[i] = kKeyNone; out_s[i] = -1; }
 }
 
-template <typename Get>
+template <int NT = kThreads, typename Get>
 __device__ __forceinline__ void block_topk(int n, int k, Get get, long long* wk, int* ws, long long* out_k,
                                            int* out_s) {
   const int w = threadIdx.x >> 6, lane = threadIdx.x & 63;
@@ -387,14 +390,14 @@
   }
 #pragma unroll
   for (int j = 0; j < 4; ++j) {
-    const int i = w * 64 + lane + kThreads * j;
+    const int i = w * 64 + lane + NT * j;
     rk[j] = kKeyNone;
     rs[j] = INT_MAX;
     if (i < n) get(i, rk[j], rs[j]);
   }
   wave_topk_regs<4>(rk, rs, k, wk + w * k, ws + w * k);
   __syncthreads();
-  if (w == 0) wave_merge_lists(kWaves, k, wk, ws, out_k, out_s);
+  if (w == 0) wave_merge_lists(NT / 64, k, wk, ws, out_k, out_s);
   __syncthreads();
 }
 
@@ -419,7 +422,8 @@
   thr = nt;
 }
 
-template <typename Get>
+constexpr int kWideLists = 256;
+template <int NT = kThreads, typename Get>
 __device__ __forceinline__ void block_topk_wide(int n, int k, Get get, long long* lk, int* ls, long long* wk,
                                                 int* ws, long long* out_k, int* out_s) {
   const int tid = threadIdx.x, w = tid >> 6;
@@ -428,20 +432,24 @@
 #pragma unroll
   for (int t = 0; t < kMaxTopkLarge; ++t) { tk[t] = kKeyNone; ts[t] = INT_MAX; }
   long long thr = kKeyNone;
-  for (int i = tid; i < n; i += kThreads) {
-    long long key;
-    int song;
-    get(i, key, song);
-    if (key > thr) lane_list_insert(tk, ts, k, key, song, thr);
-  }
+  const bool lister = NT == kWideLists || tid < kWideLists;
+  if (lister)
+    for (int i = tid; i < n; i += kWideLists) {
+      long long key;
+      int song;
+      get(i, key, song);
+      if (key > thr) lane_list_insert(tk, ts, k, key, song, thr);
+    }
   __syncthreads();
-#pragma unroll
-  for (int t = 0; t < kMaxTopkLarge; ++t)
-    if (t < k) { lk[tid * k + t] = tk[t]; ls[tid * k + t] = tk[t] >= 0 ? ts[t] : -1; }
+  if (lister) {
+#pragma unroll
+    for (int t = 0; t < kMaxTopkLarge; ++t)
+      if (t < k) { lk[tid * k + t] = tk[t]; ls[tid * k + t] = tk[t] >= 0 ? ts[t] : -1; }
+  }
   __syncthreads();
-  wave_merge_lists(64, k, lk + (size_t)w * 64 * k, ls + (size_t)w * 64 * k, wk + w * k, ws + w * k);
+  if (lister) wave_merge_lists(64, k, lk + (size_t)w * 64 * k, ls + (size_t)w * 64 * k, wk + w * k, ws + w * k);
   __syncthreads();
-  if (w == 0) wave_merge_lists(kWaves, k, wk, ws, out_k, out_s);
+  if (w == 0) wave_merge_lists(kWideLists / 64, k, wk, ws, out_k, out_s);
   __syncthreads();
 }
 
@@ -510,11 +518,12 @@
 template <int NT>
 constexpr int kRankU = NT <= 256 ? MR_RANK_UNROLL_FUSED : 1;
 
-template <int NT>
+template <int NT, bool FR = false, bool COLD = false>
 __device__ __forceinline__ void rank_survivors(int nc, int k, const long long* ck, const int* cs, int* crank,
                                                long long* out_k, int* out_s, const TopkDst& dst = TopkDst{}) {
   const int tid = threadIdx.x, lane = tid & 63;
-  if (nc * nc > kRankQ<NT> * NT) {
+  const bool one_wave = FR ? nc * nc > kRankQ<256> * 256 : nc * nc > kRankQ<NT> * NT;
+  if (COLD ? __builtin_expect(one_wave, 0) : one_wave) {
     if (tid < 64) {
       long long rk[4];
       int rs[4];
@@ -541,7 +550,7 @@
       int c = 0;
       const int je = min(nc, j0 + per);
       int j = j0;
-      constexpr int U = kRankU<NT>;
+      constexpr int U = FR ? kRankU<256> : kRankU<NT>;
       if constexpr (U > 1) {
         for (; j + U <= je; j += U) {
           long long o[U];
@@ -625,8 +634,8 @@
   if (tau_k < 0) { tau_k = 0; tau_s = INT_MAX; }
 }
 
-template <int NT, typename Get, int NG = NT / 16>
-__device__ __forceinline__ bool block_topk_threshold(int n, int k, Get get, long long mk, int ms, unsigned char* gm,
+template <int NT, typename Get, int NG, bool FR, bool COLD>
+__device__ __forceinline__ bool block_topk_threshold_as(int n, int k, Get get, long long mk, int ms, unsigned char* gm,
                                                      long long* ck, int* cs, int cap, long long* out_k, int* out_s,
                                                      long long* sb = nullptr, const TopkDst& dst = TopkDst{}) {
   long long* gk = reinterpret_cast<long long*>(gm);
@@ -652,8 +661,14 @@
   stamp_at(sb, 11);
   const int nc = *counter;
   if (nc > cap) return false;
-  rank_survivors<NT>(nc, k, ck, cs, crank, out_k, out_s, dst);
+  rank_survivors<NT, FR, COLD>(nc, k, ck, cs, crank, out_k, out_s, dst);
   return true;
+}
+template <int NT, typename Get, int NG = NT / 16>
+__device__ __forceinline__ bool block_topk_threshold(int n, int k, Get get, long long mk, int ms, unsigned char* gm,
+                                                     long long* ck, int* cs, int cap, long long* out_k, int* out_s,
+                                                     long long* sb = nullptr, const TopkDst& dst = TopkDst{}) {
+  return block_topk_threshold_as<NT, Get, NG, false, false>(n, k, get, mk, ms, gm, ck, cs, cap, out_k, out_s, sb, dst);
 }
 
 constexpr int kMergeStageBytes = 32 * 1024;
@@ -705,7 +720,7 @@
   return lo;
 }
 
-template <int MODEL, typename Add, typename Mark>
+template <int MODEL, int NT = kThreads, typename Add, typename Mark>
 __device__ __forceinline__ void walk_neighbours(long long t0, long long t1, const int* te_songs,
                                                 const long long* trs_off, const int* trs_users,
                                                 const long long* q_song, long long* s_lo, long long* s_w,
@@ -714,8 +729,8 @@
                                                 int chunk_idx = 0, int nc1 = 0, const int2* te_rng = nullptr,
                                                 const long long* te_q = nullptr, long long* sb = nullptr) {
   const int tid = threadIdx.x;
-  for (long long base = t0; base < t1; base += kThreads) {
-    const int n = (int)min((long long)kThreads, t1 - base);
+  for (long long base = t0; base < t1; base += NT) {
+    const int n = (int)min((long long)NT, t1 - base);
     int len = 0;
     if (tid < n && te_rng && !ranged) {
       const int s2 = te_songs[base + tid];
@@ -741,13 +756,13 @@
       mark(s2);
     }
     int total;
-    const int pre = block_excl_scan(len, &total, s_scan);
+    const int pre = block_excl_scan<NT>(len, &total, s_scan);
     s_pre[tid] = pre;
-    if (tid == 0) s_pre[kThreads] = total;
+    if (tid == 0) s_pre[NT] = total;
     __syncthreads();
     stamp_at(sb, 10);
     const int nsteps = n > 1 ? 32 - __clz(n - 1) : 0;
-    for (int i0 = tid; i0 < total; i0 += 16 * kThreads) {
+    for (int i0 = tid; i0 < total; i0 += 16 * NT) {
       const int ib = i0 - tid;
       int v[16];
       unsigned long long wv[16];
@@ -755,22 +770,22 @@
       for (int r = 0; r < 16; ++r) { v[r] = -1; wv[r] = 0ull; }
 #pragma unroll
       for (int g2 = 0; g2 < 4; g2 += 2) {
-        if (ib + g2 * 4 * kThreads >= total) break;
-        if (ib + (g2 + 1) * 4 * kThreads < total) {
+        if (ib + g2 * 4 * NT >= total) break;
+        if (ib + (g2 + 1) * 4 * NT < total) {
           int a[8], b[8];
 #pragma unroll
           for (int e = 0; e < 8; ++e) { a[e] = 0; b[e] = n; }
           for (int st = 0; st < nsteps; ++st) {
 #pragma unroll
             for (int e = 0; e < 8; ++e) {
-              const int i = i0 + (g2 * 4 + e) * kThreads;
+              const int i = i0 + (g2 * 4 + e) * NT;
               const int m = (a[e] + b[e]) >> 1;
               if (s_pre[m] <= i) a[e] = m; else b[e] = m;
             }
           }
 #pragma unroll
           for (int e = 0; e < 8; ++e) {
-            const int i = i0 + (g2 * 4 + e) * kThreads;
+            const int i = i0 + (g2 * 4 + e) * NT;
             if (i < total) {
               v[g2 * 4 + e] = trs_users[s_lo[a[e]] + (i - s_pre[a[e]])];
               wv[g2 * 4 + e] = (unsigned long long)s_w[a[e]];
@@ -785,14 +800,14 @@
         for (int st = 0; st < nsteps; ++st) {
 #pragma unroll
           for (int e = 0; e < 4; ++e) {
-            const int i = i0 + (g * 4 + e) * kThreads;
+            const int i = i0 + (g * 4 + e) * NT;
             const int m = (a[e] + b[e]) >> 1;
             if (s_pre[m] <= i) a[e] = m; else b[e] = m;
           }
         }
 #pragma unroll
         for (int e = 0; e < 4; ++e) {
-          const int i = i0 + (g * 4 + e) * kThreads;
+          const int i = i0 + (g * 4 + e) * NT;
           if (i < total) {
             v[g * 4 + e] = trs_users[s_lo[a[e]] + (i - s_pre[a[e]])];
             wv[g * 4 + e] = (unsigned long long)s_w[a[e]];
@@ -808,7 +823,7 @@
   }
 }
 
-template <int MODEL>
+template <int MODEL, int NT = kThreads>
 __device__ __forceinline__ void accumulate_neighbours(unsigned long long* Y, long long t0, long long t1,
                                                       const int* te_songs, const long long* trs_off,
                                                       const int* trs_users, const long long* q_song,
@@ -817,7 +832,7 @@
                                                       int v0 = 0, int v1 = 0, const int* sbound = nullptr,
                                                       int chunk_idx = 0, int nc1 = 0, const int2* te_rng = nullptr,
                                                       const long long* te_q = nullptr, long long* sb = nullptr) {
-  walk_neighbours<MODEL>(
+  walk_neighbours<MODEL, NT>(
       t0, t1, te_songs, trs_off, trs_users, q_song, s_lo, s_w, s_pre, s_scan,
       [&](int v, unsigned long long w) { atomicAdd(&Y[v - v0], w); },
       [&](int s2) {
@@ -896,6 +911,9 @@
 #ifndef MR_SCHED_SE
 #define MR_SCHED_SE 8
 #endif
+constexpr int sched_se(int nt) { return MR_SCHED_SE * 256 / nt > 1 ? MR_SCHED_SE * 256 / nt : 1; }
+constexpr int fused_pre(int nt) { return kFusedPre * 256 / nt > 1 ? kFusedPre * 256 / nt : 1; }
+constexpr int kFusedCap = 256;
 #ifndef MR_COUNTER_STRIDE
 #define MR_COUNTER_STRIDE 64
 #endif
@@ -948,11 +966,86 @@
   const float* rsq_c;
 };
 
-template <int MODEL, typename OutT, bool FUSED>
-__global__ __launch_bounds__(kThreads) void k_score(ScoreParams p) {
+template <int NT>
+__device__ __forceinline__ bool merge_staged(int n_tiles, int k, int merge_rows, int topk_lists, int stage_lists,
+                                             const long long* ck, const int* cs, long long* mk, int* ms,
+                                             unsigned char* gm, long long* wk, int* ws, long long* fk, int* fs,
+                                             long long* top_key, int* top_song, double* top_score, long long* sb) {
+  const int tid = threadIdx.x, w = tid >> 6;
+  int done = 0, off = 0;
+  bool merged_direct = false;
+  while (done < n_tiles) {
+    const int nl = min(n_tiles - done, stage_lists - off);
+    for (int i0 = tid; i0 < nl * k; i0 += 4 * NT) {
+      long long lk4[4];
+      int ls4[4];
+#pragma unroll
+      for (int r = 0; r < 4; ++r) {
+        const int i = i0 + r * NT;
+        lk4[r] = kKeyNone;
+        ls4[r] = -1;
+        if (i < nl * k) {
+          lk4[r] = ld_sc1(&ck[(size_t)done * k + i]);
+          ls4[r] = ld_sc1(&cs[(size_t)done * k + i]);
+        }
+      }
+#pragma unroll
+      for (int r = 0; r < 4; ++r) {
+        const int i = i0 + r * NT;
+        if (i < nl * k) {
+          mk[off * k + i] = lk4[r];
+          ms[off * k + i] = ls4[r];
+        }
+      }
+    }
+    for (int i = tid; i < off * k; i += NT) {
+      mk[i] = fk[i];
+      ms[i] = fs[i];
+    }
+    __syncthreads();
+    stamp_at(sb, 6);
+    bool merged = false;
+    TopkDst mdst;
+#ifndef MR_TOPK_VIA_LDS
+    mdst.key = top_key;
+    mdst.song = top_song;
+    mdst.score = top_score;
+#endif
+    if (!topk_lists && done == 0 && nl == n_tiles && k <= NT / 16) {
+      auto get_c = [&](int i, long long& key, int& song) { key = mk[i]; song = ms[i]; };
+      long long bk;
+      int bsg;
+      thread_best<NT>(nl * k, get_c, bk, bsg);
+      if (merge_rows == 16)
+        merged = block_topk_threshold_as<NT, decltype(get_c), 16, true, false>(nl * k, k, get_c, bk, bsg, gm,
+                                                                    wk, ws, kFusedCap, fk, fs, nullptr, mdst);
+      else if (merge_rows == 64)
+        merged = block_topk_threshold_as<NT, decltype(get_c), 64, true, false>(nl * k, k, get_c, bk, bsg, gm,
+                                                                    wk, ws, kFusedCap, fk, fs, nullptr, mdst);
+      else
+        merged = block_topk_threshold_as<NT, decltype(get_c), 32, true, false>(nl * k, k, get_c, bk, bsg, gm,
+                                                                    wk, ws, kFusedCap, fk, fs, nullptr, mdst);
+    }
+    if (!merged) {
+      if (w == 0) wave_merge_lists(nl + off, k, mk, ms, fk, fs);
+      __syncthreads();
+    }
+    stamp_at(sb, 8);
+    merged_direct = merged && mdst.key;
+    done += nl;
+    off = 1;
+  }
+  return merged_direct;
+}
+template <int MODEL, typename OutT, bool FUSED, int NT = kThreads, bool LEAN = false>
+__global__ __launch_bounds__(NT) void k_score(ScoreParams p) {
+  static_assert(NT == 256 || NT == 512 || NT == 1024, "workgroup of 4, 8 or 16 waves");
+  static_assert(FUSED || (NT == kThreads && !LEAN), "the separate shape keeps 256 threads");
+  constexpr int NW = NT / 64;
+  constexpr int kPre = fused_pre(NT);
   extern __shared__ __align__(16) unsigned char smem_raw[];
   const int bs = p.block_songs;
-  const ScoreLds L = score_lds(bs, FUSED ? p.n_tr : 0, p.topk, p.n_tiles, FUSED ? 0 : p.n_chunks);
+  const ScoreLds L = score_lds(bs, FUSED ? p.n_tr : 0, p.topk, p.n_tiles, FUSED ? 0 : p.n_chunks, NT);
   unsigned long long* acc = reinterpret_cast<unsigned long long*>(smem_raw + L.acc);
   unsigned* heard = reinterpret_cast<unsigned*>(smem_raw + L.heard);
   long long* wk = reinterpret_cast<long long*>(smem_raw + L.wk);
@@ -981,11 +1074,11 @@
 #endif
   MR_STAMP(0);
 
-  for (int i = tid; i < bw; i += kThreads) acc[i] = 0ull;
-  for (int i = tid; i < bs / 32; i += kThreads) heard[i] = 0u;
+  for (int i = tid; i < bw; i += NT) acc[i] = 0ull;
+  for (int i = tid; i < bs / 32; i += NT) heard[i] = 0u;
   const long long t0 = p.te_off[u], t1 = p.te_off[u + 1];
-  const bool sched = FUSED && p.te_sched != nullptr;
-  constexpr int kSE = MR_SCHED_SE;
+  const bool sched = LEAN || (FUSED && p.te_sched != nullptr);
+  constexpr int kSE = sched_se(NT);
   long long se0 = 0, se1 = 0;
   int hs0 = -1;
   uint2 sc1[kSE];
@@ -995,28 +1088,28 @@
     if (t1 > t0) hs0 = p.te_songs[min(t0 + tid, t1 - 1)];
     if (se1 > se0) {
 #pragma unroll
-      for (int r = 0; r < kSE; ++r) sc1[r] = p.te_sched[min(se0 + tid + (long long)r * kThreads, se1 - 1)];
-    }
-  }
-  double sc[kFusedPre];
-#pragma unroll
-  for (int j = 0; j < kFusedPre; ++j) {
-    const int i = tid + j * kThreads;
+      for (int r = 0; r < kSE; ++r) sc1[r] = p.te_sched[min(se0 + tid + (long long)r * NT, se1 - 1)];
+    }
+  }
+  double sc[kPre];
+#pragma unroll
+  for (int j = 0; j < kPre; ++j) {
+    const int i = tid + j * NT;
     sc[j] = (MODEL == MR_IBM && i < bw) ? p.sqrt_c[blo + i] : 1.0;
   }
 
   if (FUSED) {
     const int e0 = p.toff[(size_t)tile * p.n_tr], e1 = p.toff[(size_t)(tile + 1) * p.n_tr];
-    unsigned pk[kFusedPre];
-#pragma unroll
-    for (int j = 0; j < kFusedPre; ++j) {
-      const int i = e0 + tid + j * kThreads;
+    unsigned pk[kPre];
+#pragma unroll
+    for (int j = 0; j < kPre; ++j) {
+      const int i = e0 + tid + j * NT;
       pk[j] = i < e1 ? p.tpack[i] : 0xffffffffu;
     }
-    double str[kFusedPre];
-#pragma unroll
-    for (int r = 0; r < kFusedPre; ++r) {
-      const int v = tid + r * kThreads;
+    double str[kPre];
+#pragma unroll
+    for (int r = 0; r < kPre; ++r) {
+      const int v = tid + r * NT;
       str[r] = (MODEL == MR_UBM && v < p.n_tr) ? p.sqrt_tr[v] : 1.0;
     }
     unsigned long long* Y = reinterpret_cast<unsigned long long*>(smem_raw + L.y);
@@ -1030,7 +1123,7 @@
       }
     };
     const bool any = sched && se1 > se0;
-    for (int i = tid; i < p.n_tr; i += kThreads) Y[i] = 0ull;
+    for (int i = tid; i < p.n_tr; i += NT) Y[i] = 0ull;
     __syncthreads();
     if (sched) {
       if (any) gather();
@@ -1038,26 +1131,26 @@
         if (s2 >= blo && s2 < bhi) atomicOr(&heard[(s2 - blo) >> 5], 1u << ((s2 - blo) & 31));
       };
       if (t0 + tid < t1) mark(hs0);
-      for (long long i = t0 + tid + kThreads; i < t1; i += kThreads) mark(p.te_songs[i]);
+      for (long long i = t0 + tid + NT; i < t1; i += NT) mark(p.te_songs[i]);
 #ifdef MR_STAMPS
       stamp_at(sb, 10);
 #endif
       for (long long i0 = se0 + tid; any;) {
 #pragma unroll
         for (int r = 0; r < kSE; ++r)
-          if (i0 + (long long)r * kThreads < se1) atomicAdd(&Y[v[r]], wv[r]);
-        i0 += (long long)kSE * kThreads;
+          if (i0 + (long long)r * NT < se1) atomicAdd(&Y[v[r]], wv[r]);
+        i0 += (long long)kSE * NT;
         if (i0 >= se1) break;
 #pragma unroll
-        for (int r = 0; r < kSE; ++r) sc1[r] = p.te_sched[min(i0 + (long long)r * kThreads, se1 - 1)];
+        for (int r = 0; r < kSE; ++r) sc1[r] = p.te_sched[min(i0 + (long long)r * NT, se1 - 1)];
         gather();
       }
 #ifdef MR_STAMPS
       stamp_at(sb, 11);
 #endif
       __syncthreads();
-    } else
-    accumulate_neighbours<MODEL>(Y, t0, t1, p.te_songs, p.trs_off, p.trs_users, p.q_song,
+    } else if constexpr (!LEAN)
+    accumulate_neighbours<MODEL, NT>(Y, t0, t1, p.te_songs, p.trs_off, p.trs_users, p.q_song,
                                  reinterpret_cast<long long*>(smem_raw + L.s_lo),
                                  reinterpret_cast<long long*>(smem_raw + L.s_w),
                                  reinterpret_cast<int*>(smem_raw + L.s_pre),
@@ -1072,14 +1165,14 @@
     MR_STAMP(1);
     if (MODEL == MR_UBM) {
       const double rs_u = p.sqrt_te[u];
-      for (int v = tid, r = 0; v < p.n_tr; v += kThreads, ++r) {
+      for (int v = tid, r = 0; v < p.n_tr; v += NT, ++r) {
         const unsigned long long y = Y[v];
         if (y != 0ull) {
           double sv;
-          if (r < kFusedPre) {
+          if (r < kPre) {
             sv = str[0];
 #pragma unroll
-            for (int x = 1; x < kFusedPre; ++x) sv = r == x ? str[x] : sv;
+            for (int x = 1; x < kPre; ++x) sv = r == x ? str[x] : sv;
           } else {
             sv = p.sqrt_tr[v];
           }
@@ -1089,19 +1182,19 @@
       __syncthreads();
     }
 #pragma unroll
-    for (int j = 0; j < kFusedPre; ++j) {
+    for (int j = 0; j < kPre; ++j) {
       if (pk[j] == 0xffffffffu) continue;
       const unsigned long long y = Y[pk[j] >> 16];
       if (y != 0ull) atomicAdd(&acc[pk[j] & 0xffffu], y);
     }
-    for (int i = e0 + tid + kFusedPre * kThreads; i < e1; i += kThreads) {
+    for (int i = e0 + tid + kPre * NT; i < e1; i += NT) {
       const unsigned e = p.tpack[i];
       const unsigned long long y = Y[e >> 16];
       if (y != 0ull) atomicAdd(&acc[e & 0xffffu], y);
     }
   } else {
     __syncthreads();
-    for (long long i = t0 + tid; i < t1; i += kThreads) {
+    for (long long i = t0 + tid; i < t1; i += NT) {
       const int s = p.te_songs[i];
       if (s >= blo && s < bhi) atomicOr(&heard[(s - blo) >> 5], 1u << ((s - blo) & 31));
     }
@@ -1109,7 +1202,7 @@
     int* s_scan = reinterpret_cast<int*>(smem_raw + L.s_scan);
     const int nch = p.n_chunks;
     int cnt = 0;
-    for (int c0 = 0; c0 < nch; c0 += kThreads) {
+    for (int c0 = 0; c0 < nch; c0 += NT) {
       const int cc = c0 + tid;
       const int x = cc < nch ? p.nbr_cnt[(size_t)bu * nch + cc] : 0;
       int tot;
@@ -1155,7 +1248,7 @@
         }
       }
     };
-    const int step = kWaves * kStgItems;
+    const int step = NW * kStgItems;
     int v0[R], a0[R], b0[R], v1[R], a1[R], b1[R], v2[R];
     unsigned long long q0[R], q1[R], q2[R];
     int k0 = w * kStgItems;
@@ -1216,8 +1309,8 @@
   long long mk = kKeyNone;
   int ms = INT_MAX;
 #pragma unroll
-  for (int j = 0; j < kFusedPre; ++j) {
-    const int i = tid + j * kThreads;
+  for (int j = 0; j < kPre; ++j) {
+    const int i = tid + j * NT;
     if (i < bw) {
       const bool h = (heard[i >> 5] >> (i & 31)) & 1u;
       double score = (double)(long long)acc[i] * inv_f;
@@ -1228,7 +1321,8 @@
       if (key > mk) { mk = key; ms = blo + i; }
     }
   }
-  for (int i = tid + kFusedPre * kThreads; i < bw; i += kThreads) {
+  if constexpr (!LEAN)
+  for (int i = tid + kPre * NT; i < bw; i += NT) {
     const bool h = (heard[i >> 5] >> (i & 31)) & 1u;
     double score = (double)(long long)acc[i] * inv_f;
     if (MODEL == MR_IBM) score = score / p.sqrt_c[blo + i];
@@ -1261,29 +1355,31 @@
     tdst.sc1 = true;
   }
 #endif
-  if (!p.topk_lists && k <= kThreads / 16) {
+  if (LEAN || (!p.topk_lists && k <= NT / 16)) {
 #ifdef MR_STAMPS
     long long* sbt = sb ? sb + 3 : nullptr;
 #else
     long long* sbt = nullptr;
 #endif
-    thr_done = block_topk_threshold<kThreads, decltype(get_key), MR_TILE_ROWS>(
-        bw, k, get_key, mk, ms, smem_raw + L.gm, wk, ws, kWaves * kMaxTopK, fk, fs, sbt, tdst);
+    thr_done = block_topk_threshold_as<NT, decltype(get_key), MR_TILE_ROWS, true, LEAN>(
+        bw, k, get_key, mk, ms, smem_raw + L.gm, wk, ws, kFusedCap, fk, fs, sbt, tdst);
   }
   const bool direct = thr_done && tdst.key;
-  if (thr_done) {
+  if (LEAN ? __builtin_expect(thr_done, 1) : thr_done) {
+  } else if constexpr (LEAN) {
+    block_topk<NT>(bw, k, get_key, wk, ws, fk, fs);
   } else if (bs <= kMaxTopkTile) {
-    block_topk(bw, k, get_key, wk, ws, fk, fs);
+    block_topk<NT>(bw, k, get_key, wk, ws, fk, fs);
   } else {
     long long* lk = reinterpret_cast<long long*>(smem_raw + L.acc);
-    int* ls = reinterpret_cast<int*>(smem_raw + L.acc + kThreads * k * 8);
-    block_topk_wide(bw, k, get_key, lk, ls, wk, ws, fk, fs);
+    int* ls = reinterpret_cast<int*>(smem_raw + L.acc + kWideLists * k * 8);
+    block_topk_wide<NT>(bw, k, get_key, lk, ls, wk, ws, fk, fs);
   }
   MR_STAMP(4);
 
   if (p.n_tiles == 1) {
     if (!direct)
-      for (int r = tid; r < k; r += kThreads) {
+      for (int r = tid; r < k; r += NT) {
         const size_t o = (size_t)u * k + r;
         p.top_key[o] = fk[r];
         p.top_song[o] = fs[r];
@@ -1293,7 +1389,7 @@
   }
 
   if (!direct)
-    for (int r = tid; r < k; r += kThreads) {
+    for (int r = tid; r < k; r += NT) {
       st_sc1(&ck[(size_t)tile * k + r], fk[r]);
       st_sc1(&cs[(size_t)tile * k + r], fs[r]);
     }
@@ -1316,12 +1412,10 @@
   {
     long long* mk = reinterpret_cast<long long*>(smem_raw + L.acc);
     int* ms = reinterpret_cast<int*>(smem_raw + L.acc + L.stage_lists * k * 8);
-    const int w = tid >> 6;
-    int done = 0, off = 0;
     merged_direct = false;
 #ifndef MR_MERGE_VIA_LDS
     const int nck = p.n_tiles * k;
-    if (!p.topk_lists && nck <= kThreads && k <= kThreads / 16 && p.merge_rows == 32) {
+    if (LEAN || (!p.topk_lists && nck <= NT && k <= NT / 16 && p.merge_rows == 32)) {
       long long rk = kKeyNone;
       int rs = INT_MAX;
       if (tid < nck) {
@@ -1339,76 +1433,27 @@
       mdst.key = p.top_key + (size_t)u * k;
       mdst.song = p.top_song + (size_t)u * k;
       mdst.score = p.top_score + (size_t)u * k;
-      merged_direct = block_topk_threshold<kThreads, decltype(get_r), 32>(
+      merged_direct = block_topk_threshold_as<NT, decltype(get_r), 32, true, LEAN>(
           nck, k, get_r, rk >= 0 ? rk : kKeyNone, rk >= 0 ? rs : INT_MAX, smem_raw + L.gm, wk, ws,
-          kWaves * kMaxTopK, fk, fs, nullptr, mdst);
+          kFusedCap, fk, fs, nullptr, mdst);
       MR_STAMP(8);
     }
 #endif
-    while (!merged_direct && done < p.n_tiles) {
-      const int nl = min(p.n_tiles - done, L.stage_lists - off);
-      for (int i0 = tid; i0 < nl * k; i0 += 4 * kThreads) {
-        long long lk4[4];
-        int ls4[4];
-#pragma unroll
-        for (int r = 0; r < 4; ++r) {
-          const int i = i0 + r * kThreads;
-          lk4[r] = kKeyNone;
-          ls4[r] = -1;
-          if (i < nl * k) {
-            lk4[r] = ld_sc1(&ck[(size_t)done * k + i]);
-            ls4[r] = ld_sc1(&cs[(size_t)done * k + i]);
-          }
-        }
-#pragma unroll
-        for (int r = 0; r < 4; ++r) {
-          const int i = i0 + r * kThreads;
-          if (i < nl * k) {
-            mk[off * k + i] = lk4[r];
-            ms[off * k + i] = ls4[r];
-          }
-        }
-      }
-      for (int i = tid; i < off * k; i += kThreads) {
-        mk[i] = fk[i];
-        ms[i] = fs[i];
-      }
-      __syncthreads();
-      MR_STAMP(6);
-      bool merged = false;
-      TopkDst mdst;
-#ifndef MR_TOPK_VIA_LDS
-      mdst.key = p.top_key + (size_t)u * k;
-      mdst.song = p.top_song + (size_t)u * k;
-      mdst.score = p.top_score + (size_t)u * k;
-#endif
-      if (!p.topk_lists && done == 0 && nl == p.n_tiles && k <= kThreads / 16) {
-        auto get_c = [&](int i, long long& key, int& song) { key = mk[i]; song = ms[i]; };
-        long long bk;
-        int bsg;
-        thread_best<kThreads>(nl * k, get_c, bk, bsg);
-        if (p.merge_rows == 16)
-          merged = block_topk_threshold<kThreads, decltype(get_c), 16>(nl * k, k, get_c, bk, bsg, smem_raw + L.gm,
-                                                                      wk, ws, kWaves * kMaxTopK, fk, fs, nullptr, mdst);
-        else if (p.merge_rows == 64)
-          merged = block_topk_threshold<kThreads, decltype(get_c), 64>(nl * k, k, get_c, bk, bsg, smem_raw + L.gm,
-                                                                      wk, ws, kWaves * kMaxTopK, fk, fs, nullptr, mdst);
-        else
-          merged = block_topk_threshold<kThreads, decltype(get_c), 32>(nl * k, k, get_c, bk, bsg, smem_raw + L.gm,
-                                                                      wk, ws, kWaves * kMaxTopK, fk, fs, nullptr, mdst);
-      }
-      if (!merged) {
-        if (w == 0) wave_merge_lists(nl + off, k, mk, ms, fk, fs);
-        __syncthreads();
-      }
-      MR_STAMP(8);
-      merged_direct = merged && mdst.key;
-      done += nl;
-      off = 1;
+    if (LEAN ? __builtin_expect(!merged_direct, 0) : !merged_direct) {
+#ifdef MR_STAMPS
+      long long* sbm = sb;
+#else
+      long long* sbm = nullptr;
+#endif
+      long long* tk = p.top_key + (size_t)u * k;
+      int* tsg = p.top_song + (size_t)u * k;
+      double* tsc = p.top_score + (size_t)u * k;
+      merged_direct = merge_staged<NT>(p.n_tiles, k, LEAN ? 32 : p.merge_rows, LEAN ? 0 : p.topk_lists, L.stage_lists,
+                                       ck, cs, mk, ms, smem_raw + L.gm, wk, ws, fk, fs, tk, tsg, tsc, sbm);
     }
   }
   if (!merged_direct)
-    for (int r = tid; r < k; r += kThreads) {
+    for (int r = tid; r < k; r += NT) {
       const size_t o = (size_t)u * k + r;
       p.top_key[o] = fk[r];
       p.top_song[o] = fs[r];
@@ -3207,6 +3252,8 @@
   bool loaded = false;
   bool ran = false;
   bool fused = false;
+  int fused_nt = kThreads;
+  bool fused_lean = false;
   int shape = kShapeSeparate;
   int last_model = -1;
   int n_tr = 0, n_te = 0, n_s = 0;
@@ -3386,6 +3433,19 @@
   const char* e = std::getenv("MR_FUSED_SCHED");
   return MR_FUSED_SCHED && !(e && std::atoi(e) == 0);
 }
+#ifndef MR_FUSED_LEAN_DEFAULT
+#define MR_FUSED_LEAN_DEFAULT 1
+#endif
+int fused_nt_opt(int block_songs) {
+  const char* e = std::getenv("MR_FUSED_NT");
+  const int v = e ? std::atoi(e) : 0;
+  if (v == 256 || v == 512 || v == 1024) return v;
+  return block_songs > 512 ? 512 : 256;
+}
+bool fused_lean_opt() {
+  const char* e = std::getenv("MR_FUSED_LEAN");
+  return e ? std::atoi(e) != 0 : MR_FUSED_LEAN_DEFAULT != 0;
+}
 int cooc_nt_opt() {
   const char* e = std::getenv("MR_COOC_NT");
   return e && std::atoi(e) == 512 ? 512 : 1024;
@@ -3459,11 +3519,25 @@
   return (int)std::max<long long>(256, std::min(bs, cover));
 }
 
+bool lean_ok(const mr_ctx* c, int nt, int bs, int k, int n_tiles) {
+  return c->fused && c->te_sched.p != nullptr && !c->opt.topk_lists && k >= 1 && k <= MR_TILE_ROWS &&
+         k <= nt / 16 && (long long)n_tiles * k <= nt && merge_rows_opt() == 32 && bs <= fused_pre(nt) * nt &&
+         bs <= kMaxTopkTile;
+}
+
+template <int MODEL, typename OutT>
+ScoreKernel fused_kernel(int nt, bool lean) {
+  if (nt == 1024) return lean ? k_score<MODEL, OutT, true, 1024, true> : k_score<MODEL, OutT, true, 1024, false>;
+  if (nt == 512) return lean ? k_score<MODEL, OutT, true, 512, true> : k_score<MODEL, OutT, true, 512, false>;
+  return lean ? k_score<MODEL, OutT, true, 256, true> : k_score<MODEL, OutT, true, 256, false>;
+}
+
 template <int MODEL>
 void pick_kernels(mr_ctx* c) {
   const bool f64 = c->opt.out_dtype == MR_OUT_F64;
   if (c->fused)
-    c->score_kernel[MODEL] = f64 ? k_score<MODEL, double, true> : k_score<MODEL, float, true>;
+    c->score_kernel[MODEL] = f64 ? fused_kernel<MODEL, double>(c->fused_nt, c->fused_lean)
+                                 : fused_kernel<MODEL, float>(c->fused_nt, c->fused_lean);
   else
     c->score_kernel[MODEL] = f64 ? k_score<MODEL, double, false> : k_score<MODEL, float, false>;
   if (c->shape == kShapeWide) {
@@ -4165,10 +4239,13 @@
                  !(e && e[0] == '0');
   }
   c->wide_lds = wide ? (size_t)wide_lds<kWideThreads>(bs, k, n_chunks).total : 0;
+  c->fused_nt = fused ? fused_nt_opt(bs) : kThreads;
+  if (fused && score_lds(bs, n_tr, k, lp.n_tiles, 0, c->fused_nt).total > kLdsBytes) c->fused_nt = kThreads;
+  c->fused_lean = fused && fused_lean_opt() && lean_ok(c, c->fused_nt, bs, k, lp.n_tiles);
   pick_kernels<MR_UBM>(c);
   pick_kernels<MR_IBM>(c);
   c->score_lds = wide ? c->wide_lds
-                      : (size_t)score_lds(bs, fused ? n_tr : 0, k, lp.n_tiles, fused ? 0 : n_chunks).total;
+                      : (size_t)score_lds(bs, fused ? n_tr : 0, k, lp.n_tiles, fused ? 0 : n_chunks, c->fused_nt).total;
   if (c->score_lds > 160 * 1024)
     return fail(MR_E_INVALID, "scoring kernel needs %zu B of LDS (> 160 KiB): lower block_songs or topk",
                 c->score_lds);
@@ -4480,6 +4557,14 @@
   if (fused) *fused = c->shape;
   if (block_songs) *block_songs = c->block_songs;
   if (n_tiles) *n_tiles = c->n_tiles;
+  return MR_OK;
+}
+
+int mr_fused_info(const mr_ctx* c, int32_t* threads, int32_t* lean) {
+  if (!c) return fail(MR_E_INVALID, "null context");
+  if (!c->loaded) return fail(MR_E_STATE, "mr_fused_info before mr_load");
+  if (threads) *threads = c->fused ? c->fused_nt : 0;
+  if (lean) *lean = c->fused_lean ? 1 : 0;
   return MR_OK;
 }
 
@@ -4745,8 +4830,8 @@
       sp.topk_lists = c->opt.topk_lists;
       if (c->mm_on && wide) { sp.mm_key = c->mm_key.p; sp.mm_n = c->n_te; }
       sp.cand = wide && c->cand_on && !sp.mm_key; sp.rsq_c = c->rsq_c.p;
-      hipLaunchKernelGGL(c->score_kernel[model], dim3(c->n_tiles, gy), dim3(wide ? kWideThreads : kThreads),
-                         c->score_lds, st, sp);
+      hipLaunchKernelGGL(c->score_kernel[model], dim3(c->n_tiles, gy),
+                         dim3(wide ? kWideThreads : c->fused ? c->fused_nt : kThreads), c->score_lds, st, sp);
       MR_HIP(hipGetLastError());
       if (wide && k > 0 && c->n_tiles > 1) {
         MergeParams mp{c->n_tiles, k, k, (long long)c->n_tiles * k, (long long)k, (long long)k, c->cand_key.p, c->cand_song.p,
diff --git a/musicrecommendation_amd/engine.py b/musicrecommendation_amd/engine.py
--- a/musicrecommendation_amd/engine.py
+++ b/musicrecommendation_amd/engine.py
@@ -65,6 +65,9 @@
                    "mr_launch_info")
         self.shape = _lib.SHAPES[fz.value]
         self.fused, self.block_songs, self.n_tiles = self.shape == "fused", bsz.value, nt.value
+        fth, fln = ctypes.c_int32(), ctypes.c_int32()
+        _lib.check(self._L.mr_fused_info(self._h, ctypes.byref(fth), ctypes.byref(fln)), "mr_fused_info")
+        self.fused_threads, self.fused_lean = fth.value, bool(fln.value)
         b, ch, nch = ctypes.c_int32(), ctypes.c_int32(), ctypes.c_int32()
         _lib.check(self._L.mr_batch_info(self._h, ctypes.byref(b), ctypes.byref(ch), ctypes.byref(nch)),
                    "mr_batch_info")
```

Result: faster. 18.79 billion, median of 6 (+10.7%).
